# Whisper-6/DynamicTreeAttn

Measured on AMD Instinct MI355X. Metric: tree-attn fwd+bwd tokens/sec, Qwen3-0.6B tau2-16k tries, higher is better.
Workload: dtype bf16

## Files before the change

### dynamictreeattn_amd/_lib.py

```python
from __future__ import annotations

import ctypes as C
import os

from .build import LIB

_lib = None
_i32, _i64, _f32, _vp = C.c_int32, C.c_int64, C.c_float, C.c_void_p

_PROTOS = {
    "dta_version": ([], C.c_int),
    "dta_take_pending_error": ([C.c_char_p, _i32], C.c_int),
    "dta_lcp_adjacent": ([_vp, _vp, _vp, _i32, _vp, _vp, _vp], C.c_int),
    "dta_leafize": ([_vp, _vp, _i32, _vp, _vp, _vp, _vp, _vp], C.c_int),
    "dta_preorder_meta": ([_vp] * 8 + [_i32, _i32] + [_vp] * 4 + [_vp], C.c_int),
    "dta_tree_attn_fwd": ([_vp] * 8 + [_i32] * 6 + [_i64] * 3 + [_f32, _i32, _vp], C.c_int),
    "dta_tree_attn_bwd": ([_vp] * 14 + [_i32] * 6 + [_i64] * 5 + [_f32, _i32, _i32, _vp], C.c_int),
    "dta_tree_attn_fwd_ex": ([_vp] * 8 + [_i32] * 6 + [_i64] * 8 + [_f32, _i32, _vp], C.c_int),
    "dta_tree_attn_bwd_ex": ([_vp] * 14 + [_i32] * 6 + [_i64] * 12 + [_f32, _i32, _i32, _i32, _vp, _i32, _vp, _i32, _vp, _vp], C.c_int),
    "dta_tree_attn_fwd_win": ([_vp] * 8 + [_i32] * 6 + [_i64] * 8 + [_f32, _i32, _vp, _i32, _vp], C.c_int),
    "dta_tree_attn_bwd_win": ([_vp] * 14 + [_i32] * 6 + [_i64] * 12 + [_f32, _i32, _i32, _i32, _vp, _i32, _vp, _i32, _vp, _vp, _i32, _vp], C.c_int),
    "dta_window_lo": ([_vp] * 4 + [_i32, _i32, _i32, _vp, _vp], C.c_int),
    "dta_logprob_entropy_fwd": ([_vp] * 8 + [_i32, _i32, _i64, _f32, _i32, _vp], C.c_int),
    "dta_logprob_entropy_shard_stats": ([_vp] * 6 + [_i32, _i32, _i64, _f32, _i32, _vp], C.c_int),
    "dta_logprob_entropy_bwd": ([_vp] * 10 + [_i32, _i32, _i64, _i64, _f32, _i32, _vp], C.c_int),
    "dta_rmsnorm_fwd": ([_vp] * 6 + [_i32, _i32, _f32, _i32, _vp], C.c_int),
    "dta_rmsnorm_bwd_blocks": ([_i32], C.c_int),
    "dta_rmsnorm_bwd": ([_vp] * 7 + [_i32, _i32, _i32, _vp], C.c_int),
    "dta_qk_norm_rope_fwd": ([_vp] * 5 + [_i32, _i32, _i32, _i64, _f32, _i32, _vp], C.c_int),
    "dta_qk_norm_rope_bwd_blocks": ([_i64], C.c_int),
    "dta_qk_norm_rope_bwd": ([_vp] * 7 + [_i32, _i32, _i32, _i64, _i64, _i64, _i64, _i32, _vp], C.c_int),
    "dta_swiglu_fwd": ([_vp] * 3 + [_i64, _i32, _i64, _i32, _vp], C.c_int),
    "dta_swiglu_bwd": ([_vp] * 5 + [_i64, _i32, _i64, _i64, _i32, _vp], C.c_int),
    "dta_transpose": ([_vp, _vp, _i64, _i64, _i64, _i64, _i32, _vp], C.c_int),
    "dta_sum_slabs": ([_vp, _i64, _i64, _i64, _vp, _vp, _i32, _vp], C.c_int),
    "dta_moe_router_fwd": ([_vp] * 4 + [_i32] * 5 + [_vp], C.c_int),
    "dta_moe_router_bwd": ([_vp] * 5 + [_i32] * 5 + [_vp], C.c_int),
    "dta_moe_permute_workspace": ([_i32, _i32], C.c_int),
    "dta_moe_tile_bound": ([_i32, _i32], C.c_int),
    "dta_moe_permute": ([_vp, _i32, _i32, _i32] + [_vp] * 5 + [_vp], C.c_int),
    "dta_moe_grouped_gemm": ([_i32] + [_vp] * 7 + [_i32] * 5 + [_vp], C.c_int),
    "dta_moe_combine_fwd": ([_vp] * 4 + [_i32] * 4 + [_vp], C.c_int),
    "dta_moe_combine_bwd": ([_vp] * 6 + [_i32] * 4 + [_vp], C.c_int),
    "dta_lora_down": ([_vp, _i64, _vp, _i64, _vp, _i64, _vp, _i32, _i32, _i32, _i32, _vp], C.c_int),
    "dta_lora_wgrad_slabs": ([_i32, _i32], C.c_int),
    "dta_lora_wgrad": ([_vp, _i64, _vp, _i64, _vp, _vp, _i32, _i32, _i32, _i32, _vp], C.c_int),
}
EXPORTS = tuple(_PROTOS)
_ERR = {-1: "DTA_EINVAL", -2: "DTA_EUNSUPPORTED", -3: "DTA_EALIGN", -4: "DTA_ELAUNCH", -5: "DTA_EPRIOR"}


def _hip_runtimes_mapped():
    try:
        with open("/proc/self/maps") as f:
            return sorted({line.split()[-1] for line in f if "libamdhip64" in line})
    except OSError:
        return []


def lib():
    global _lib
    if _lib is None:
        if not os.path.exists(LIB):
            raise RuntimeError(f"{LIB} is missing: run `python -m dynamictreeattn_amd.build` (hipcc, gfx950). "
                               "There is no CPU fallback for the hot path.")
        import torch
        l = C.CDLL(LIB)
        rts = _hip_runtimes_mapped()
        if len(rts) > 1:
            raise RuntimeError("more than one libamdhip64 is mapped into this process: " + ", ".join(rts) +
                               " — libdta_mi355x.so must resolve to the HIP runtime torch ships")
        for name, (args, res) in _PROTOS.items():
            fn = getattr(l, name)
            fn.argtypes, fn.restype = args, res
        _lib = l
    return _lib


def check(status: int, what: str):
    if status == 0:
        return
    if status == -5:
        buf = C.create_string_buffer(256)
        code = lib().dta_take_pending_error(buf, 256)
        raise RuntimeError(f"{what}: not launched, a HIP error was already pending on this thread: {buf.value.decode() or code} "
                           f"(hipError {code}; now cleared — after an asynchronous kernel fault the GPU context stays unusable)")
    raise RuntimeError(f"{what} failed: {_ERR.get(status, status)}")


def ptr(t):
    return None if t is None else t.data_ptr()
```

### dynamictreeattn_amd/csrc/tree_attn.hip

```cpp
#include <hip/hip_runtime.h>
#include <stdint.h>
#include <type_traits>
#include "dta_common.h"

#if defined(DTA_STAMP) && DTA_STAMP
__device__ unsigned long long* dta_stamp_buf = nullptr;
extern "C" int dta_debug_set_stamp_buffer(void* p) { return hipMemcpyToSymbol(HIP_SYMBOL(dta_stamp_buf), &p, sizeof(p)) == hipSuccess ? 0 : -4; }
#define DTA_STAMP_DECL unsigned long long st_prev_, st_sum_[6] = {0, 0, 0, 0, 0, 0}; unsigned long long st_tiles_ = 0; \
  __builtin_amdgcn_sched_barrier(0); asm volatile("s_memtime %0\n\ts_waitcnt lgkmcnt(0)" : "=s"(st_prev_) :: "memory"); __builtin_amdgcn_sched_barrier(0);
#define DTA_STAMP_AT(K) { unsigned long long t_; __builtin_amdgcn_sched_barrier(0); asm volatile("s_memtime %0\n\ts_waitcnt lgkmcnt(0)" : "=s"(t_) :: "memory"); \
  __builtin_amdgcn_sched_barrier(0); st_sum_[K] += t_ - st_prev_; st_prev_ = t_; }
#define DTA_STAMP_TILE ++st_tiles_;
#define DTA_STAMP_STORE if (dta_stamp_buf && lane == 0) { unsigned long long* o_ = dta_stamp_buf + ((size_t)blockIdx.x * 8 + wave) * 8; \
  for (int k_ = 0; k_ < 6; ++k_) o_[k_] = st_sum_[k_]; o_[6] = st_tiles_; o_[7] = (unsigned long long)__builtin_amdgcn_s_getreg(0xF804) ; }
#else
#define DTA_STAMP_DECL
#define DTA_STAMP_AT(K)
#define DTA_STAMP_TILE
#define DTA_STAMP_STORE
#endif

namespace {

typedef __attribute__((ext_vector_type(16))) float f32x16;
typedef __attribute__((ext_vector_type(4))) short s16x4;
typedef __attribute__((ext_vector_type(8))) short s16x8;
typedef __attribute__((ext_vector_type(8))) __bf16 bf16x8;
typedef __attribute__((ext_vector_type(8))) _Float16 f16x8;
typedef __attribute__((ext_vector_type(4))) __bf16 bf16x4;
typedef __attribute__((ext_vector_type(4))) _Float16 f16x4;

template <int DT> struct Ty;
template <> struct Ty<DTA_BF16> {
  using e = __bf16; using v8 = bf16x8; using v4 = bf16x4;
  static __device__ __forceinline__ f32x16 mma(v8 a, v8 b, f32x16 c) { return __builtin_amdgcn_mfma_f32_32x32x16_bf16(a, b, c, 0, 0, 0); }
};
template <> struct Ty<DTA_F16> {
  using e = _Float16; using v8 = f16x8; using v4 = f16x4;
  static __device__ __forceinline__ f32x16 mma(v8 a, v8 b, f32x16 c) { return __builtin_amdgcn_mfma_f32_32x32x16_f16(a, b, c, 0, 0, 0); }
};

struct AttnParams {
  const void *q, *k, *v, *o, *dout;
  void *out, *dq, *dk, *dv;
  float *lse_w; const float* lse_r; float* delta;
  const int32_t *subtree_end, *run_ptr, *runs, *ktile_qend;
  const int32_t *dkv_units, *dkv_splits; float* dkv_ws;
  int32_t Tq, Tk, q_offset, Hq, Hkv, group;
  int32_t hgroups, head0;
  int64_t q_st, q_sh, kv_st, kv_sh, v_st, v_sh, o_st, o_sh, dq_st, dq_sh, dkv_st, dkv_sh;
  float scale; int32_t accumulate; int32_t ktile;
};
struct AttnParamsW : AttnParams { const int32_t* win_lo; int32_t window; };
template <bool WIN> using AttnP = typename std::conditional<WIN, AttnParamsW, AttnParams>::type;

constexpr float LOG2E = 1.4426950408889634f;

__device__ __forceinline__ int swz64(int row) { return ((row & 2) << 1) | ((row >> 2) & 3); }
template <int D> __device__ __forceinline__ int img_off_d(int row, int ch) {
  if constexpr (D == 128) return row * 256 + ((ch ^ (((row & 3) << 2) | ((row >> 2) & 3))) << 4);
  else { static_assert(D == 64, "head_dim 64 or 128"); return row * 128 + ((ch ^ swz64(row)) << 4); }
}
template <int D> constexpr int tile_bytes() { return 64 * 2 * D; }

template <class V8, int D> __device__ __forceinline__ V8 row_frag(const char* img, int row, int ch) {
  return *reinterpret_cast<const V8*>(img + img_off_d<D>(row, ch));
}

__device__ __forceinline__ s16x4 tr_read(const char* p) {
  return __builtin_amdgcn_ds_read_tr16_b64_v4i16((__attribute__((address_space(3))) s16x4*)(p));
}

template <class V8, int D> __device__ __forceinline__ V8 tr_frag(const char* img, int R0, int mb, int lane) {
  const int G = lane >> 4, hh = lane >> 5, i = lane & 15, qd = i >> 2, p = i & 3;
  const int ch = 4 * mb + 2 * (G & 1) + (p >> 1);
  const int ra = R0 + 4 * hh + qd;
  s16x4 lo = tr_read(img + img_off_d<D>(ra, ch) + 8 * (p & 1));
  s16x4 hi = tr_read(img + img_off_d<D>(ra + 8, ch) + 8 * (p & 1));
  s16x8 both = {lo[0], lo[1], lo[2], lo[3], hi[0], hi[1], hi[2], hi[3]};
  return __builtin_bit_cast(V8, both);
}

template <int DT> __device__ __forceinline__ typename Ty<DT>::v8 pack_half(const f32x16& x, int s2) {
  typename Ty<DT>::v8 r;
#pragma unroll
  for (int j = 0; j < 8; ++j) r[j] = (typename Ty<DT>::e)x[8 * s2 + j];
  return r;
}

__device__ __forceinline__ float fast_exp2(float x) { return __builtin_amdgcn_exp2f(x); }

struct TileIter {
  const int32_t* runs; int ri, re;
  int k0, kend, flag;
  int diag_first_q;
  __device__ __forceinline__ bool load_run() {
    while (ri < re) {
      k0 = __builtin_amdgcn_readfirstlane(runs[4 * ri]); kend = __builtin_amdgcn_readfirstlane(runs[4 * ri + 1]);
      flag = __builtin_amdgcn_readfirstlane(runs[4 * ri + 2]);
      if (k0 < kend) return true;
      ++ri;
    }
    return false;
  }
  __device__ __forceinline__ bool advance() {
    k0 += 64;
    if (k0 < kend) return true;
    if (runs == nullptr) return false;
    ++ri;
    return load_run();
  }
  __device__ __forceinline__ bool masked() const {
    if (runs == nullptr) return (k0 + 63 > diag_first_q) || (k0 + 64 > kend);
    return flag != 0 || (k0 + 64 > kend);
  }
};

#ifndef DTA_FWD_THR
#define DTA_FWD_THR 4.0f
#endif
constexpr float FWD_THR = DTA_FWD_THR;
constexpr int SE_BYTES = 256;

__device__ __forceinline__ float max3(float a, float b, float c) { return fmaxf(fmaxf(a, b), c); }
__device__ __forceinline__ float half_max(float x) {
  const unsigned u = __float_as_uint(x);
  const auto r = __builtin_amdgcn_permlane32_swap(u, u, false, false);
  return fmaxf(__uint_as_float(r[0]), __uint_as_float(r[1]));
}

template <int D> struct FragOffsT { int row[D / 16]; int tr[D / 16]; };
template <int D> __device__ __forceinline__ FragOffsT<D> frag_offsets(int lane) {
  FragOffsT<D> o;
  const int r = lane & 31, h = lane >> 5;
#pragma unroll
  for (int s = 0; s < D / 16; ++s) o.row[s] = img_off_d<D>(r, 2 * s + h);
  const int G = lane >> 4, i = lane & 15, qd = i >> 2, pp = i & 3;
#pragma unroll
  for (int mb = 0; mb < D / 32; ++mb) {
    const int ch = 4 * mb + 2 * (G & 1) + (pp >> 1);
    o.tr[mb] = img_off_d<D>(4 * h + qd, ch) + 8 * (pp & 1);
    o.tr[D / 32 + mb] = img_off_d<D>(4 * h + qd + 8, ch) + 8 * (pp & 1);
  }
  return o;
}
template <class V8> __device__ __forceinline__ V8 tr_pair(const char* lo_p, const char* hi_p) {
  s16x4 lo = tr_read(lo_p);
  s16x4 hi = tr_read(hi_p);
  s16x8 both = {lo[0], lo[1], lo[2], lo[3], hi[0], hi[1], hi[2], hi[3]};
  return __builtin_bit_cast(V8, both);
}
template <class V8, int D> __device__ __forceinline__ V8 tr_frag_o(const char* img_r0, const FragOffsT<D>& o, int mb) {
  s16x4 lo = tr_read(img_r0 + o.tr[mb]);
  s16x4 hi = tr_read(img_r0 + o.tr[D / 32 + mb]);
  s16x8 both = {lo[0], lo[1], lo[2], lo[3], hi[0], hi[1], hi[2], hi[3]};
  return __builtin_bit_cast(V8, both);
}

__device__ __forceinline__ uint32_t lds_addr(const void* p) {
  return (uint32_t)(uintptr_t)(__attribute__((address_space(3))) const char*)(p);
}
__device__ __forceinline__ void dma_pair2(uint32_t oa0, uint32_t oa1, const void* ba, uint32_t ob0, uint32_t ob1, const void* bb, uint32_t lds) {
  asm volatile(
      "s_nop 4\n\t"
      "s_mov_b32 m0, %6\n\t"
      "s_nop 0\n\t"
      "global_load_lds_dwordx4 %0, %4\n\t"
      "s_add_u32 m0, %6, 0x4000\n\t"
      "s_nop 0\n\t"
      "global_load_lds_dwordx4 %2, %5\n\t"
      "s_add_u32 m0, %6, 0x400\n\t"
      "s_nop 0\n\t"
      "global_load_lds_dwordx4 %1, %4\n\t"
      "s_add_u32 m0, %6, 0x4400\n\t"
      "s_nop 0\n\t"
      "global_load_lds_dwordx4 %3, %5"
      :: "v"(oa0), "v"(oa1), "v"(ob0), "v"(ob1), "s"(ba), "s"(bb), "s"(lds) : "memory", "scc");
}
__device__ __forceinline__ void dma_dword(uint32_t off, const void* base, uint32_t lds) {
  asm volatile("s_nop 4\n\ts_mov_b32 m0, %2\n\ts_nop 0\n\tglobal_load_lds_dword %0, %1" :: "v"(off), "s"(base), "s"(lds) : "memory");
}
#define DMA_WAIT() asm volatile("s_waitcnt vmcnt(0)" ::: "memory")

template <int D> __device__ __forceinline__ uint32_t dma_src_off_d(int row, int img_row, int lane, int64_t stride, int esz) {
  if constexpr (D == 128) return (uint32_t)((row * stride + ((lane & 15) ^ (((img_row & 3) << 2) | ((img_row >> 2) & 3))) * 8) * (int64_t)esz);
  else return (uint32_t)((row * stride + ((lane & 7) ^ swz64(img_row)) * 8) * (int64_t)esz);
}
template <int D> constexpr int dma_lane_row_shift() { return D == 128 ? 4 : 3; }
template <int TB> __device__ __forceinline__ void dma_one2(uint32_t oa, const void* ba, uint32_t ob, const void* bb, uint32_t lds) {
  asm volatile(
      "s_nop 4\n\t"
      "s_mov_b32 m0, %4\n\t"
      "s_nop 0\n\t"
      "global_load_lds_dwordx4 %0, %2\n\t"
      "s_add_u32 m0, %4, %5\n\t"
      "s_nop 0\n\t"
      "global_load_lds_dwordx4 %1, %3"
      :: "v"(oa), "v"(ob), "s"(ba), "s"(bb), "s"(lds), "n"(TB) : "memory", "scc");
}

#define DTA_KV_PPW(NW) (DH / 8 / (NW))
#define DTA_KV_ROW(NW, I) ((512 / DH) * (wave * DTA_KV_PPW(NW) + (I)) + (lane >> dma_lane_row_shift<DH>()))
#define DTA_KV_OFFSETS(NW)                                                                                 \
  uint32_t voff_k[DTA_KV_PPW(NW)], voff_v[DTA_KV_PPW(NW)];                                                 \
  _Pragma("unroll") for (int i_ = 0; i_ < DTA_KV_PPW(NW); ++i_) {                                          \
    const int row_ = DTA_KV_ROW(NW, i_);                                                                   \
    voff_k[i_] = dma_src_off_d<DH>(row_, row_, lane, p.kv_st, sizeof(e));                                  \
    voff_v[i_] = dma_src_off_d<DH>(row_, row_, lane, p.v_st, sizeof(e)); }
#define DTA_KV_DMA(BASE, K0, NW)                                                                           \
  { char* base_ = (BASE); const int k0_ = (K0);                                                            \
    if (wave == 0) {                                                                                       \
      if (p.subtree_end) { int ki_ = k0_ + lane; ki_ = ki_ < p.Tk ? ki_ : p.Tk - 1;                        \
        dma_dword((uint32_t)ki_ * 4u, p.subtree_end, lds_addr(base_ + 2 * tile_bytes<DH>())); }           \
      else reinterpret_cast<int*>(base_ + 2 * tile_bytes<DH>())[lane] = 0x7fffffff; }                     \
    const char* kb_ = reinterpret_cast<const char*>(kbase) + (int64_t)k0_ * p.kv_st * (int64_t)sizeof(e);  \
    const char* vb_ = reinterpret_cast<const char*>(vbase) + (int64_t)k0_ * p.v_st * (int64_t)sizeof(e);   \
    uint32_t ok_[DTA_KV_PPW(NW)], ov_[DTA_KV_PPW(NW)];                                                     \
    _Pragma("unroll") for (int i_ = 0; i_ < DTA_KV_PPW(NW); ++i_) { ok_[i_] = voff_k[i_]; ov_[i_] = voff_v[i_]; } \
    if (k0_ + 64 > p.Tk) {                          \
      _Pragma("unroll") for (int i_ = 0; i_ < DTA_KV_PPW(NW); ++i_) {                                      \
        const int row_ = DTA_KV_ROW(NW, i_);                                                               \
        const int rr_ = k0_ + row_ < p.Tk ? row_ : p.Tk - 1 - k0_;                                         \
        ok_[i_] = dma_src_off_d<DH>(rr_, row_, lane, p.kv_st, sizeof(e)); ov_[i_] = dma_src_off_d<DH>(rr_, row_, lane, p.v_st, sizeof(e)); } } \
    if constexpr (DH == 128) {                                                                             \
      _Pragma("unroll") for (int i_ = 0; i_ < DTA_KV_PPW(NW); i_ += 2)                                     \
        dma_pair2(ok_[i_], ok_[i_ + 1], kb_, ov_[i_], ov_[i_ + 1], vb_, lds_addr(base_ + (wave * DTA_KV_PPW(NW) + i_) * 1024)); \
    } else {                                                                                               \
      _Pragma("unroll") for (int i_ = 0; i_ < DTA_KV_PPW(NW); ++i_)                                        \
        dma_one2<tile_bytes<DH>()>(ok_[i_], kb_, ov_[i_], vb_, lds_addr(base_ + (wave * DTA_KV_PPW(NW) + i_) * 1024)); } }

#ifndef DTA_V_PRELOAD_N
#define DTA_V_PRELOAD_N 4
#endif
#if DTA_V_PRELOAD_N
#define DTA_V_PRELOAD v8 vpre_[DTA_V_PRELOAD_N]; _Pragma("unroll") for (int i_ = 0; i_ < DTA_V_PRELOAD_N; ++i_) { vpre_[i_] = tr_frag_o<v8>(Vs + 32 * DH * (i_ / (DH / 32)), offs, i_ % (DH / 32)); asm volatile("" : "+v"(vpre_[i_])); }
#define DTA_V_FRAG(S4, DB) (((DH / 32) * (S4) + (DB) < DTA_V_PRELOAD_N) ? vpre_[(DH / 32) * (S4) + (DB) < DTA_V_PRELOAD_N ? (DH / 32) * (S4) + (DB) : 0] : tr_frag_o<v8>(Vs + 32 * DH * (S4), offs, (DB)))
#else
#define DTA_V_PRELOAD
#define DTA_V_FRAG(S4, DB) tr_frag_o<v8>(Vs + 32 * DH * (S4), offs, (DB))
#endif

#ifndef DTA_SCORE_ORDER
#define DTA_SCORE_ORDER 1
#endif
#if DTA_SCORE_ORDER
#define DTA_SCORE_MFMAS                                                                                    \
    { v8 ka_ = *reinterpret_cast<const v8*>(Ks + offs.row[0]), kb2_ = *reinterpret_cast<const v8*>(Ks + 64 * DH + offs.row[0]); \
      _Pragma("unroll") for (int s = 0; s < DH / 16; ++s) {                                                \
        v8 na_ = ka_, nb_ = kb2_;                                                                          \
        if (s < DH / 16 - 1) { na_ = *reinterpret_cast<const v8*>(Ks + offs.row[s + 1]); nb_ = *reinterpret_cast<const v8*>(Ks + 64 * DH + offs.row[s + 1]); } \
        X[0] = T::mma(ka_, qf[s], X[0]); X[1] = T::mma(kb2_, qf[s], X[1]);                                 \
        ka_ = na_; kb2_ = nb_;                                                                             \
      } }
#else
#define DTA_SCORE_MFMAS                                                                                    \
    _Pragma("unroll") for (int kb = 0; kb < 2; ++kb)                                                       \
      _Pragma("unroll") for (int s = 0; s < DH / 16; ++s)                                                  \
        X[kb] = T::mma(*reinterpret_cast<const v8*>(Ks + 64 * DH * kb + offs.row[s]), qf[s], X[kb]);
#endif

template <int DT, int HPB, int DH, bool WIN>
__global__ __launch_bounds__(256 * HPB, 2) void tree_attn_fwd_kernel(AttnP<WIN> p) {
  using T = Ty<DT>; using e = typename T::e; using v8 = typename T::v8; using v4 = typename T::v4;
  constexpr int TB = tile_bytes<DH>(), NKS = DH / 16, NDB = DH / 32;
  constexpr int NW = 4 * HPB, BUF = 2 * TB + SE_BYTES;
  __shared__ __attribute__((aligned(16))) char smem[2 * BUF];

  const int tid = threadIdx.x, lane = tid & 63, r = lane & 31, h = lane >> 5;
  const int wave = __builtin_amdgcn_readfirstlane(tid >> 6);
  const int hb = wave >> 2, rw = wave & 3;
  const int bid = blockIdx.x;
  const int hgroups = p.hgroups;
  const int kvh = bid % p.Hkv; const int rest = bid / p.Hkv; const int hgb = rest % hgroups;
  const int nqt = (p.Tq + DTA_QTILE - 1) / DTA_QTILE;
  const int qt = nqt - 1 - rest / hgroups;
  const int hq = kvh * p.group + p.head0 + hgb * HPB + hb;
  const int q0 = qt * DTA_QTILE;
  const int qrow = q0 + rw * 32 + r;
  const int qrow_c = qrow < p.Tq ? qrow : p.Tq - 1;
  const int qidx = p.q_offset + qrow;
  int wlo = 0, wmax = 0;
  if constexpr (WIN) {
    wlo = p.win_lo ? p.win_lo[qrow_c] : (qidx - p.window + 1 > 0 ? qidx - p.window + 1 : 0);
    wmax = p.win_lo ? 0 : p.q_offset + (q0 + DTA_QTILE < p.Tq ? q0 + DTA_QTILE : p.Tq) - p.window;
  }

  TileIter it; it.runs = p.runs; it.diag_first_q = p.subtree_end ? -64 : p.q_offset + q0;
  if (p.runs) { it.ri = p.run_ptr[qt]; it.re = p.run_ptr[qt + 1]; if (!it.load_run()) return; }
  else { it.ri = 0; it.re = 1; it.k0 = 0; it.flag = 1; int last = p.q_offset + (q0 + DTA_QTILE < p.Tq ? q0 + DTA_QTILE : p.Tq); it.kend = last < p.Tk ? last : p.Tk; if (it.kend <= 0) return; }
  if constexpr (WIN) {
    const int lo0 = p.q_offset + q0 - p.window + 1;
    if (!p.runs && !p.win_lo && lo0 > 0) { it.k0 = lo0; if (it.k0 >= it.kend) return; }
  }

  const e* qp = reinterpret_cast<const e*>(p.q) + (int64_t)qrow_c * p.q_st + (int64_t)hq * p.q_sh;
  v8 qf[NKS];
#pragma unroll
  for (int s = 0; s < NKS; ++s) qf[s] = *reinterpret_cast<const v8*>(qp + 16 * s + 8 * h);

  const e* kbase = reinterpret_cast<const e*>(p.k) + (int64_t)kvh * p.kv_sh;
  const e* vbase = reinterpret_cast<const e*>(p.v) + (int64_t)kvh * p.v_sh;
  const FragOffsT<DH> offs = frag_offsets<DH>(lane);
  DTA_KV_OFFSETS(NW)

  f32x16 O[NDB];
#pragma unroll
  for (int db = 0; db < NDB; ++db)
#pragma unroll
    for (int g = 0; g < 16; ++g) O[db][g] = 0.f;
  float m = -1e30f, lsum = 0.f;
  const float c = p.scale * LOG2E;

  int ck0 = it.k0, ckend = it.kend; bool cmask = it.masked() || (WIN && it.k0 < wmax);
  DTA_KV_DMA(smem, it.k0, NW)
  bool has_next = it.advance();
#pragma unroll
  for (int s = 0; s < NKS; ++s) asm volatile("" : "+v"(qf[s]));
  DMA_WAIT(); __syncthreads();

#define FWD_TILE(BUFI)                                                                                     \
  {                                                                                                        \
    int nk0_ = 0, nkend_ = 0; bool nmask_ = false;                                                         \
    DTA_STAMP_AT(5) DTA_STAMP_TILE                                                                         \
    if (has_next) { nk0_ = it.k0; nkend_ = it.kend; nmask_ = it.masked() || (WIN && it.k0 < wmax); DTA_KV_DMA(smem + (1 - (BUFI)) * BUF, it.k0, NW) } \
    DTA_STAMP_AT(0)                                                                                        \
    const char* Ks = smem + (BUFI) * BUF; const char* Vs = Ks + TB;                                \
    const int* se_s = reinterpret_cast<const int*>(Ks + 2 * TB);                                   \
    f32x16 X[2];                                                                                           \
    _Pragma("unroll") for (int kb = 0; kb < 2; ++kb)                                                       \
      _Pragma("unroll") for (int g = 0; g < 16; ++g) X[kb][g] = 0.f;                                       \
    DTA_SCORE_MFMAS                                                                                        \
    DTA_STAMP_AT(1)                                                                                        \
    if (cmask) {                                                                                           \
      const int qlim = qidx < ckend ? qidx : ckend - 1;       \
      _Pragma("unroll") for (int kb = 0; kb < 2; ++kb)                                                     \
        _Pragma("unroll") for (int gq = 0; gq < 4; ++gq) {                                                 \
          const int kl = 32 * kb + 8 * gq + 4 * h;                                                         \
          const int4 se4 = *reinterpret_cast<const int4*>(se_s + kl);                                      \
          const int sev[4] = {se4.x, se4.y, se4.z, se4.w};                                                 \
          _Pragma("unroll") for (int j = 0; j < 4; ++j) {                                                  \
            const bool ok = (ck0 + kl + j <= qlim) && (qidx < sev[j]) && (!WIN || ck0 + kl + j >= wlo);    \
            X[kb][4 * gq + j] = ok ? X[kb][4 * gq + j] : -INFINITY;                                        \
          }                                                                                                \
        }                                                                                                  \
    }                                                                                                      \
    DTA_V_PRELOAD                                                                                          \
    float mx = max3(X[0][0], X[0][1], X[0][2]), mx1 = max3(X[1][0], X[1][1], X[1][2]);    \
    _Pragma("unroll") for (int g = 3; g < 15; g += 2) { mx = max3(mx, X[0][g], X[0][g + 1]); mx1 = max3(mx1, X[1][g], X[1][g + 1]); } \
    mx = max3(mx, X[0][15], mx1);                                                                          \
    mx = half_max(fmaxf(mx, X[1][15]));         \
    const float mc = mx * c;                                                                               \
    if (__any(mc > m + FWD_THR)) {              \
      const float mnew = fmaxf(m, mc);                                                                     \
      const float alpha = fast_exp2(m - mnew);                                                             \
      m = mnew; lsum *= alpha;                                                                             \
      _Pragma("unroll") for (int db = 0; db < NDB; ++db)                                                   \
        _Pragma("unroll") for (int g = 0; g < 16; ++g) O[db][g] *= alpha;                                  \
    }                                                                                                      \
    DTA_STAMP_AT(2)                                                                                        \
    _Pragma("unroll") for (int kb = 0; kb < 2; ++kb)                                                       \
      _Pragma("unroll") for (int g = 0; g < 16; ++g) { const float pv = fast_exp2(__builtin_fmaf(X[kb][g], c, -m)); lsum += pv; X[kb][g] = pv; } \
    _Pragma("unroll") for (int s4 = 0; s4 < 4; ++s4) {                                                     \
      const v8 pb = pack_half<DT>(X[s4 >> 1], s4 & 1);                                                     \
      _Pragma("unroll") for (int db = 0; db < NDB; ++db) O[db] = T::mma(DTA_V_FRAG(s4, db), pb, O[db]);      \
    }                                                                                                      \
    DTA_STAMP_AT(3)                                                                                        \
    DMA_WAIT(); __syncthreads();                         \
    DTA_STAMP_AT(4)                                                                                        \
    if (!has_next) break;                                                                                  \
    ck0 = nk0_; ckend = nkend_; cmask = nmask_;                                                            \
    has_next = it.advance();                                                                               \
  }
  DTA_STAMP_DECL
  while (true) {
    FWD_TILE(0)
    FWD_TILE(1)
  }
#undef FWD_TILE
  DTA_STAMP_STORE

  lsum += __shfl_xor(lsum, 32);
  const float inv = 1.f / lsum;
  if (qrow < p.Tq) {
    e* op = reinterpret_cast<e*>(p.out) + (int64_t)qrow * p.o_st + (int64_t)hq * p.o_sh;
#pragma unroll
    for (int db = 0; db < NDB; ++db)
#pragma unroll
      for (int gq = 0; gq < 4; ++gq) {
        v4 w;
#pragma unroll
        for (int j = 0; j < 4; ++j) w[j] = (e)(O[db][4 * gq + j] * inv);
        *reinterpret_cast<v4*>(op + 32 * db + 8 * gq + 4 * h) = w;
      }
    if (h == 0) p.lse_w[(int64_t)hq * p.Tq + qrow] = m + __builtin_amdgcn_logf(lsum);
  }
}

template <int DT, int HPB, int DH, bool WIN>
__global__ __launch_bounds__(256 * HPB, 2) void tree_attn_bwd_dq_kernel(AttnP<WIN> p) {
  using T = Ty<DT>; using e = typename T::e; using v8 = typename T::v8; using v4 = typename T::v4;
  constexpr int TB = tile_bytes<DH>(), NKS = DH / 16, NDB = DH / 32;
  __shared__ __attribute__((aligned(16))) char smem[2 * (2 * TB + SE_BYTES)];

  const int tid = threadIdx.x, lane = tid & 63, r = lane & 31, h = lane >> 5;
  const int wave = __builtin_amdgcn_readfirstlane(tid >> 6);
  const int hb = wave >> 2, rw = wave & 3;
  const int bid = blockIdx.x;
  const int hgroups = p.hgroups;
  const int kvh = bid % p.Hkv; const int rest = bid / p.Hkv; const int hgb = rest % hgroups;
  const int nqt = (p.Tq + DTA_QTILE - 1) / DTA_QTILE;
  const int qt = nqt - 1 - rest / hgroups;
  const int hq = kvh * p.group + p.head0 + hgb * HPB + hb;
  const int q0 = qt * DTA_QTILE;
  const int qrow = q0 + rw * 32 + r;
  const int qrow_c = qrow < p.Tq ? qrow : p.Tq - 1;
  const int qidx = p.q_offset + qrow;
  int wlo = 0, wmax = 0;
  if constexpr (WIN) {
    wlo = p.win_lo ? p.win_lo[qrow_c] : (qidx - p.window + 1 > 0 ? qidx - p.window + 1 : 0);
    wmax = p.win_lo ? 0 : p.q_offset + (q0 + DTA_QTILE < p.Tq ? q0 + DTA_QTILE : p.Tq) - p.window;
  }

  const e* qp = reinterpret_cast<const e*>(p.q) + (int64_t)qrow_c * p.q_st + (int64_t)hq * p.q_sh;
  const e* dop = reinterpret_cast<const e*>(p.dout) + (int64_t)qrow_c * p.o_st + (int64_t)hq * p.o_sh;
  const e* op = reinterpret_cast<const e*>(p.o) + (int64_t)qrow_c * p.o_st + (int64_t)hq * p.o_sh;
  v8 qf[NKS], dof[NKS];
  float dsum = 0.f;
#pragma unroll
  for (int s = 0; s < NKS; ++s) {
    qf[s] = *reinterpret_cast<const v8*>(qp + 16 * s + 8 * h);
    dof[s] = *reinterpret_cast<const v8*>(dop + 16 * s + 8 * h);
    const v8 of = *reinterpret_cast<const v8*>(op + 16 * s + 8 * h);
#pragma unroll
    for (int j = 0; j < 8; ++j) dsum += (float)dof[s][j] * (float)of[j];
  }
  dsum += __shfl_xor(dsum, 32);
  const float delta = dsum;
  const float lse2 = p.lse_r[(int64_t)hq * p.Tq + qrow_c];
  if (h == 0 && qrow < p.Tq) p.delta[(int64_t)hq * p.Tq + qrow] = -delta;

  TileIter it; it.runs = p.runs; it.diag_first_q = p.subtree_end ? -64 : p.q_offset + q0;
  bool any = true;
  if (p.runs) { it.ri = p.run_ptr[qt]; it.re = p.run_ptr[qt + 1]; any = it.load_run(); }
  else { it.ri = 0; it.re = 1; it.k0 = 0; it.flag = 1; int last = p.q_offset + (q0 + DTA_QTILE < p.Tq ? q0 + DTA_QTILE : p.Tq); it.kend = last < p.Tk ? last : p.Tk; any = it.kend > 0; }
  if constexpr (WIN) {
    const int lo0 = p.q_offset + q0 - p.window + 1;
    if (!p.runs && !p.win_lo && lo0 > 0) { it.k0 = lo0; any = any && it.k0 < it.kend; }
  }

  const e* kbase = reinterpret_cast<const e*>(p.k) + (int64_t)kvh * p.kv_sh;
  const e* vbase = reinterpret_cast<const e*>(p.v) + (int64_t)kvh * p.v_sh;
  constexpr int NW = 4 * HPB, BUF = 2 * TB + SE_BYTES;
  DTA_KV_OFFSETS(NW)

  f32x16 DQ[NDB];
#pragma unroll
  for (int db = 0; db < NDB; ++db)
#pragma unroll
    for (int g = 0; g < 16; ++g) DQ[db][g] = 0.f;
  const float c = p.scale * LOG2E;

  f32x16 DI;
#pragma unroll
  for (int g = 0; g < 16; ++g) DI[g] = -delta;
  if (any) {
    int ck0 = it.k0, ckend = it.kend; bool cmask = it.masked() || (WIN && it.k0 < wmax);
    DTA_KV_DMA(smem, it.k0, NW)
    bool has_next = it.advance();
    DMA_WAIT(); __syncthreads();
    int cur = 0;
    while (true) {
      int nk0 = 0, nkend = 0; bool nmask = false;
      if (has_next) { nk0 = it.k0; nkend = it.kend; nmask = it.masked() || (WIN && it.k0 < wmax); DTA_KV_DMA(smem + (cur ^ 1) * BUF, it.k0, NW) }
      const char* Ks = smem + cur * BUF; const char* Vs = Ks + TB;
      const int* se_s = reinterpret_cast<const int*>(Ks + 2 * TB);
#pragma unroll
      for (int kb = 0; kb < 2; ++kb) {
        f32x16 X, DP;
#pragma unroll
        for (int g = 0; g < 16; ++g) X[g] = 0.f;
        {
          v8 kf_ = row_frag<v8, DH>(Ks, 32 * kb + r, h), vf_ = row_frag<v8, DH>(Vs, 32 * kb + r, h);
#pragma unroll
          for (int s = 0; s < NKS; ++s) {
            v8 nk_ = kf_, nv_ = vf_;
            if (s < NKS - 1) { nk_ = row_frag<v8, DH>(Ks, 32 * kb + r, 2 * s + 2 + h); nv_ = row_frag<v8, DH>(Vs, 32 * kb + r, 2 * s + 2 + h); }
            X = T::mma(kf_, qf[s], X);
            DP = T::mma(vf_, dof[s], s == 0 ? DI : DP);
            kf_ = nk_; vf_ = nv_;
          }
          __builtin_amdgcn_sched_group_barrier(0x100, 4, 0);
#pragma unroll
          for (int i_ = 0; i_ < NKS - 2; ++i_) { __builtin_amdgcn_sched_group_barrier(0x008, 2, 0); __builtin_amdgcn_sched_group_barrier(0x100, 2, 0); }
          __builtin_amdgcn_sched_group_barrier(0x008, 4, 0);
        }
        if (cmask) {
          const int qlim = qidx < ckend ? qidx : ckend - 1;
#pragma unroll
          for (int gq = 0; gq < 4; ++gq) {
            const int kl = 32 * kb + 8 * gq + 4 * h;
            const int4 se4 = *reinterpret_cast<const int4*>(se_s + kl);
            const int sev[4] = {se4.x, se4.y, se4.z, se4.w};
#pragma unroll
            for (int j = 0; j < 4; ++j) {
              const int g = 4 * gq + j;
              const bool ok = (ck0 + kl + j <= qlim) && (qidx < sev[j]) && (!WIN || ck0 + kl + j >= wlo);
              const float pv = ok ? fast_exp2(__builtin_fmaf(X[g], c, -lse2)) : 0.f;
              X[g] = pv * DP[g];
            }
          }
        } else {
#pragma unroll
          for (int g = 0; g < 16; ++g) X[g] = fast_exp2(__builtin_fmaf(X[g], c, -lse2)) * DP[g];
        }
#pragma unroll
        for (int s2 = 0; s2 < 2; ++s2) {
          const v8 db_ = pack_half<DT>(X, s2);
#pragma unroll
          for (int db = 0; db < NDB; ++db) DQ[db] = T::mma(tr_frag<v8, DH>(Ks, 32 * kb + 16 * s2, db, lane), db_, DQ[db]);
        }
      }
      DMA_WAIT(); __syncthreads();
      if (!has_next) break;
      cur ^= 1; ck0 = nk0; ckend = nkend; cmask = nmask;
      has_next = it.advance();
    }
  }
  if (qrow < p.Tq) {
    e* dqp = reinterpret_cast<e*>(p.dq) + (int64_t)qrow * p.dq_st + (int64_t)hq * p.dq_sh;
#pragma unroll
    for (int db = 0; db < NDB; ++db)
#pragma unroll
      for (int gq = 0; gq < 4; ++gq) {
        v4 w;
#pragma unroll
        for (int j = 0; j < 4; ++j) w[j] = (e)(DQ[db][4 * gq + j] * p.scale);
        *reinterpret_cast<v4*>(dqp + 32 * db + 8 * gq + 4 * h) = w;
      }
  }
}

#ifndef DTA_KV2_PIN
#define DTA_KV2_PIN 2
#endif
#if DTA_KV2_PIN == 2
#define DTA_KV2_PIN_ORDER                                                                                  \
    __builtin_amdgcn_sched_group_barrier(0x100, 4, 0);                                                     \
    _Pragma("unroll") for (int i_ = 0; i_ < 2 * NKS; ++i_) { __builtin_amdgcn_sched_group_barrier(0x100, 2, 0); __builtin_amdgcn_sched_group_barrier(0x008, 1, 0); }
#elif DTA_KV2_PIN
#define DTA_KV2_PIN_ORDER                                                                                  \
    __builtin_amdgcn_sched_group_barrier(0x100, 12, 0);                                                    \
    _Pragma("unroll") for (int i_ = 0; i_ < NKS - 2; ++i_) { __builtin_amdgcn_sched_group_barrier(0x008, 2, 0); __builtin_amdgcn_sched_group_barrier(0x100, 4, 0); } \
    __builtin_amdgcn_sched_group_barrier(0x008, 4, 0);
#else
#define DTA_KV2_PIN_ORDER
#endif

template <int D> constexpr int kv2_slot() { return 2 * (D / 16) * 1024; }
template <int D> constexpr int kv2_frags() { return 4 * kv2_slot<D>(); }
template <int D, bool WIN> constexpr int kv2_buf() { return 2 * tile_bytes<D>() + (WIN ? 768 : 512); }
template <int D, bool WIN> constexpr int kv2_lds() { return kv2_frags<D>() + 2 * kv2_buf<D, WIN>() + 16; }

template <int DT, int DH, bool WIN>
__global__ __launch_bounds__(512, 2) void tree_attn_bwd_dkv2_kernel(AttnP<WIN> p) {
  using T = Ty<DT>; using e = typename T::e; using v8 = typename T::v8; using v4 = typename T::v4;
  constexpr int KT = 128;
  constexpr int TB = tile_bytes<DH>(), NKS = DH / 16, NDB = DH / 32, KV2_FRAGS = kv2_frags<DH>(), KV2_BUF = kv2_buf<DH, WIN>(), KSLOT = kv2_slot<DH>();
  __shared__ __attribute__((aligned(16))) char smem_all[kv2_lds<DH, WIN>()];
  const int tid8 = threadIdx.x, tid = tid8 & 255, lane = tid & 63, r = lane & 31, h = lane >> 5;
  const int wave8 = __builtin_amdgcn_readfirstlane(tid8 >> 6);
  const int grp = wave8 >> 2, wave = wave8 & 3;
  char* kvs = smem_all + wave * KSLOT;
  char* smem = smem_all + KV2_FRAGS;
  const int bid = blockIdx.x;
  const int kvh = bid % p.Hkv; const int unit = bid / p.Hkv;
  const int kt = p.dkv_units ? p.dkv_units[4 * unit] : unit;
  const int slab = p.dkv_units ? p.dkv_units[4 * unit + 3] : -1;
  const int k0 = kt * KT;
  const int q_hi = p.q_offset + p.Tq;
  const int kidx = k0 + wave * 32 + r;
  int se_l;
  { const int kc = kidx < p.Tk ? kidx : p.Tk - 1;
    int se = (kidx < p.Tk) ? (p.subtree_end ? p.subtree_end[kidx] : 0x7fffffff) : 0;
    se_l = se < q_hi ? se : q_hi;
    if (grp == 0) {
      const e* kp = reinterpret_cast<const e*>(p.k) + (int64_t)kc * p.kv_st + (int64_t)kvh * p.kv_sh;
      const e* vp = reinterpret_cast<const e*>(p.v) + (int64_t)kc * p.v_st + (int64_t)kvh * p.v_sh;
#pragma unroll
      for (int s = 0; s < NKS; ++s) {
        *reinterpret_cast<v8*>(kvs + s * 1024 + lane * 16) = *reinterpret_cast<const v8*>(kp + 16 * s + 8 * h);
        *reinterpret_cast<v8*>(kvs + KSLOT / 2 + s * 1024 + lane * 16) = *reinterpret_cast<const v8*>(vp + 16 * s + 8 * h);
      }
    } }
  int* se_min_s = reinterpret_cast<int*>(smem_all + KV2_FRAGS + 2 * KV2_BUF);
  { int mn = se_l;
#pragma unroll
    for (int o = 32; o > 0; o >>= 1) { const int t = __shfl_xor(mn, o); mn = t < mn ? t : mn; }
    if (lane == 0 && grp == 0) se_min_s[wave] = mn; }
  __syncthreads();
  const int se_min = __builtin_amdgcn_readfirstlane(min(min(se_min_s[0], se_min_s[1]), min(se_min_s[2], se_min_s[3])));

  const FragOffsT<DH> offs = frag_offsets<DH>(lane);
  f32x16 DK[NDB], DV[NDB];
#pragma unroll
  for (int db = 0; db < NDB; ++db)
#pragma unroll
    for (int g = 0; g < 16; ++g) { DK[db][g] = 0.f; DV[db][g] = 0.f; }

  int qbeg, qend;
  if (p.dkv_units) { qbeg = __builtin_amdgcn_readfirstlane(p.dkv_units[4 * unit + 1]); qend = __builtin_amdgcn_readfirstlane(p.dkv_units[4 * unit + 2]); }
  else {
    qbeg = k0 > p.q_offset ? k0 : p.q_offset;
    qend = p.ktile_qend ? p.ktile_qend[kt] : q_hi; qend = qend < q_hi ? qend : q_hi;
    if constexpr (WIN) if (!p.win_lo) {
      const int64_t wl = (int64_t)k0 + KT - 1 + p.window; qend = wl < qend ? (int)wl : qend;
    }
  }
  const int ntile = qend > qbeg ? (qend - qbeg + 63) / 64 : 0;
  const int total = ntile * p.group;
  const float c = p.scale * LOG2E;

  constexpr int NP = DH / 64;
  uint32_t voff_q[NP], voff_d[NP];
#pragma unroll
  for (int i = 0; i < NP; ++i) {
    const int row_ = 8 * wave8 + (512 / DH) * i + (lane >> dma_lane_row_shift<DH>());
    voff_q[i] = dma_src_off_d<DH>(row_, row_, lane, p.q_st, sizeof(e));
    voff_d[i] = dma_src_off_d<DH>(row_, row_, lane, p.o_st, sizeof(e));
  }
  const uint32_t lds_tiles = lds_addr(smem);
  const int64_t q_step = 64 * p.q_st * (int64_t)sizeof(e), d_step = 64 * p.o_st * (int64_t)sizeof(e);
  const int64_t q_wrap = p.q_sh * (int64_t)sizeof(e) - ntile * q_step, d_wrap = p.o_sh * (int64_t)sizeof(e) - ntile * d_step;
  int64_t q_cur = ((int64_t)(kvh * p.group) * p.q_sh + (int64_t)(qbeg - p.q_offset) * p.q_st) * (int64_t)sizeof(e);
  int64_t d_cur = ((int64_t)(kvh * p.group) * p.o_sh + (int64_t)(qbeg - p.q_offset) * p.o_st) * (int64_t)sizeof(e);
  int64_t c_cur = (int64_t)(kvh * p.group) * p.Tq;
  int row_n = qbeg - p.q_offset, ti_n = 0;
#define KV2_DMA(B)                                                                                         \
  { const uint32_t lb_ = lds_tiles + (uint32_t)(B) * KV2_BUF;                                              \
    if (wave8 < 2) { int qr_ = row_n + lane; qr_ = qr_ < p.Tq ? qr_ : p.Tq - 1;    \
      dma_dword((uint32_t)qr_ * 4u, (wave8 == 0 ? p.lse_r : p.delta) + c_cur, lb_ + 2 * TB + wave8 * 256); } \
    if constexpr (WIN) if (wave8 == 2 && p.win_lo) { int qr_ = row_n + lane; qr_ = qr_ < p.Tq ? qr_ : p.Tq - 1;    \
      dma_dword((uint32_t)qr_ * 4u, p.win_lo, lb_ + 2 * TB + 512); }                                       \
    uint32_t oq_[NP], od_[NP];                                                                             \
    _Pragma("unroll") for (int i_ = 0; i_ < NP; ++i_) { oq_[i_] = voff_q[i_]; od_[i_] = voff_d[i_]; }      \
    if (row_n + 64 > p.Tq) {                        \
      _Pragma("unroll") for (int i_ = 0; i_ < NP; ++i_) {                                                  \
        const int ra_ = 8 * wave8 + (512 / DH) * i_ + (lane >> dma_lane_row_shift<DH>());                  \
        const int ca_ = row_n + ra_ < p.Tq ? ra_ : p.Tq - 1 - row_n;                                       \
        oq_[i_] = dma_src_off_d<DH>(ca_, ra_, lane, p.q_st, sizeof(e)); od_[i_] = dma_src_off_d<DH>(ca_, ra_, lane, p.o_st, sizeof(e)); } } \
    if constexpr (NP == 2) dma_pair2(oq_[0], oq_[1], reinterpret_cast<const char*>(p.q) + q_cur, od_[0], od_[1], reinterpret_cast<const char*>(p.dout) + d_cur, lb_ + wave8 * 2048); \
    else dma_one2<TB>(oq_[0], reinterpret_cast<const char*>(p.q) + q_cur, od_[0], reinterpret_cast<const char*>(p.dout) + d_cur, lb_ + wave8 * 1024); \
    ++ti_n; row_n += 64; q_cur += q_step; d_cur += d_step;                                                 \
    if (ti_n >= ntile) { ti_n = 0; row_n = qbeg - p.q_offset; q_cur += q_wrap; d_cur += d_wrap; c_cur += p.Tq; } }

  int ar[NKS], at[NKS];
#pragma unroll
  for (int j = 0; j < NKS; ++j) { ar[j] = offs.row[j] + grp * (64 * DH); at[j] = offs.tr[j] + grp * (64 * DH); }
  const int rc_off = (32 * grp + 4 * h) * 4;

#define KV2_TILE(BUFI)                                                                                     \
  {                                                                                                        \
    const int ti = ti_c;                                                                                   \
    ti_c += 1;                                                                                             \
    if (ti_c >= ntile) ti_c = 0;                                                                           \
    if (idx + 1 < total) KV2_DMA(1 - (BUFI))       \
    const char* tb = smem + (BUFI) * KV2_BUF;                                                              \
    const char* rc = tb + 2 * TB + rc_off;                                                         \
    const int qi0 = qbeg + 64 * ti + 32 * grp;                        \
    bool full = (qbeg + 64 * ti >= k0 + KT - 1) && (qbeg + 64 * ti + 63 < se_min);    \
    if constexpr (WIN) full = full && !p.win_lo && qbeg + 64 * ti + 64 - p.window <= k0;    \
     \
    f32x16 S, DP;                                                                                          \
    _Pragma("unroll") for (int gq = 0; gq < 4; ++gq) {                                                     \
      const float4 d4 = *reinterpret_cast<const float4*>(rc + 256 + 32 * gq);                              \
      DP[4 * gq] = d4.x; DP[4 * gq + 1] = d4.y; DP[4 * gq + 2] = d4.z; DP[4 * gq + 3] = d4.w;              \
    }                                                                                                      \
    _Pragma("unroll") for (int g = 0; g < 16; ++g) S[g] = 0.f;                                             \
    _Pragma("unroll") for (int s = 0; s < NKS; ++s) {                                                      \
      const v8 aq = *reinterpret_cast<const v8*>(tb + ar[s]);                                              \
      const v8 ad = *reinterpret_cast<const v8*>(tb + ar[s] + TB);                                         \
      const v8 kfs = *reinterpret_cast<const v8*>(kvs + s * 1024 + lane * 16);                             \
      const v8 vfs = *reinterpret_cast<const v8*>(kvs + KSLOT / 2 + s * 1024 + lane * 16);                 \
      S = T::mma(aq, kfs, S); DP = T::mma(ad, vfs, DP);                                                    \
    }                                                                                                      \
    DTA_KV2_PIN_ORDER                                                                                      \
    float nl[16];                                                                                          \
    _Pragma("unroll") for (int gq = 0; gq < 4; ++gq) {                                                     \
      const float4 l4 = *reinterpret_cast<const float4*>(rc + 32 * gq);                                    \
      nl[4 * gq] = l4.x; nl[4 * gq + 1] = l4.y; nl[4 * gq + 2] = l4.z; nl[4 * gq + 3] = l4.w;              \
    }                                                                                                      \
    if (full) {                                                                                            \
      _Pragma("unroll") for (int g = 0; g < 16; ++g) {                                                     \
        const float pv = fast_exp2(__builtin_fmaf(S[g], c, -nl[g]));                                       \
        S[g] = pv;                                                                                         \
        DP[g] = pv * DP[g];                                                                                \
      }                                                                                                    \
    } else {                                                                                               \
      int wl[16];                                    \
      if constexpr (WIN) {                                                                                 \
        if (p.win_lo) {                                                                                    \
          _Pragma("unroll") for (int gq = 0; gq < 4; ++gq) {                                               \
            const int4 w4 = *reinterpret_cast<const int4*>(rc + 512 + 32 * gq);                            \
            wl[4 * gq] = w4.x; wl[4 * gq + 1] = w4.y; wl[4 * gq + 2] = w4.z; wl[4 * gq + 3] = w4.w; }      \
        } else {                                                                                           \
          _Pragma("unroll") for (int g = 0; g < 16; ++g) wl[g] = qi0 + 8 * (g >> 2) + 4 * h + (g & 3) - p.window + 1; } \
      }                                                                                                    \
      _Pragma("unroll") for (int g = 0; g < 16; ++g) {                                                     \
        const int qi = qi0 + 8 * (g >> 2) + 4 * h + (g & 3);                                               \
        const bool ok = (kidx <= qi) && (qi < se_l) && (!WIN || kidx >= wl[g]);                            \
        const float pv = ok ? fast_exp2(__builtin_fmaf(S[g], c, -nl[g])) : 0.f;                            \
        S[g] = pv;                                                                                         \
        DP[g] = pv * DP[g];                                                                                \
      }                                                                                                    \
    }                                                                                                      \
    _Pragma("unroll") for (int s2 = 0; s2 < 2; ++s2) {                                                     \
      const v8 pb = pack_half<DT>(S, s2), sbf = pack_half<DT>(DP, s2);                                     \
      _Pragma("unroll") for (int db = 0; db < NDB; ++db) {                                                 \
        const v8 adt = tr_pair<v8>(tb + at[db] + TB + 32 * DH * s2, tb + at[NDB + db] + TB + 32 * DH * s2); \
        const v8 aqt = tr_pair<v8>(tb + at[db] + 32 * DH * s2, tb + at[NDB + db] + 32 * DH * s2);          \
        DV[db] = T::mma(adt, pb, DV[db]); DK[db] = T::mma(aqt, sbf, DK[db]);                               \
      }                                                                                                    \
    }                                                                                                      \
    DMA_WAIT(); __syncthreads();                                                                           \
    ++idx;                                                                                                 \
  }

  {
    int ti_c = 0;
    if (total > 0) KV2_DMA(0)
    DMA_WAIT(); __syncthreads();
    int idx = 0;
    while (idx < total) {
      KV2_TILE(0)
      if (idx >= total) break;
      KV2_TILE(1)
    }
  }
#undef KV2_TILE
#undef KV2_DMA
  {
    float* red = reinterpret_cast<float*>(smem_all);
#pragma unroll
    for (int db = 0; db < NDB; ++db) {
      if (grp == 1) {
#pragma unroll
        for (int g = 0; g < 16; ++g) { red[g * 256 + tid] = DK[db][g]; red[(16 + g) * 256 + tid] = DV[db][g]; }
      }
      __syncthreads();
      if (grp == 0) {
#pragma unroll
        for (int g = 0; g < 16; ++g) { DK[db][g] += red[g * 256 + tid]; DV[db][g] += red[(16 + g) * 256 + tid]; }
      }
      __syncthreads();
    }
    if (grp == 1) return;
  }
#pragma unroll
  for (int db = 0; db < NDB; ++db)
#pragma unroll
    for (int g = 0; g < 16; ++g) DK[db][g] *= p.scale;
  const int kloc = wave * 32 + r;
  if (slab >= 0) {
    float* ws = p.dkv_ws + ((int64_t)slab * p.Hkv + kvh) * (2 * KT * DH) + (int64_t)kloc * DH;
#pragma unroll
    for (int db = 0; db < NDB; ++db)
#pragma unroll
      for (int gq = 0; gq < 4; ++gq) {
        const int d = 32 * db + 8 * gq + 4 * h;
        *reinterpret_cast<float4*>(ws + d) = make_float4(DK[db][4 * gq], DK[db][4 * gq + 1], DK[db][4 * gq + 2], DK[db][4 * gq + 3]);
        *reinterpret_cast<float4*>(ws + KT * DH + d) = make_float4(DV[db][4 * gq], DV[db][4 * gq + 1], DV[db][4 * gq + 2], DV[db][4 * gq + 3]);
      }
  } else if (kidx < p.Tk && p.accumulate == 2) {
    float* dkp = reinterpret_cast<float*>(p.dk) + (int64_t)kidx * p.dkv_st + (int64_t)kvh * p.dkv_sh;
    float* dvp = reinterpret_cast<float*>(p.dv) + (int64_t)kidx * p.dkv_st + (int64_t)kvh * p.dkv_sh;
#pragma unroll
    for (int db = 0; db < NDB; ++db)
#pragma unroll
      for (int gq = 0; gq < 4; ++gq) {
        const int d = 32 * db + 8 * gq + 4 * h;
        float4 a = *reinterpret_cast<const float4*>(dkp + d), b = *reinterpret_cast<const float4*>(dvp + d);
        a.x += DK[db][4 * gq]; a.y += DK[db][4 * gq + 1]; a.z += DK[db][4 * gq + 2]; a.w += DK[db][4 * gq + 3];
        b.x += DV[db][4 * gq]; b.y += DV[db][4 * gq + 1]; b.z += DV[db][4 * gq + 2]; b.w += DV[db][4 * gq + 3];
        *reinterpret_cast<float4*>(dkp + d) = a;
        *reinterpret_cast<float4*>(dvp + d) = b;
      }
  } else if (kidx < p.Tk) {
    e* dkp = reinterpret_cast<e*>(p.dk) + (int64_t)kidx * p.dkv_st + (int64_t)kvh * p.dkv_sh;
    e* dvp = reinterpret_cast<e*>(p.dv) + (int64_t)kidx * p.dkv_st + (int64_t)kvh * p.dkv_sh;
#pragma unroll
    for (int db = 0; db < NDB; ++db)
#pragma unroll
      for (int gq = 0; gq < 4; ++gq) {
        const int d = 32 * db + 8 * gq + 4 * h;
        v4 wk, wv;
        if (p.accumulate) {
          const v4 ok_ = *reinterpret_cast<const v4*>(dkp + d); const v4 ov_ = *reinterpret_cast<const v4*>(dvp + d);
#pragma unroll
          for (int j = 0; j < 4; ++j) { wk[j] = (e)(DK[db][4 * gq + j] + (float)ok_[j]); wv[j] = (e)(DV[db][4 * gq + j] + (float)ov_[j]); }
        } else {
#pragma unroll
          for (int j = 0; j < 4; ++j) { wk[j] = (e)DK[db][4 * gq + j]; wv[j] = (e)DV[db][4 * gq + j]; }
        }
        *reinterpret_cast<v4*>(dkp + d) = wk;
        *reinterpret_cast<v4*>(dvp + d) = wv;
      }
  }
}

constexpr int FIN_SPLIT = 8;
template <int DT, int DH>
__global__ __launch_bounds__(256) void tree_attn_bwd_dkv_finalize_kernel(AttnParams p) {
  using e = typename Ty<DT>::e; using v4 = typename Ty<DT>::v4;
  const int KT = p.ktile;
  const int kvh = blockIdx.x % p.Hkv, sp = blockIdx.x / p.Hkv;
  const int kt = p.dkv_splits[4 * sp], first = p.dkv_splits[4 * sp + 1], n = p.dkv_splits[4 * sp + 2];
  constexpr int Q4 = DH / 4, Q4_SHIFT = DH == 128 ? 5 : 4;
  const int per = 2 * KT * Q4 / FIN_SPLIT;
  const float* ws0 = p.dkv_ws + ((int64_t)first * p.Hkv + kvh) * (2 * KT * DH);
  const int64_t slab_st = (int64_t)p.Hkv * (2 * KT * DH);
  for (int i = blockIdx.y * per + threadIdx.x; i < (blockIdx.y + 1) * per; i += 256) {
    const int which = i / (KT * Q4), rem = i - which * KT * Q4;
    const int key = rem >> Q4_SHIFT, d = (rem & (Q4 - 1)) << 2;
    const int kidx = kt * KT + key;
    if (kidx >= p.Tk) continue;
    float4 acc = make_float4(0.f, 0.f, 0.f, 0.f);
    int j = 0;
    for (; j + 4 <= n; j += 4) {
      const float4 a0 = *reinterpret_cast<const float4*>(ws0 + (j + 0) * slab_st + (int64_t)i * 4);
      const float4 a1 = *reinterpret_cast<const float4*>(ws0 + (j + 1) * slab_st + (int64_t)i * 4);
      const float4 a2 = *reinterpret_cast<const float4*>(ws0 + (j + 2) * slab_st + (int64_t)i * 4);
      const float4 a3 = *reinterpret_cast<const float4*>(ws0 + (j + 3) * slab_st + (int64_t)i * 4);
      acc.x += a0.x; acc.y += a0.y; acc.z += a0.z; acc.w += a0.w;
      acc.x += a1.x; acc.y += a1.y; acc.z += a1.z; acc.w += a1.w;
      acc.x += a2.x; acc.y += a2.y; acc.z += a2.z; acc.w += a2.w;
      acc.x += a3.x; acc.y += a3.y; acc.z += a3.z; acc.w += a3.w;
    }
    for (; j < n; ++j) {
      const float4 v = *reinterpret_cast<const float4*>(ws0 + j * slab_st + (int64_t)i * 4);
      acc.x += v.x; acc.y += v.y; acc.z += v.z; acc.w += v.w;
    }
    if (p.accumulate == 2) {
      float* outf = reinterpret_cast<float*>(which ? p.dv : p.dk) + (int64_t)kidx * p.dkv_st + (int64_t)kvh * p.dkv_sh + d;
      float4 o = *reinterpret_cast<const float4*>(outf);
      o.x += acc.x; o.y += acc.y; o.z += acc.z; o.w += acc.w;
      *reinterpret_cast<float4*>(outf) = o;
      continue;
    }
    e* out = reinterpret_cast<e*>(which ? p.dv : p.dk) + (int64_t)kidx * p.dkv_st + (int64_t)kvh * p.dkv_sh + d;
    if (p.accumulate) { const v4 o = *reinterpret_cast<const v4*>(out); acc.x += (float)o[0]; acc.y += (float)o[1]; acc.z += (float)o[2]; acc.w += (float)o[3]; }
    v4 w; w[0] = (e)acc.x; w[1] = (e)acc.y; w[2] = (e)acc.z; w[3] = (e)acc.w;
    *reinterpret_cast<v4*>(out) = w;
  }
}

template <int DT, int DH, bool WIN>
void launch_bwd(const AttnP<WIN>& p, const AttnP<WIN>& pp, const AttnP<WIN>& ps, int npair, dim3 gqp, dim3 gqs, int ndkv, bool fin, int n_splits,
                int which, hipStream_t st) {
  if (which & 1) {
    if (npair > 0) hipLaunchKernelGGL((tree_attn_bwd_dq_kernel<DT, 2, DH, WIN>), gqp, dim3(512), 0, st, pp);
    if (p.group % 2) hipLaunchKernelGGL((tree_attn_bwd_dq_kernel<DT, 1, DH, WIN>), gqs, dim3(256), 0, st, ps);
  }
  if (which & 2) hipLaunchKernelGGL((tree_attn_bwd_dkv2_kernel<DT, DH, WIN>), dim3(ndkv * p.Hkv), dim3(512), 0, st, p);
  if (fin && p.dkv_units && n_splits > 0)
    hipLaunchKernelGGL((tree_attn_bwd_dkv_finalize_kernel<DT, DH>), dim3(n_splits * p.Hkv, FIN_SPLIT), dim3(256), 0, st, static_cast<const AttnParams&>(p));
}

inline bool aligned16(const void* p) { return (reinterpret_cast<uintptr_t>(p) & 15) == 0; }

}

template <bool WIN>
static int attn_fwd(const void* q, const void* k, const void* v, void* out, float* lse,
                                    const int32_t* subtree_end, const int32_t* run_ptr, const int32_t* runs,
                                    int32_t Tq, int32_t Tk, int32_t q_offset, int32_t Hq, int32_t Hkv, int32_t head_dim,
                                    int64_t q_st, int64_t q_sh, int64_t kv_st, int64_t kv_sh, int64_t v_st, int64_t v_sh, int64_t o_st, int64_t o_sh,
                                    float scale, int32_t dtype, const int32_t* win_lo, int32_t window, void* stream) {
  if (!q || !k || !v || !out || !lse || Tq <= 0 || Tk <= 0 || Hq <= 0 || Hkv <= 0 || q_offset < 0) return DTA_EINVAL;
  if ((runs == nullptr) != (run_ptr == nullptr)) return DTA_EINVAL;
  if ((head_dim != 128 && head_dim != 64) || Hq % Hkv != 0 || (dtype != DTA_BF16 && dtype != DTA_F16 && dtype != DTA_F32)) return DTA_EUNSUPPORTED;
  if (!aligned16(q) || !aligned16(k) || !aligned16(v) || !aligned16(out) || (q_st | q_sh | kv_st | kv_sh | v_st | v_sh | o_st | o_sh) % 8 != 0) return DTA_EALIGN;
  if (dtype == DTA_F32) {
    DTA_REFUSE_IF_PRIOR_ERROR();
    return dta_attn_fwd_f32(q, k, v, out, lse, subtree_end, run_ptr, runs, Tq, Tk, q_offset, Hq, Hkv, head_dim, q_st, q_sh, kv_st, kv_sh, v_st, v_sh, o_st, o_sh,
                            scale, win_lo, WIN ? window : 0, static_cast<hipStream_t>(stream));
  }
  if (kv_st < 0 || v_st < 0 || kv_st > (1 << 24) || v_st > (1 << 24)) return DTA_EUNSUPPORTED;
  AttnP<WIN> p{};
  if constexpr (WIN) { p.win_lo = win_lo; p.window = window; }
  p.q = q; p.k = k; p.v = v; p.out = out; p.lse_w = lse; p.subtree_end = subtree_end; p.run_ptr = run_ptr; p.runs = runs;
  p.Tq = Tq; p.Tk = Tk; p.q_offset = q_offset; p.Hq = Hq; p.Hkv = Hkv; p.group = Hq / Hkv;
  p.q_st = q_st; p.q_sh = q_sh; p.kv_st = kv_st; p.kv_sh = kv_sh; p.v_st = v_st; p.v_sh = v_sh; p.o_st = o_st; p.o_sh = o_sh; p.scale = scale;
  const int nqt = (Tq + DTA_QTILE - 1) / DTA_QTILE;
  hipStream_t st = static_cast<hipStream_t>(stream);
  DTA_REFUSE_IF_PRIOR_ERROR();
  const int npair = p.group / 2;
  if (npair > 0) {
    p.hgroups = npair; p.head0 = 0;
    dim3 grid(nqt * Hkv * npair), block(512);
    if (head_dim == 64) {
      if (dtype == DTA_BF16) hipLaunchKernelGGL((tree_attn_fwd_kernel<DTA_BF16, 2, 64, WIN>), grid, block, 0, st, p);
      else hipLaunchKernelGGL((tree_attn_fwd_kernel<DTA_F16, 2, 64, WIN>), grid, block, 0, st, p);
    } else {
      if (dtype == DTA_BF16) hipLaunchKernelGGL((tree_attn_fwd_kernel<DTA_BF16, 2, 128, WIN>), grid, block, 0, st, p);
      else hipLaunchKernelGGL((tree_attn_fwd_kernel<DTA_F16, 2, 128, WIN>), grid, block, 0, st, p);
    }
  }
  if (p.group % 2) {
    p.hgroups = 1; p.head0 = p.group - 1;
    dim3 grid(nqt * Hkv), block(256);
    if (head_dim == 64) {
      if (dtype == DTA_BF16) hipLaunchKernelGGL((tree_attn_fwd_kernel<DTA_BF16, 1, 64, WIN>), grid, block, 0, st, p);
      else hipLaunchKernelGGL((tree_attn_fwd_kernel<DTA_F16, 1, 64, WIN>), grid, block, 0, st, p);
    } else {
      if (dtype == DTA_BF16) hipLaunchKernelGGL((tree_attn_fwd_kernel<DTA_BF16, 1, 128, WIN>), grid, block, 0, st, p);
      else hipLaunchKernelGGL((tree_attn_fwd_kernel<DTA_F16, 1, 128, WIN>), grid, block, 0, st, p);
    }
  }
  return DTA_LAUNCH_STATUS();
}

template <bool WIN>
static int attn_bwd(const void* q, const void* k, const void* v, const void* out, const void* dout,
                                    const float* lse, float* delta, void* dq, void* dk, void* dv,
                                    const int32_t* subtree_end, const int32_t* run_ptr, const int32_t* runs,
                                    const int32_t* ktile_qend,
                                    int32_t Tq, int32_t Tk, int32_t q_offset, int32_t Hq, int32_t Hkv, int32_t head_dim,
                                    int64_t q_st, int64_t q_sh, int64_t kv_st, int64_t kv_sh, int64_t v_st, int64_t v_sh, int64_t o_st, int64_t o_sh,
                                    int64_t dq_st, int64_t dq_sh, int64_t dkv_st, int64_t dkv_sh,
                                    float scale, int32_t dtype, int32_t accumulate, int32_t which,
                                    const int32_t* dkv_units, int32_t n_units, const int32_t* dkv_splits, int32_t n_splits, float* dkv_ws,
                                    const int32_t* win_lo, int32_t window, void* stream) {
  if (!q || !k || !v || !out || !dout || !lse || !delta || !dq || !dk || !dv || Tq <= 0 || Tk <= 0 || Hq <= 0 || Hkv <= 0 || q_offset < 0) return DTA_EINVAL;
  if ((runs == nullptr) != (run_ptr == nullptr)) return DTA_EINVAL;
  if (dkv_units && (n_units <= 0 || n_splits < 0 || (n_splits > 0 && (!dkv_splits || !dkv_ws)))) return DTA_EINVAL;
  if ((head_dim != 128 && head_dim != 64) || Hq % Hkv != 0 || (dtype != DTA_BF16 && dtype != DTA_F16 && dtype != DTA_F32) || accumulate < 0 || accumulate > 2) return DTA_EUNSUPPORTED;
  if (!aligned16(q) || !aligned16(k) || !aligned16(v) || !aligned16(out) || !aligned16(dout) || !aligned16(dq) || !aligned16(dk) || !aligned16(dv) ||
      (q_st | q_sh | kv_st | kv_sh | v_st | v_sh | o_st | o_sh | dq_st | dq_sh | dkv_st | dkv_sh) % 8 != 0) return DTA_EALIGN;
  if (dtype == DTA_F32) {
    if ((which & 7) == 0) return DTA_EINVAL;
    DTA_REFUSE_IF_PRIOR_ERROR();
    return dta_attn_bwd_f32(q, k, v, out, dout, lse, delta, dq, dk, dv, subtree_end, run_ptr, runs, ktile_qend, Tq, Tk, q_offset, Hq, Hkv, head_dim,
                            q_st, q_sh, kv_st, kv_sh, v_st, v_sh, o_st, o_sh, dq_st, dq_sh, dkv_st, dkv_sh, scale, accumulate, which,
                            win_lo, WIN ? window : 0, static_cast<hipStream_t>(stream));
  }
  if (q_st < 0 || o_st < 0 || q_st > (1 << 24) || o_st > (1 << 24)) return DTA_EUNSUPPORTED;
  AttnP<WIN> p{};
  if constexpr (WIN) { p.win_lo = win_lo; p.window = window; }
  p.q = q; p.k = k; p.v = v; p.o = out; p.dout = dout; p.lse_r = lse; p.delta = delta; p.dq = dq; p.dk = dk; p.dv = dv;
  p.subtree_end = subtree_end; p.run_ptr = run_ptr; p.runs = runs; p.ktile_qend = ktile_qend;
  p.dkv_units = dkv_units; p.dkv_splits = dkv_splits; p.dkv_ws = dkv_ws;
  p.Tq = Tq; p.Tk = Tk; p.q_offset = q_offset; p.Hq = Hq; p.Hkv = Hkv; p.group = Hq / Hkv;
  p.q_st = q_st; p.q_sh = q_sh; p.kv_st = kv_st; p.kv_sh = kv_sh; p.v_st = v_st; p.v_sh = v_sh; p.o_st = o_st; p.o_sh = o_sh;
  p.dq_st = dq_st; p.dq_sh = dq_sh; p.dkv_st = dkv_st; p.dkv_sh = dkv_sh; p.scale = scale; p.accumulate = accumulate;
  const int nqt = (Tq + DTA_QTILE - 1) / DTA_QTILE;
  p.ktile = DTA_KTILE;
  const int nkt = (Tk + p.ktile - 1) / p.ktile;
  hipStream_t st = static_cast<hipStream_t>(stream);
  DTA_REFUSE_IF_PRIOR_ERROR();
  if ((which & 7) == 0) return DTA_EINVAL;
  const bool fin = ((which & 2) && !(which & 8)) || (which & 4);
  const int ndkv = dkv_units ? n_units : nkt;
  const int npair = p.group / 2;
  AttnP<WIN> pp = p, ps = p;
  pp.hgroups = npair; pp.head0 = 0; ps.hgroups = 1; ps.head0 = p.group - 1;
  const dim3 gqp(nqt * Hkv * (npair > 0 ? npair : 1)), gqs(nqt * Hkv);
  if (head_dim == 64) {
    if (dtype == DTA_BF16) launch_bwd<DTA_BF16, 64, WIN>(p, pp, ps, npair, gqp, gqs, ndkv, fin, n_splits, which, st);
    else launch_bwd<DTA_F16, 64, WIN>(p, pp, ps, npair, gqp, gqs, ndkv, fin, n_splits, which, st);
  } else {
    if (dtype == DTA_BF16) launch_bwd<DTA_BF16, 128, WIN>(p, pp, ps, npair, gqp, gqs, ndkv, fin, n_splits, which, st);
    else launch_bwd<DTA_F16, 128, WIN>(p, pp, ps, npair, gqp, gqs, ndkv, fin, n_splits, which, st);
  }
  return DTA_LAUNCH_STATUS();
}

extern "C" int dta_tree_attn_fwd_ex(const void* q, const void* k, const void* v, void* out, float* lse,
                                    const int32_t* subtree_end, const int32_t* run_ptr, const int32_t* runs,
                                    int32_t Tq, int32_t Tk, int32_t q_offset, int32_t Hq, int32_t Hkv, int32_t head_dim,
                                    int64_t q_st, int64_t q_sh, int64_t kv_st, int64_t kv_sh, int64_t v_st, int64_t v_sh, int64_t o_st, int64_t o_sh,
                                    float scale, int32_t dtype, void* stream) {
  return attn_fwd<false>(q, k, v, out, lse, subtree_end, run_ptr, runs, Tq, Tk, q_offset, Hq, Hkv, head_dim, q_st, q_sh, kv_st, kv_sh, v_st, v_sh,
                         o_st, o_sh, scale, dtype, nullptr, 0, stream);
}

extern "C" int dta_tree_attn_bwd_ex(const void* q, const void* k, const void* v, const void* out, const void* dout,
                                    const float* lse, float* delta, void* dq, void* dk, void* dv,
                                    const int32_t* subtree_end, const int32_t* run_ptr, const int32_t* runs,
                                    const int32_t* ktile_qend,
                                    int32_t Tq, int32_t Tk, int32_t q_offset, int32_t Hq, int32_t Hkv, int32_t head_dim,
                                    int64_t q_st, int64_t q_sh, int64_t kv_st, int64_t kv_sh, int64_t v_st, int64_t v_sh, int64_t o_st, int64_t o_sh,
                                    int64_t dq_st, int64_t dq_sh, int64_t dkv_st, int64_t dkv_sh,
                                    float scale, int32_t dtype, int32_t accumulate, int32_t which,
                                    const int32_t* dkv_units, int32_t n_units, const int32_t* dkv_splits, int32_t n_splits, float* dkv_ws,
                                    void* stream) {
  return attn_bwd<false>(q, k, v, out, dout, lse, delta, dq, dk, dv, subtree_end, run_ptr, runs, ktile_qend, Tq, Tk, q_offset, Hq, Hkv, head_dim,
                         q_st, q_sh, kv_st, kv_sh, v_st, v_sh, o_st, o_sh, dq_st, dq_sh, dkv_st, dkv_sh, scale, dtype, accumulate, which,
                         dkv_units, n_units, dkv_splits, n_splits, dkv_ws, nullptr, 0, stream);
}

static int window_args(const int32_t* subtree_end, const int32_t* win_lo, int32_t window) {
  if (window <= 0) return win_lo ? DTA_EINVAL : 0;
  if (subtree_end && !win_lo) return DTA_EINVAL;
  return 1;
}

extern "C" int dta_tree_attn_fwd_win(const void* q, const void* k, const void* v, void* out, float* lse,
                                    const int32_t* subtree_end, const int32_t* run_ptr, const int32_t* runs,
                                    int32_t Tq, int32_t Tk, int32_t q_offset, int32_t Hq, int32_t Hkv, int32_t head_dim,
                                    int64_t q_st, int64_t q_sh, int64_t kv_st, int64_t kv_sh, int64_t v_st, int64_t v_sh, int64_t o_st, int64_t o_sh,
                                    float scale, int32_t dtype, const int32_t* win_lo, int32_t window, void* stream) {
  const int w = window_args(subtree_end, win_lo, window);
  if (w < 0) return w;
  if (w == 0) return dta_tree_attn_fwd_ex(q, k, v, out, lse, subtree_end, run_ptr, runs, Tq, Tk, q_offset, Hq, Hkv, head_dim, q_st, q_sh, kv_st, kv_sh,
                                          v_st, v_sh, o_st, o_sh, scale, dtype, stream);
  return attn_fwd<true>(q, k, v, out, lse, subtree_end, run_ptr, runs, Tq, Tk, q_offset, Hq, Hkv, head_dim, q_st, q_sh, kv_st, kv_sh, v_st, v_sh,
                        o_st, o_sh, scale, dtype, win_lo, window, stream);
}

extern "C" int dta_tree_attn_bwd_win(const void* q, const void* k, const void* v, const void* out, const void* dout,
                                    const float* lse, float* delta, void* dq, void* dk, void* dv,
                                    const int32_t* subtree_end, const int32_t* run_ptr, const int32_t* runs,
                                    const int32_t* ktile_qend,
                                    int32_t Tq, int32_t Tk, int32_t q_offset, int32_t Hq, int32_t Hkv, int32_t head_dim,
                                    int64_t q_st, int64_t q_sh, int64_t kv_st, int64_t kv_sh, int64_t v_st, int64_t v_sh, int64_t o_st, int64_t o_sh,
                                    int64_t dq_st, int64_t dq_sh, int64_t dkv_st, int64_t dkv_sh,
                                    float scale, int32_t dtype, int32_t accumulate, int32_t which,
                                    const int32_t* dkv_units, int32_t n_units, const int32_t* dkv_splits, int32_t n_splits, float* dkv_ws,
                                    const int32_t* win_lo, int32_t window, void* stream) {
  const int w = window_args(subtree_end, win_lo, window);
  if (w < 0) return w;
  if (w == 0) return dta_tree_attn_bwd_ex(q, k, v, out, dout, lse, delta, dq, dk, dv, subtree_end, run_ptr, runs, ktile_qend, Tq, Tk, q_offset, Hq, Hkv,
                                          head_dim, q_st, q_sh, kv_st, kv_sh, v_st, v_sh, o_st, o_sh, dq_st, dq_sh, dkv_st, dkv_sh, scale, dtype,
                                          accumulate, which, dkv_units, n_units, dkv_splits, n_splits, dkv_ws, stream);
  return attn_bwd<true>(q, k, v, out, dout, lse, delta, dq, dk, dv, subtree_end, run_ptr, runs, ktile_qend, Tq, Tk, q_offset, Hq, Hkv, head_dim,
                        q_st, q_sh, kv_st, kv_sh, v_st, v_sh, o_st, o_sh, dq_st, dq_sh, dkv_st, dkv_sh, scale, dtype, accumulate, which,
                        dkv_units, n_units, dkv_splits, n_splits, dkv_ws, win_lo, window, stream);
}

extern "C" int dta_tree_attn_fwd(const void* q, const void* k, const void* v, void* out, float* lse,
                                 const int32_t* subtree_end, const int32_t* run_ptr, const int32_t* runs,
                                 int32_t Tq, int32_t Tk, int32_t q_offset, int32_t Hq, int32_t Hkv, int32_t head_dim,
                                 int64_t q_stride_t, int64_t kv_stride_t, int64_t o_stride_t,
                                 float scale, int32_t dtype, void* stream) {
  return dta_tree_attn_fwd_ex(q, k, v, out, lse, subtree_end, run_ptr, runs, Tq, Tk, q_offset, Hq, Hkv, head_dim == 128 ? 128 : 0,
                              q_stride_t, 128, kv_stride_t, 128, kv_stride_t, 128, o_stride_t, 128, scale, dtype, stream);
}

extern "C" int dta_tree_attn_bwd(const void* q, const void* k, const void* v, const void* out, const void* dout,
                                 const float* lse, float* delta, void* dq, void* dk, void* dv,
                                 const int32_t* subtree_end, const int32_t* run_ptr, const int32_t* runs,
                                 const int32_t* ktile_qend,
                                 int32_t Tq, int32_t Tk, int32_t q_offset, int32_t Hq, int32_t Hkv, int32_t head_dim,
                                 int64_t q_stride_t, int64_t kv_stride_t, int64_t o_stride_t,
                                 int64_t dq_stride_t, int64_t dkv_stride_t,
                                 float scale, int32_t dtype, int32_t accumulate, void* stream) {
  return dta_tree_attn_bwd_ex(q, k, v, out, dout, lse, delta, dq, dk, dv, subtree_end, run_ptr, runs, ktile_qend,
                              Tq, Tk, q_offset, Hq, Hkv, head_dim == 128 ? 128 : 0, q_stride_t, 128, kv_stride_t, 128, kv_stride_t, 128, o_stride_t, 128,
                              dq_stride_t, 128, dkv_stride_t, 128, scale, dtype, accumulate, 3, nullptr, 0, nullptr, 0, nullptr, stream);
}
```

### dynamictreeattn_amd/ops.py

```python
from __future__ import annotations

import math
from dataclasses import dataclass
from typing import Optional

import numpy as np
import torch
import torch.nn.functional as F

from . import packing
from ._lib import check, lib, ptr

_DT = {torch.bfloat16: 0, torch.float16: 1, torch.float32: 2}
_DT_LOGITS = _DT


class _on:
    __slots__ = ("dev", "_guard")

    def __init__(self, *ts):
        dev = None
        for t in ts:
            if t is None:
                continue
            if not t.is_cuda:
                raise RuntimeError("dynamictreeattn_amd ops run on the MI355X only (tensor is on %s); there is no CPU path" % t.device)
            if dev is None:
                dev = t.device
            elif t.device != dev:
                raise RuntimeError(f"operands of one dynamictreeattn_amd op live on different devices ({dev} and {t.device})")
        if dev is None:
            raise RuntimeError("dynamictreeattn_amd op called without a device tensor")
        self.dev, self._guard = dev, None

    def __enter__(self):
        if torch.cuda.current_device() != self.dev.index:
            self._guard = torch.cuda.device(self.dev)
            self._guard.__enter__()
        return torch.cuda.current_stream(self.dev).cuda_stream

    def __exit__(self, *exc):
        if self._guard is not None:
            self._guard.__exit__(*exc)
        return False


class KernelTimer:
    active: Optional["KernelTimer"] = None

    def __init__(self):
        from collections import defaultdict
        self.spans = defaultdict(list)
        for k in ("fwd", "bwd_dq", "bwd_dkv", "bwd_dkv_finalize"):
            self.spans[k]

    def span(self, name, nbytes: int = 0):
        a, b = torch.cuda.Event(enable_timing=True), torch.cuda.Event(enable_timing=True)
        self.spans[name].append((a, b, nbytes))
        return a, b

    def totals_ms(self):
        torch.cuda.synchronize()
        return {k: (sum(s[0].elapsed_time(s[1]) for s in v), len(v)) for k, v in self.spans.items()}

    def totals_bytes(self):
        return {k: sum(s[2] for s in v) for k, v in self.spans.items()}


def _require_cuda(*ts):
    _on(*ts)


def free_hbm(device) -> int:
    free, total = torch.cuda.mem_get_info(device)
    alloc, reserved = torch.cuda.memory_allocated(device), torch.cuda.memory_reserved(device)
    usable = free + reserved - alloc
    frac = torch.cuda.get_per_process_memory_fraction(device)
    if frac < 1.0:
        usable = min(usable, int(frac * total) - alloc)
    return max(int(usable), 0)


def _launch(name: str, tensors, *args, nbytes: int = 0, span: Optional[str] = None):
    tm = KernelTimer.active
    with _on(*tensors) as stream:
        if tm is not None:
            a, b = tm.span(span or name, nbytes); a.record()
        st = getattr(lib(), name)(*args, stream)
        if tm is not None:
            b.record()
    check(st, name)


@dataclass
class TreeAttnMeta:
    T: int
    subtree_end: Optional[torch.Tensor]
    run_ptr: Optional[torch.Tensor]
    runs: Optional[torch.Tensor]
    ktile_qend: Optional[torch.Tensor]
    q_offset: int = 0
    dkv_units: Optional[torch.Tensor] = None
    dkv_splits: Optional[torch.Tensor] = None
    n_slabs: int = 0
    win_lo: Optional[torch.Tensor] = None
    window: int = 0


def ktile_qend_from(subtree_end: torch.Tensor, tile: int = packing.KTILE) -> torch.Tensor:
    T = subtree_end.numel()
    nkt = (T + tile - 1) // tile
    pad = nkt * tile - T
    se = torch.nn.functional.pad(subtree_end, (0, pad), value=0) if pad else subtree_end
    return se.view(nkt, tile).amax(dim=1).to(torch.int32).contiguous()


def _strides(t):
    if t.stride(-1) != 1:
        raise ValueError("head_dim must be contiguous")
    return t.stride(0), t.stride(1)


def attn_fwd_raw(q, k, v, meta: TreeAttnMeta, scale: float):
    _require_cuda(q, k, v)
    Tq, Hq, D = q.shape
    Tk, Hkv, _ = k.shape
    out = torch.empty((Tq, Hq, D), dtype=q.dtype, device=q.device)
    lse = torch.empty((Hq, Tq), dtype=torch.float32, device=q.device)
    (qs, qh), (ks, kh), (vs, vh), (os_, oh) = _strides(q), _strides(k), _strides(v), _strides(out)
    tm = KernelTimer.active
    win = (ptr(meta.win_lo), int(meta.window)) if meta.window > 0 else ()
    with _on(q, k, v, meta.subtree_end, meta.runs) as stream:
        if tm is not None:
            ev = tm.span("fwd"); ev[0].record()
        st = getattr(lib(), "dta_tree_attn_fwd_win" if win else "dta_tree_attn_fwd_ex")(
            ptr(q), ptr(k), ptr(v), ptr(out), ptr(lse), ptr(meta.subtree_end), ptr(meta.run_ptr), ptr(meta.runs),
            Tq, Tk, meta.q_offset, Hq, Hkv, D, qs, qh, ks, kh, vs, vh, os_, oh, float(scale), _DT[q.dtype], *win, stream)
        if tm is not None:
            ev[1].record()
    check(st, "dta_tree_attn_fwd")
    return out, lse, k, v


def attn_bwd_raw(q, k, v, out, dout, lse, meta: TreeAttnMeta, scale: float, dk=None, dv=None, accumulate=False, dq=None):
    Tq, Hq, D = q.shape
    Tk, Hkv, _ = k.shape
    if dout.stride() != out.stride():
        dout = dout.contiguous(); out = out.contiguous()
    if dq is None:
        dq = torch.empty((Tq, Hq, D), dtype=q.dtype, device=q.device)
    if dk is None:
        dk = torch.empty((Tk, Hkv, D), dtype=q.dtype, device=q.device); dv = torch.empty_like(dk)
    delta = torch.empty((Hq, Tq), dtype=torch.float32, device=q.device)
    (qs, qh), (ks, kh), (vs, vh), (os_, oh), (dqs, dqh), (dks, dkh) = _strides(q), _strides(k), _strides(v), _strides(out), _strides(dq), _strides(dk)
    units, splits = meta.dkv_units, meta.dkv_splits
    n_units = units.shape[0] if units is not None else 0
    n_splits = splits.shape[0] if splits is not None else 0
    if q.dtype == torch.float32:
        units = splits = None; n_units = n_splits = 0
    ws = torch.empty((meta.n_slabs, Hkv, 2, packing.KTILE, D), dtype=torch.float32, device=q.device) if (units is not None and meta.n_slabs) else None

    win = (ptr(meta.win_lo), int(meta.window)) if meta.window > 0 else ()

    def launch(which, stream):
        return getattr(lib(), "dta_tree_attn_bwd_win" if win else "dta_tree_attn_bwd_ex")(
            ptr(q), ptr(k), ptr(v), ptr(out), ptr(dout), ptr(lse), ptr(delta), ptr(dq), ptr(dk), ptr(dv),
            ptr(meta.subtree_end), ptr(meta.run_ptr), ptr(meta.runs), ptr(meta.ktile_qend),
            Tq, Tk, meta.q_offset, Hq, Hkv, D, qs, qh, ks, kh, vs, vh, os_, oh, dqs, dqh, dks, dkh,
            float(scale), _DT[q.dtype], int(accumulate), which,
            ptr(units), n_units, ptr(splits) if n_splits else None, n_splits, ptr(ws), *win, stream)
    tm = KernelTimer.active
    with _on(q, k, v, out, dout, lse, dk, dv, meta.subtree_end, units, meta.win_lo) as stream:
        if tm is None:
            check(launch(3, stream), "dta_tree_attn_bwd")
        else:
            for which, name in ((1, "bwd_dq"), (2 | 8, "bwd_dkv"), (4, "bwd_dkv_finalize")):
                if which == 4 and not n_splits:
                    continue
                a, b = tm.span(name); a.record(); st = launch(which, stream); b.record()
                check(st, "dta_tree_attn_bwd")
    return dq, dk, dv


class AttentionTape:
    current = None

    def __init__(self, mode: str, items=None):
        assert mode in ("record", "replay")
        self.mode, self.items, self.pos = mode, ([] if items is None else items), 0

    def __enter__(self):
        self._prev, AttentionTape.current = AttentionTape.current, self
        return self

    def __exit__(self, *exc):
        AttentionTape.current = self._prev
        return False


class _TreeAttention(torch.autograd.Function):
    @staticmethod
    def forward(ctx, q, k, v, meta: TreeAttnMeta, scale: float):
        tape = AttentionTape.current
        if tape is not None and tape.mode == "replay" and tape.pos < len(tape.items):
            out, lse = tape.items[tape.pos]; tape.pos += 1
            if out.shape != q.shape:
                raise RuntimeError("attention replay: recorded output does not match the recomputed query")
        else:
            out, lse, k, v = attn_fwd_raw(q, k, v, meta, scale)
            if tape is not None and tape.mode == "record":
                tape.items.append((out, lse))
        ctx.save_for_backward(q, k, v, out, lse)
        ctx.meta, ctx.scale = meta, scale
        return out

    @staticmethod
    def backward(ctx, dout):
        q, k, v, out, lse = ctx.saved_tensors
        Hq, Hkv = q.shape[1], k.shape[1]
        if q.shape[0] == k.shape[0]:
            fused = torch.empty((q.shape[0], Hq + 2 * Hkv, q.shape[2]), dtype=q.dtype, device=q.device)
            dq, dk, dv = fused[:, :Hq], fused[:, Hq:Hq + Hkv], fused[:, Hq + Hkv:]
            attn_bwd_raw(q, k, v, out, dout, lse, ctx.meta, ctx.scale, dk=dk, dv=dv, dq=dq)
        else:
            dq, dk, dv = attn_bwd_raw(q, k, v, out, dout, lse, ctx.meta, ctx.scale)
        return dq, dk, dv, None, None


class _StackAttention(torch.autograd.Function):

    @staticmethod
    def forward(ctx, q, k_new, v_new, kst, vst, gk, gv, start, scale, window):
        B = q.shape[0]
        end = start + B
        kst[start:end].copy_(k_new); vst[start:end].copy_(v_new)
        meta = stack_meta(start, window)
        out, lse, _, _ = attn_fwd_raw(q, kst[:end], vst[:end], meta, scale)
        ctx.save_for_backward(q, out, lse)
        ctx.stacks, ctx.meta, ctx.scale, ctx.span = (kst, vst, gk, gv), meta, scale, (start, end)
        return out

    @staticmethod
    def backward(ctx, dout):
        q, out, lse = ctx.saved_tensors
        kst, vst, gk, gv = ctx.stacks
        start, end = ctx.span
        dq, _, _ = attn_bwd_raw(q, kst[:end], vst[:end], out, dout, lse, ctx.meta, ctx.scale, dk=gk[:end], dv=gv[:end], accumulate=2)
        return dq, gk[start:end].to(q.dtype), gv[start:end].to(q.dtype), None, None, None, None, None, None, None


def stack_attention(q, k_new, v_new, kst, vst, gk, gv, start: int, scale: Optional[float] = None, window: int = 0):
    if q.dtype not in _DT:
        raise TypeError("stack_attention supports bf16 / f16 / f32 (got %s)" % q.dtype)
    scale = q.shape[-1] ** -0.5 if scale is None else scale
    return _StackAttention.apply(q, k_new, v_new, kst, vst, gk, gv, start, scale, int(window))


def tree_attention(q: torch.Tensor, k: torch.Tensor, v: torch.Tensor, meta: TreeAttnMeta, scale: Optional[float] = None) -> torch.Tensor:
    if q.dtype not in _DT:
        raise TypeError("tree_attention supports bf16 / f16 / f32 (got %s)" % q.dtype)
    scale = q.shape[-1] ** -0.5 if scale is None else scale
    return _TreeAttention.apply(q, k, v, meta, scale)


def stack_meta(start: int, window: int = 0) -> TreeAttnMeta:
    return TreeAttnMeta(T=0, subtree_end=None, run_ptr=None, runs=None, ktile_qend=None, q_offset=start, window=max(int(window), 0))


def attach_dkv_units(meta: TreeAttnMeta, Hkv: int) -> TreeAttnMeta:
    kq = meta.ktile_qend.cpu().numpy()
    units, splits, n_slabs = packing.plan_dkv_units(kq, meta.T, meta.T, meta.q_offset, Hkv)
    dev = meta.ktile_qend.device
    meta.dkv_units = torch.from_numpy(units).to(dev).contiguous()
    meta.dkv_splits = torch.from_numpy(splits).to(dev).contiguous() if splits.shape[0] else None
    meta.n_slabs = n_slabs
    return meta


def meta_from_plan(plan: packing.SegmentPlan, subtree_end: torch.Tensor, device, Hkv: int = 8) -> TreeAttnMeta:
    rp, runs = packing.plan_qtile_runs(plan)
    meta = TreeAttnMeta(T=plan.T, subtree_end=subtree_end,
                        run_ptr=torch.from_numpy(rp).to(device), runs=torch.from_numpy(runs).to(device).contiguous(),
                        ktile_qend=ktile_qend_from(subtree_end))
    return attach_dkv_units(meta, Hkv)


def window_lo_device(depth: torch.Tensor, seg_off: torch.Tensor, seg_depth0: torch.Tensor, parent_of_seg: torch.Tensor,
                     window: int) -> torch.Tensor:
    T, M = depth.numel(), parent_of_seg.numel()
    out = torch.empty(T, dtype=torch.int32, device=depth.device)
    _launch("dta_window_lo", (depth,), ptr(depth), ptr(seg_off), ptr(seg_depth0), ptr(parent_of_seg), M, T, int(window), ptr(out))
    return out


def window_meta(meta: TreeAttnMeta, plan: packing.SegmentPlan, depth: torch.Tensor, window: int, Hkv: int = 8, seg_tables=None) -> TreeAttnMeta:
    if window <= 0 or window > packing.max_depth(plan):
        return meta
    dev = depth.device
    up = lambda a: torch.from_numpy(np.ascontiguousarray(a, np.int32)).to(dev)
    if seg_tables is None:
        seg_tables = (up(plan.seg_off), up(plan.seg_depth0), up(plan.parent_of_seg))
    win_lo = window_lo_device(depth, *seg_tables, window)
    wl_host = packing.window_lo_host(plan, window)
    rp, runs = packing.plan_qtile_runs_window(plan, wl_host)
    kq = packing.ktile_qend_window(packing.ktile_qend_host(plan), wl_host)
    units, splits, n_slabs = packing.plan_dkv_units(kq, plan.T, plan.T, 0, Hkv)
    return TreeAttnMeta(T=plan.T, subtree_end=meta.subtree_end, run_ptr=up(rp), runs=up(runs).view(-1, 4), ktile_qend=up(kq),
                        dkv_units=up(units).view(-1, 4), dkv_splits=up(splits).view(-1, 4) if splits.shape[0] else None, n_slabs=n_slabs,
                        win_lo=win_lo, window=int(window))


def logprob_entropy_fwd_raw(logits, labels, want_entropy=True, temperature=1.0, extra_ptr=None, extra_labels=None, extra_out=None):
    R, V = logits.shape
    lse = torch.empty(R, dtype=torch.float32, device=logits.device)
    ent = torch.empty_like(lse) if want_entropy else None
    lp = torch.empty_like(lse) if labels is not None else None
    _launch("dta_logprob_entropy_fwd", (logits, labels, extra_ptr, extra_labels, extra_out),
            ptr(logits), ptr(labels), ptr(extra_ptr), ptr(extra_labels), ptr(lse), ptr(ent), ptr(lp), ptr(extra_out),
            R, V, logits.stride(0), float(temperature), _DT_LOGITS[logits.dtype], nbytes=R * V * logits.element_size())
    return lse, ent, lp


def logprob_entropy_bwd_raw(logits, labels, lse, ent, g_lp, g_ent, temperature=1.0, extra_ptr=None, extra_labels=None, g_extra=None, out=None):
    R, V = logits.shape
    out = logits if out is None else out
    _launch("dta_logprob_entropy_bwd", (logits, out, labels, extra_ptr, extra_labels, lse, g_lp, g_extra, g_ent),
            ptr(logits), ptr(out), ptr(labels), ptr(extra_ptr), ptr(extra_labels), ptr(lse), ptr(ent), ptr(g_lp), ptr(g_extra), ptr(g_ent),
            R, V, logits.stride(0), out.stride(0), float(temperature), _DT_LOGITS[logits.dtype], nbytes=2 * R * V * logits.element_size())
    return out


def logprob_entropy_shard_stats_raw(logits, labels_local, temperature=1.0, extra_ptr=None, extra_labels=None, extra_out=None):
    R, V = logits.shape
    stats = torch.empty((R, 4), dtype=torch.float32, device=logits.device)
    _launch("dta_logprob_entropy_shard_stats", (logits, labels_local, extra_ptr, extra_labels, extra_out),
            ptr(logits), ptr(labels_local), ptr(extra_ptr), ptr(extra_labels), ptr(stats), ptr(extra_out),
            R, V, logits.stride(0), float(temperature), _DT_LOGITS[logits.dtype], nbytes=R * V * logits.element_size())
    return stats


_LN2 = 0.6931471805599453


def combine_shard_stats(stats, extra_sum, group):
    import torch.distributed as dist
    m = stats[:, 0].contiguous()
    M = m.clone()
    dist.all_reduce(M, op=dist.ReduceOp.MAX, group=group)
    f = torch.exp2(m - M)
    R = stats.shape[0]
    packed = torch.cat([stats[:, 1] * f, stats[:, 2] * f, stats[:, 3], extra_sum])
    dist.all_reduce(packed, op=dist.ReduceOp.SUM, group=group)
    S, Tt, picked, extra = packed[:R], packed[R:2 * R], packed[2 * R:3 * R], packed[3 * R:]
    lse = (M + torch.log2(S)) * _LN2
    ent = lse - (Tt / S) * _LN2
    return lse, ent, picked, extra


def local_labels(t, vocab_offset, V):
    return torch.where((t >= vocab_offset) & (t < vocab_offset + V), t - vocab_offset, torch.full_like(t, -1))


HEAD_WGRAD_FUSED_ACCUMULATE = False


class _HeadRows(torch.autograd.Function):

    @staticmethod
    def forward(ctx, h, W, next_tok, fork_ptr, fork_tok, fork_rows, fork_bounds, want_entropy, chunk, keep_bytes, tp_group, vocab_offset):
        T = h.shape[0]
        dev = h.device
        V = W.shape[0]
        F_ = fork_tok.numel()
        keep = T * V * h.element_size() <= keep_bytes
        step = T if keep else chunk
        lse = torch.empty(T, dtype=torch.float32, device=dev)
        ent = torch.empty(T, dtype=torch.float32, device=dev) if (want_entropy or tp_group is not None) else None
        lp_next = torch.empty(T, dtype=torch.float32, device=dev)
        lp_fork = torch.empty(F_, dtype=torch.float32, device=dev)
        if tp_group is not None:
            next_loc, fork_loc = local_labels(next_tok, vocab_offset, V), local_labels(fork_tok, vocab_offset, V)
        else:
            next_loc, fork_loc = next_tok, fork_tok
        xp = fork_ptr if F_ else None
        kept = None
        for ci, a in enumerate(range(0, T, step)):
            b = min(a + step, T)
            logits = torch.mm(h[a:b], W.t())
            if tp_group is None:
                l, e, p = logprob_entropy_fwd_raw(logits, next_loc[a:b], want_entropy, 1.0,
                                                  xp[a:b + 1] if F_ else None, fork_loc if F_ else None, lp_fork if F_ else None)
            else:
                f0, f1 = (0, F_) if keep else (fork_bounds[ci], fork_bounds[ci + 1])
                stats = logprob_entropy_shard_stats_raw(logits, next_loc[a:b], 1.0, xp[a:b + 1] if F_ else None, fork_loc if F_ else None,
                                                        lp_fork if F_ else None)
                l, e, picked, raw = combine_shard_stats(stats, lp_fork[f0:f1], tp_group)
                p = picked - l
                if f1 > f0:
                    lp_fork[f0:f1] = raw - l[fork_rows[f0:f1] - a]
            lse[a:b] = l; lp_next[a:b] = p
            if ent is not None:
                ent[a:b] = e
            if keep:
                kept = logits
        ctx.save_for_backward(h, W, next_loc, fork_loc, lse, ent if ent is not None else lse, xp if F_ else lse)
        ctx.kept, ctx.chunk, ctx.want_entropy, ctx.tp_group, ctx.has_forks = kept, chunk, want_entropy, tp_group, bool(F_)
        return lp_next, lp_fork, (ent if want_entropy else lse.new_zeros(0))

    @staticmethod
    def backward(ctx, g_next, g_fork, g_ent):
        h, W, next_loc, fork_loc, lse, ent, xp = ctx.saved_tensors
        T = h.shape[0]
        g_next = g_next.contiguous().float()
        g_ent = g_ent.contiguous().float() if ctx.want_entropy else None
        g_fork = g_fork.contiguous().float() if ctx.has_forks else None
        kept = ctx.kept
        step = T if kept is not None else ctx.chunk
        dh = torch.empty_like(h)
        need_w = ctx.needs_input_grad[1]
        dW = None if (kept is not None or not need_w) else torch.zeros(W.shape, dtype=torch.float32, device=W.device)
        pending = []
        for a in range(0, T, step):
            b = min(a + step, T)
            logits = kept if kept is not None else torch.mm(h[a:b], W.t())
            logprob_entropy_bwd_raw(logits, next_loc[a:b], lse[a:b], ent[a:b] if ctx.want_entropy else None, g_next[a:b],
                                    g_ent[a:b] if ctx.want_entropy else None, 1.0,
                                    xp[a:b + 1] if ctx.has_forks else None, fork_loc if ctx.has_forks else None, g_fork)
            if W.dtype in (torch.bfloat16, torch.float16) and (b - a) >= 4096 and W.shape[0] % 8 == 0 and W.shape[1] % 8 == 0:
                torch.mm(logits, _TransposedWeights.get(W).t(), out=dh[a:b])
            else:
                torch.mm(logits, W, out=dh[a:b])
            if ctx.tp_group is not None:
                import torch.distributed as dist
                pending.append(dist.all_reduce(dh[a:b], op=dist.ReduceOp.SUM, group=ctx.tp_group, async_op=True))
            if not need_w:
                pass
            elif kept is not None:
                dW = torch.mm(logits.t(), h)
            elif HEAD_WGRAD_FUSED_ACCUMULATE:
                dW = torch.addmm(dW, logits.t(), h[a:b], out_dtype=torch.float32)
            else:
                dW += torch.mm(logits.t(), h[a:b])
        ctx.kept = None
        for w in pending:
            w.wait()
        return dh, (dW.to(W.dtype) if need_w else None), None, None, None, None, None, None, None, None, None, None


def lm_head_rows(h, W, next_tok, fork_ptr, fork_tok, fork_rows, fork_bounds, want_entropy, chunk, keep_bytes=None, tp_group=None, vocab_offset=0):
    _require_cuda(h, W)
    if keep_bytes is None:
        keep_bytes = free_hbm(h.device) // 4
    if tp_group is not None:
        import torch.distributed as dist
        ok = torch.tensor([1 if h.shape[0] * W.shape[0] * h.element_size() <= keep_bytes else 0], device=h.device, dtype=torch.int32)
        dist.all_reduce(ok, op=dist.ReduceOp.MIN, group=tp_group)
        keep_bytes = (1 << 62) if int(ok.item()) else 0
    lp_next, lp_fork, ent = _HeadRows.apply(h, W, next_tok, fork_ptr, fork_tok, fork_rows, fork_bounds, want_entropy, chunk, keep_bytes,
                                            tp_group, vocab_offset)
    return lp_next, lp_fork, (ent if want_entropy else None)


class _LogProbEntropyHIP(torch.autograd.Function):

    @staticmethod
    def forward(ctx, logits, labels, temperature, want_entropy):
        lse, ent, lp = logprob_entropy_fwd_raw(logits, labels, want_entropy, temperature)
        ctx.save_for_backward(logits, labels, lse, ent if ent is not None else lse)
        ctx.temperature, ctx.want_entropy = temperature, want_entropy
        return lp, (ent if want_entropy else lse.new_zeros(0))

    @staticmethod
    def backward(ctx, g_lp, g_ent):
        logits, labels, lse, ent = ctx.saved_tensors
        out = torch.empty_strided(logits.shape, logits.stride(), dtype=logits.dtype, device=logits.device)
        logprob_entropy_bwd_raw(logits, labels, lse, ent if ctx.want_entropy else None, g_lp.contiguous().float(),
                                g_ent.contiguous().float() if ctx.want_entropy else None, ctx.temperature, out=out)
        return out, None, None, None


class _ShardedLogProbEntropyHIP(torch.autograd.Function):

    @staticmethod
    def forward(ctx, logits, labels_local, temperature, want_entropy, group):
        stats = logprob_entropy_shard_stats_raw(logits, labels_local, temperature)
        lse, ent, picked, _ = combine_shard_stats(stats, stats.new_zeros(0), group)
        ctx.save_for_backward(logits, labels_local, lse, ent)
        ctx.temperature, ctx.want_entropy = temperature, want_entropy
        return picked - lse, (ent if want_entropy else lse.new_zeros(0))

    @staticmethod
    def backward(ctx, g_lp, g_ent):
        logits, labels_local, lse, ent = ctx.saved_tensors
        out = torch.empty_strided(logits.shape, logits.stride(), dtype=logits.dtype, device=logits.device)
        logprob_entropy_bwd_raw(logits, labels_local, lse, ent if ctx.want_entropy else None, g_lp.contiguous().float(),
                                g_ent.contiguous().float() if ctx.want_entropy else None, ctx.temperature, out=out)
        return out, None, None, None, None


def _rows_for_kernel(logits2d):
    if logits2d.stride(-1) != 1:
        logits2d = logits2d.contiguous()
    if logits2d.stride(0) % 8 or logits2d.data_ptr() % 32:
        R, V = logits2d.shape
        buf = torch.empty((R, (V + 7) // 8 * 8), dtype=logits2d.dtype, device=logits2d.device)
        view = buf[:, :V]
        view.copy_(logits2d)
        return view
    return logits2d


def logprob_entropy(logits2d, labels1d, temperature=1.0, want_entropy=True, tp_group=None):
    if logits2d.dtype not in _DT_LOGITS:
        raise TypeError("logprob_entropy supports bf16 / f16 / f32 logits (got %s)" % logits2d.dtype)
    x = _rows_for_kernel(logits2d)
    if tp_group is None:
        lp, ent = _LogProbEntropyHIP.apply(x, labels1d, float(temperature), want_entropy)
    else:
        import torch.distributed as dist
        V = x.shape[1]
        lab = local_labels(labels1d, dist.get_rank(tp_group) * V, V)
        lp, ent = _ShardedLogProbEntropyHIP.apply(x, lab, float(temperature), want_entropy, tp_group)
    return lp, (ent if want_entropy else None)


class _RMSNorm(torch.autograd.Function):

    @staticmethod
    def forward(ctx, x, delta, w, eps):
        _require_cuda(x, w)
        x2 = x.contiguous().view(-1, x.shape[-1])
        R, H = x2.shape
        y = torch.empty_like(x2)
        rstd = torch.empty(R, dtype=torch.float32, device=x.device)
        if delta is not None:
            d2 = delta.contiguous().view(R, H)
            xo = torch.empty_like(x2)
        else:
            d2, xo = None, None
        _launch("dta_rmsnorm_fwd", (x2, d2, w), ptr(x2), ptr(d2), ptr(w), ptr(xo), ptr(y), ptr(rstd), R, H, float(eps), _DT[x.dtype],
                nbytes=R * H * x2.element_size() * (4 if delta is not None else 2))
        xin = xo if xo is not None else x2
        ctx.save_for_backward(xin, w, rstd)
        ctx.has_delta = delta is not None
        return xin.view(x.shape), y.view(x.shape)

    @staticmethod
    def backward(ctx, g_res, dy):
        x2, w, rstd = ctx.saved_tensors
        R, H = x2.shape
        dy2 = dy.contiguous().view(R, H)
        gr = g_res.contiguous().view(R, H) if g_res is not None else None
        dx = torch.empty_like(x2)
        need_w = ctx.needs_input_grad[2]
        part = torch.empty(lib().dta_rmsnorm_bwd_blocks(R), H, dtype=torch.float32, device=x2.device) if need_w else None
        _launch("dta_rmsnorm_bwd", (x2, w, dy2, gr), ptr(x2), ptr(w), ptr(dy2), ptr(gr), ptr(rstd), ptr(dx), ptr(part), R, H, _DT[x2.dtype],
                nbytes=R * H * x2.element_size() * (4 if gr is not None else 3))
        dx = dx.view(dy.shape)
        return dx, (dx if ctx.has_delta else None), (sum_slabs(part, w.dtype) if need_w else None), None


def rms_norm(x: torch.Tensor, w: torch.Tensor, eps: float) -> torch.Tensor:
    return _RMSNorm.apply(x, None, w, eps)[1]


def add_rms_norm(x: torch.Tensor, delta: Optional[torch.Tensor], w: torch.Tensor, eps: float):
    return _RMSNorm.apply(x, delta, w, eps)


class _QKNormRope(torch.autograd.Function):
    @staticmethod
    def forward(ctx, x, w, cos_sin, eps):
        _require_cuda(x, cos_sin)
        T, NH, D = x.shape
        if x.stride(2) != 1 or x.stride(1) != D:
            x = x.contiguous()
        y = torch.empty((T, NH, D), dtype=x.dtype, device=x.device)
        rstd = torch.empty(T * NH, dtype=torch.float32, device=x.device) if w is not None else None
        _launch("dta_qk_norm_rope_fwd", (x, w, cos_sin), ptr(x), ptr(w), ptr(cos_sin), ptr(y), ptr(rstd), T, NH, D, x.stride(0), float(eps),
                _DT[x.dtype], nbytes=2 * T * NH * D * x.element_size() + T * D * 4)
        ctx.save_for_backward(x, w if w is not None else cos_sin, cos_sin, rstd if rstd is not None else cos_sin)
        ctx.has_w = w is not None
        return y

    @staticmethod
    def backward(ctx, dy):
        x, w, cos_sin, rstd = ctx.saved_tensors
        T, NH, D = x.shape
        if dy.stride(2) != 1:
            dy = dy.contiguous()
        dx = torch.empty((T, NH, D), dtype=x.dtype, device=x.device)
        part = None
        if ctx.has_w and ctx.needs_input_grad[1]:
            part = torch.empty(lib().dta_qk_norm_rope_bwd_blocks(T * NH), D, dtype=torch.float32, device=x.device)
        _launch("dta_qk_norm_rope_bwd", (x, cos_sin, dy), ptr(x), ptr(w) if ctx.has_w else None, ptr(cos_sin), ptr(dy), ptr(rstd) if ctx.has_w else None,
                ptr(dx), ptr(part), T, NH, D, x.stride(0), dy.stride(0), dy.stride(1), dx.stride(0), _DT[x.dtype],
                nbytes=(3 if ctx.has_w else 2) * T * NH * D * x.element_size() + T * D * 4)
        return dx, (sum_slabs(part, w.dtype) if part is not None else None), None, None


class _QKVPrep(torch.autograd.Function):

    @staticmethod
    def forward(ctx, qkv, wq, wk, cos_sin, eps, Hq, Hkv):
        _require_cuda(qkv, cos_sin)
        T, H3, D = qkv.shape
        assert H3 == Hq + 2 * Hkv and qkv.is_contiguous()
        outs, rstds = [], []
        for x, w, NH in ((qkv[:, :Hq], wq, Hq), (qkv[:, Hq:Hq + Hkv], wk, Hkv)):
            y = torch.empty((T, NH, D), dtype=qkv.dtype, device=qkv.device)
            rstd = torch.empty(T * NH, dtype=torch.float32, device=qkv.device) if w is not None else None
            _launch("dta_qk_norm_rope_fwd", (qkv, w, cos_sin), ptr(x), ptr(w), ptr(cos_sin), ptr(y), ptr(rstd), T, NH, D, qkv.stride(0), float(eps),
                    _DT[qkv.dtype], nbytes=2 * T * NH * D * qkv.element_size() + T * D * 4)
            outs.append(y); rstds.append(rstd if rstd is not None else cos_sin)
        ctx.save_for_backward(qkv, wq if wq is not None else cos_sin, wk if wk is not None else cos_sin, cos_sin, rstds[0], rstds[1])
        ctx.has_w = (wq is not None, wk is not None)
        ctx.heads = (Hq, Hkv)
        return outs[0], outs[1], qkv[:, Hq + Hkv:]

    @staticmethod
    def backward(ctx, dq, dk, dv):
        qkv, wq, wk, cos_sin, rq, rk = ctx.saved_tensors
        Hq, Hkv = ctx.heads
        T, H3, D = qkv.shape
        base = dv._base
        in_place = (base is not None and dq._base is base and dk._base is base and base.shape == qkv.shape and base.is_contiguous()
                    and base.dtype == qkv.dtype and dq.shape == (T, Hq, D) and dk.shape == (T, Hkv, D) and dv.shape == (T, Hkv, D)
                    and dq.stride() == dk.stride() == dv.stride() == (H3 * D, D, 1)
                    and (dq.storage_offset(), dk.storage_offset(), dv.storage_offset()) == (0, Hq * D, (Hq + Hkv) * D))
        d = base if in_place else torch.empty_like(qkv)
        dws = []
        for lo, NH, w, rstd, has_w, need_w, dy in ((0, Hq, wq, rq, ctx.has_w[0], ctx.needs_input_grad[1], dq),
                                                   (Hq, Hkv, wk, rk, ctx.has_w[1], ctx.needs_input_grad[2], dk)):
            if dy.stride(2) != 1:
                dy = dy.contiguous()
            part = torch.empty(lib().dta_qk_norm_rope_bwd_blocks(T * NH), D, dtype=torch.float32, device=qkv.device) if has_w and need_w else None
            _launch("dta_qk_norm_rope_bwd", (qkv, cos_sin, dy), ptr(qkv[:, lo:lo + NH]), ptr(w) if has_w else None, ptr(cos_sin), ptr(dy),
                    ptr(rstd) if has_w else None, ptr(d[:, lo:lo + NH]), ptr(part), T, NH, D, qkv.stride(0), dy.stride(0), dy.stride(1), d.stride(0),
                    _DT[qkv.dtype], nbytes=(3 if has_w else 2) * T * NH * D * qkv.element_size() + T * D * 4)
            dws.append(sum_slabs(part, w.dtype) if part is not None else None)
        if not in_place:
            d[:, Hq + Hkv:].copy_(dv)
        return d, dws[0], dws[1], None, None, None, None


def qkv_prep(qkv: torch.Tensor, wq: Optional[torch.Tensor], wk: Optional[torch.Tensor], cos_sin: torch.Tensor, eps: float,
             Hq: int, Hkv: int):
    return _QKVPrep.apply(qkv, wq, wk, cos_sin, eps, Hq, Hkv)


def qk_norm_rope(x: torch.Tensor, w: Optional[torch.Tensor], cos_sin: torch.Tensor, eps: float) -> torch.Tensor:
    return _QKNormRope.apply(x, w, cos_sin, eps)


ROPE_TYPES = ("default", "linear", "llama3", "yarn")


def rope_inv_freq(D: int, rope_parameters: dict, max_position_embeddings: Optional[int] = None):
    rp = rope_parameters
    kind = rp.get("rope_type", rp.get("type")) or "default"
    if kind not in ROPE_TYPES:
        raise ValueError(f"rope_parameters: rope_type {kind!r} is not supported ({' / '.join(ROPE_TYPES)})")
    base = float(rp["rope_theta"])
    steps = torch.arange(0, D, 2, dtype=torch.int64).to(torch.float32)
    if kind == "default":
        return 1.0 / (base ** (steps / D)), 1.0
    if kind == "linear":
        inv = 1.0 / (base ** (steps / D))
        inv /= rp["factor"]
        return inv, 1.0
    orig = rp.get("original_max_position_embeddings") or max_position_embeddings
    if orig is None:
        raise ValueError(f"rope_parameters: rope_type {kind!r} needs original_max_position_embeddings (or max_position_embeddings)")
    if kind == "llama3":
        inv = 1.0 / (base ** (steps / D))
        factor, low_f, high_f = rp["factor"], rp["low_freq_factor"], rp["high_freq_factor"]
        low_wavelen, high_wavelen = orig / low_f, orig / high_f
        wavelen = 2 * math.pi / inv
        scaled = torch.where(wavelen > low_wavelen, inv / factor, inv)
        smooth = (orig / wavelen - low_f) / (high_f - low_f)
        smoothed = (1 - smooth) * scaled / factor + smooth * scaled
        medium = ~(wavelen < high_wavelen) * ~(wavelen > low_wavelen)
        return torch.where(medium, smoothed, scaled), 1.0
    factor = rp.get("factor")
    if factor is None:
        if max_position_embeddings is None:
            raise ValueError("rope_parameters: yarn needs factor (or max_position_embeddings)")
        factor = max_position_embeddings / orig
    mscale_of = lambda scale, m=1: 1.0 if scale <= 1 else 0.1 * m * math.log(scale) + 1.0
    att = rp.get("attention_factor")
    if att is None:
        ms, ms_all = rp.get("mscale"), rp.get("mscale_all_dim")
        att = float(mscale_of(factor, ms) / mscale_of(factor, ms_all)) if ms and ms_all else mscale_of(factor)
    beta_fast, beta_slow = rp.get("beta_fast") or 32, rp.get("beta_slow") or 1
    corr_dim = lambda rot: (D * math.log(orig / (rot * 2 * math.pi))) / (2 * math.log(base))
    low, high = corr_dim(beta_fast), corr_dim(beta_slow)
    if rp.get("truncate", True):
        low, high = math.floor(low), math.ceil(high)
    low, high = max(low, 0), min(high, D - 1)
    if low == high:
        high += 0.001
    pos_freqs = base ** (steps / D)
    extrapolation, interpolation = 1.0 / pos_freqs, 1.0 / (factor * pos_freqs)
    keep = 1 - torch.clamp((torch.arange(D // 2, dtype=torch.float32) - low) / (high - low), 0, 1)
    return interpolation * (1 - keep) + extrapolation * keep, att


_INV_FREQ: dict = {}


def rope_cos_sin(depth: torch.Tensor, D: int, rope) -> torch.Tensor:
    if isinstance(rope, (int, float)):
        key, host, factor = (D, float(rope), depth.device), None, 1.0
    else:
        host, factor = rope
        if host.shape != (D // 2,) or host.dtype != torch.float32 or host.device.type != "cpu":
            raise ValueError(f"rope_cos_sin: inv_freq must be a host fp32 [{D // 2}] tensor, got {host.dtype} {tuple(host.shape)} on {host.device}")
        key = (D, host.numpy().tobytes(), depth.device)
    inv = _INV_FREQ.get(key)
    if inv is None:
        if host is None:
            host = rope_inv_freq(D, {"rope_theta": float(rope)})[0]
        inv = host.to(depth.device)
        _INV_FREQ[key] = inv
    ang = depth.float()[:, None] * inv[None, :]
    table = torch.cat([ang.cos(), ang.sin()], dim=-1)
    if float(factor) != 1.0:
        table = table * float(factor)
    return table.contiguous()


class _SwiGLU(torch.autograd.Function):

    @staticmethod
    def forward(ctx, gu, g, u):
        if gu is not None:
            _require_cuda(gu)
            gu = gu if gu.stride(-1) == 1 and gu.dim() == 2 else gu.contiguous().view(-1, gu.shape[-1])
            C = gu.shape[1] // 2
            g, u, ld = gu[:, :C], gu[:, C:], gu.stride(0)
        else:
            _require_cuda(g, u)
            g = g.contiguous().view(-1, g.shape[-1]); u = u.contiguous().view(-1, u.shape[-1])
            C, ld = g.shape[1], g.shape[1]
        rows = g.shape[0]
        y = torch.empty((rows, C), dtype=g.dtype, device=g.device)
        _launch("dta_swiglu_fwd", (g, u), ptr(g), ptr(u), ptr(y), rows, C, ld, _DT[g.dtype], nbytes=3 * rows * C * g.element_size())
        ctx.save_for_backward(g, u)
        ctx.fused, ctx.ld = gu is not None, ld
        return y

    @staticmethod
    def backward(ctx, dy):
        g, u = ctx.saved_tensors
        rows, C = g.shape
        dy = dy.contiguous()
        if ctx.fused:
            dgu = torch.empty((rows, 2 * C), dtype=g.dtype, device=g.device)
            dg, du, ldg = dgu[:, :C], dgu[:, C:], 2 * C
        else:
            dg, du, ldg = torch.empty_like(g), torch.empty_like(u), C
        _launch("dta_swiglu_bwd", (g, u, dy), ptr(g), ptr(u), ptr(dy), ptr(dg), ptr(du), rows, C, ctx.ld, ldg, _DT[g.dtype],
                nbytes=5 * rows * C * g.element_size())
        return (dgu, None, None) if ctx.fused else (None, dg, du)


def swiglu(g: torch.Tensor, u: torch.Tensor) -> torch.Tensor:
    return _SwiGLU.apply(None, g, u)


def swiglu_fused(gu: torch.Tensor) -> torch.Tensor:
    return _SwiGLU.apply(gu, None, None)


class weight_cache:
    depth = 0

    def __enter__(self):
        weight_cache.depth += 1
        return self

    def __exit__(self, *exc):
        weight_cache.depth -= 1
        if weight_cache.depth == 0:
            clear_weight_caches()
        return False


class _StackRows(torch.autograd.Function):

    CACHE_BYTES = 8 << 30
    _cache: dict = {}
    _cached_bytes = 0

    @staticmethod
    def _fused(ws):
        rows = [w.shape[0] for w in ws]
        key = tuple((id(w), w.data_ptr(), w._version) for w in ws)
        if weight_cache.depth > 0:
            hit = _StackRows._cache.get(key)
            if hit is not None:
                return hit
        out = torch.empty((sum(rows),) + tuple(ws[0].shape[1:]), dtype=ws[0].dtype, device=ws[0].device)
        o = 0
        for w, r in zip(ws, rows):
            out[o:o + r].copy_(w); o += r
        nbytes = out.numel() * out.element_size()
        if weight_cache.depth > 0 and _StackRows._cached_bytes + nbytes <= _StackRows.CACHE_BYTES:
            _StackRows._cache[key] = out; _StackRows._cached_bytes += nbytes
        return out

    @staticmethod
    def forward(ctx, *ws):
        ctx.rows = [w.shape[0] for w in ws]
        return _StackRows._fused(ws).detach()

    @staticmethod
    def backward(ctx, g):
        outs, o = [], 0
        for r in ctx.rows:
            outs.append(g[o:o + r]); o += r
        return tuple(outs)


def stack_rows(*ws: torch.Tensor) -> torch.Tensor:
    return _StackRows.apply(*ws)


def clear_stack_rows_cache() -> None:
    _StackRows._cache.clear(); _StackRows._cached_bytes = 0


def sum_slabs(part: torch.Tensor, out_dtype: torch.dtype, extra: torch.Tensor = None) -> torch.Tensor:
    assert part.dtype == torch.float32 and part.is_contiguous() and (extra is None or (extra.dtype == torch.float32 and extra.is_contiguous()))
    S, n = part.shape[0], part[0].numel()
    assert extra is None or extra.numel() == n
    out = torch.empty(part.shape[1:], dtype=out_dtype, device=part.device)
    _launch("dta_sum_slabs", (part, extra, out), ptr(part), S, n, n, ptr(extra), ptr(out), _DT[out_dtype], nbytes=(S + (extra is not None)) * n * 4)
    return out


def transpose_2d(w: torch.Tensor) -> torch.Tensor:
    R, C = w.shape
    if w.stride(1) != 1:
        w = w.contiguous()
    out = torch.empty((C, R), dtype=w.dtype, device=w.device)
    _launch("dta_transpose", (w, out), ptr(w), ptr(out), R, C, w.stride(0), R, w.element_size(), nbytes=2 * R * C * w.element_size())
    return out


class _TransposedWeights:
    cache: dict = {}
    nbytes = 0

    @staticmethod
    def get(w: torch.Tensor) -> torch.Tensor:
        if weight_cache.depth == 0:
            return transpose_2d(w)
        key = (w.data_ptr(), tuple(w.shape), w.dtype, w._version)
        hit = _TransposedWeights.cache.get(key)
        if hit is not None:
            return hit
        wt = transpose_2d(w)
        n = wt.numel() * wt.element_size()
        if _TransposedWeights.nbytes + n <= _StackRows.CACHE_BYTES:
            _TransposedWeights.cache[key] = wt; _TransposedWeights.nbytes += n
        return wt


def clear_weight_caches() -> None:
    clear_stack_rows_cache()
    _TransposedWeights.cache.clear(); _TransposedWeights.nbytes = 0


def _dgrad(dy: torch.Tensor, w: torch.Tensor) -> torch.Tensor:
    if dy.is_cuda and w.dtype in (torch.bfloat16, torch.float16) and dy.shape[0] >= 4096 and w.shape[0] % 8 == 0 and w.shape[1] % 8 == 0:
        return dy @ _TransposedWeights.get(w).t()
    return dy @ w


WGRAD_SPLIT_K = 4


def _wgrad(x: torch.Tensor, dy: torch.Tensor, transposed: bool) -> torch.Tensor:
    T = x.shape[0]
    a, b = (x, dy) if transposed else (dy, x)
    S = WGRAD_SPLIT_K
    tiles = -(-a.shape[1] // 256) * -(-b.shape[1] // 256)
    per = (T // S) // 64 * 64
    if tiles > 64 or per < 2048 or not x.is_cuda or x.dtype == torch.float32:
        out = a.t() @ b
    else:
        body = per * S
        part = torch.bmm(a[:body].reshape(S, per, a.shape[1]).transpose(1, 2), b[:body].reshape(S, per, b.shape[1]), out_dtype=torch.float32)
        rest = torch.mm(a[body:].t(), b[body:], out_dtype=torch.float32) if body < T else None
        out = sum_slabs(part, x.dtype, rest)
    if not transposed:
        return out
    V = 16 // out.element_size()
    return transpose_2d(out) if out.is_cuda and out.shape[0] % V == 0 and out.shape[1] % V == 0 else out.t()


class _Linear(torch.autograd.Function):

    @staticmethod
    def forward(ctx, x, w, b):
        ctx.save_for_backward(x, w)
        ctx.has_bias = b is not None
        return F.linear(x, w, b)

    @staticmethod
    def backward(ctx, dy):
        x, w = ctx.saved_tensors
        dx = _dgrad(dy, w) if ctx.needs_input_grad[0] else None
        dw = None
        if ctx.needs_input_grad[1]:
            dw = _wgrad(x, dy, w.shape[1] >= 2 * w.shape[0])
        db = dy.sum(0) if ctx.has_bias and ctx.needs_input_grad[2] else None
        return dx, dw, db


def linear(x: torch.Tensor, w: torch.Tensor, b: Optional[torch.Tensor] = None) -> torch.Tensor:
    return _Linear.apply(x, w, b)


MOE_FWD, MOE_DGRAD, MOE_WGRAD = 0, 1, 2


@dataclass
class MoeRouting:
    T: int
    k: int
    E: int
    expert_offsets: torch.Tensor
    row_of_pair: torch.Tensor
    src_token: torch.Tensor
    tiles: torch.Tensor


def moe_router_fwd_raw(logits: torch.Tensor, k: int, norm: bool):
    T, E_ = logits.shape
    logits = logits.contiguous()
    ids = torch.empty((T, k), dtype=torch.int32, device=logits.device)
    w = torch.empty((T, k), dtype=logits.dtype, device=logits.device)
    lse = torch.empty(T, dtype=torch.float32, device=logits.device)
    _launch("dta_moe_router_fwd", (logits,), ptr(logits), ptr(ids), ptr(w), ptr(lse), T, E_, k, int(bool(norm)), _DT[logits.dtype],
            nbytes=T * E_ * logits.element_size())
    return ids, w, lse


def moe_router_bwd_raw(logits, lse, ids, dw, norm: bool):
    T, E_ = logits.shape
    dw = dw.contiguous().to(logits.dtype)
    dl = torch.empty_like(logits)
    _launch("dta_moe_router_bwd", (logits, dw), ptr(logits), ptr(lse), ptr(ids), ptr(dw), ptr(dl), T, E_, ids.shape[1], int(bool(norm)),
            _DT[logits.dtype], nbytes=2 * T * E_ * logits.element_size())
    return dl


def moe_permute(ids: torch.Tensor, E_: int) -> MoeRouting:
    T, k = ids.shape
    P = T * k
    L = lib()
    dev = ids.device
    ws = torch.empty(max(int(L.dta_moe_permute_workspace(P, E_)), 1), dtype=torch.int32, device=dev)
    bound = int(L.dta_moe_tile_bound(P, E_))
    offs = torch.empty(E_ + 1, dtype=torch.int32, device=dev)
    rop = torch.empty(max(P, 1), dtype=torch.int32, device=dev)
    src = torch.empty(max(P, 1), dtype=torch.int32, device=dev)
    tiles = torch.empty(2 * bound, dtype=torch.int32, device=dev)
    ids = ids.contiguous()
    _launch("dta_moe_permute", (ids,), ptr(ids), T, k, E_, ptr(ws), ptr(offs), ptr(rop), ptr(src), ptr(tiles), nbytes=12 * P)
    return MoeRouting(T, k, E_, offs, rop[:P], src[:P], tiles)


def moe_grouped_gemm(mode: int, route: MoeRouting, w_shape, out_dtype, x=None, w=None, dy=None, gather: bool = False) -> torch.Tensor:
    E_, N, K = w_shape
    R = route.T * route.k
    ref = x if x is not None else dy
    shape = (R, N) if mode == MOE_FWD else (R, K) if mode == MOE_DGRAD else (E_, N, K)
    out = torch.empty(shape, dtype=out_dtype, device=ref.device)
    if R == 0 and mode != MOE_WGRAD:
        return out
    x, w, dy = (None if t is None else t.contiguous() for t in (x, w, dy))
    esz = out.element_size()
    _launch("dta_moe_grouped_gemm", tuple(t for t in (x, w, dy) if t is not None), mode, ptr(x), ptr(w), ptr(dy), ptr(out),
            ptr(route.src_token) if gather else None, ptr(route.expert_offsets), ptr(route.tiles), R, E_, N, K, _DT[out_dtype],
            nbytes=esz * (R * N + R * K + E_ * N * K), span=f"moe_gemm_{('fwd', 'dgrad', 'wgrad')[mode]}_{N}x{K}")
    return out


def moe_combine_fwd_raw(y, w, route: MoeRouting):
    H = y.shape[1]
    out = torch.empty((route.T, H), dtype=y.dtype, device=y.device)
    _launch("dta_moe_combine_fwd", (y,), ptr(y), ptr(w), ptr(route.row_of_pair), ptr(out), route.T, route.k, H, _DT[y.dtype],
            nbytes=(route.k + 1) * route.T * H * y.element_size())
    return out


def moe_combine_bwd_raw(dout, y, w, route: MoeRouting):
    H = y.shape[1]
    dout = dout.contiguous()
    dy = torch.empty_like(y)
    dw = torch.empty_like(w)
    _launch("dta_moe_combine_bwd", (dout, y, w), ptr(dout), ptr(y), ptr(w), ptr(route.row_of_pair), ptr(dy), ptr(dw), route.T, route.k, H,
            _DT[y.dtype], nbytes=(3 * route.k + 1) * route.T * H * y.element_size())
    return dy, dw


class _MoeRouter(torch.autograd.Function):

    @staticmethod
    def forward(ctx, logits, k, norm):
        ids, w, lse = moe_router_fwd_raw(logits, k, norm)
        ctx.save_for_backward(logits, lse, ids)
        ctx.norm = norm
        ctx.mark_non_differentiable(ids)
        return w, ids

    @staticmethod
    def backward(ctx, dw, _dids):
        logits, lse, ids = ctx.saved_tensors
        return moe_router_bwd_raw(logits, lse, ids, dw, ctx.norm), None, None


class _MoeLinear(torch.autograd.Function):

    @staticmethod
    def forward(ctx, x, w, route, gather):
        ctx.save_for_backward(x, w)
        ctx.route, ctx.gather = route, gather
        return moe_grouped_gemm(MOE_FWD, route, w.shape, x.dtype, x=x, w=w, gather=gather)

    @staticmethod
    def backward(ctx, dy):
        x, w = ctx.saved_tensors
        route, gather = ctx.route, ctx.gather
        dy = dy.contiguous()
        dx = dw = None
        if ctx.needs_input_grad[0]:
            dxs = moe_grouped_gemm(MOE_DGRAD, route, w.shape, x.dtype, w=w, dy=dy)
            dx = moe_combine_fwd_raw(dxs, None, route) if gather else dxs
        if ctx.needs_input_grad[1]:
            dw = moe_grouped_gemm(MOE_WGRAD, route, w.shape, w.dtype, x=x, dy=dy, gather=gather)
        return dx, dw, None, None


class _MoeCombine(torch.autograd.Function):
    @staticmethod
    def forward(ctx, y, w, route):
        ctx.save_for_backward(y, w)
        ctx.route = route
        return moe_combine_fwd_raw(y, w, route)

    @staticmethod
    def backward(ctx, dout):
        y, w = ctx.saved_tensors
        dy, dw = moe_combine_bwd_raw(dout, y, w, ctx.route)
        return dy, dw, None


def moe_mlp(h: torch.Tensor, router_w: torch.Tensor, gate_up_w: torch.Tensor, down_w: torch.Tensor, top_k: int,
            norm_topk_prob: bool) -> torch.Tensor:
    if not h.is_cuda:
        raise RuntimeError("moe_mlp runs on the MI355X only; there is no CPU path")
    E_ = gate_up_w.shape[0]
    logits = linear(h, router_w)
    w, ids = _MoeRouter.apply(logits, int(top_k), bool(norm_topk_prob))
    route = moe_permute(ids, E_)
    gu = _MoeLinear.apply(h, gate_up_w, route, True)
    act = swiglu_fused(gu)
    y = _MoeLinear.apply(act, down_w, route, False)
    return _MoeCombine.apply(y, w, route)


def _host_f32(vals):
    return None if vals is None else np.ascontiguousarray(vals, np.float32)


def lora_down(x: torch.Tensor, m: torch.Tensor, rscale=None) -> torch.Tensor:
    T, K = x.shape
    R = m.shape[0]
    assert x.stride(1) == 1 and m.stride(1) == 1 and m.shape[1] == K and m.dtype == x.dtype
    out = torch.empty((T, R), dtype=x.dtype, device=x.device)
    rs = _host_f32(rscale)
    _launch("dta_lora_down", (x, m), ptr(x), x.stride(0), ptr(m), m.stride(0), ptr(out), R, None if rs is None else rs.ctypes.data,
            T, R, K, _DT[x.dtype], nbytes=(T * K + R * K + T * R) * x.element_size())
    return out


def lora_wgrad(l: torch.Tensor, x: torch.Tensor, out_dtype: torch.dtype, rscale=None) -> torch.Tensor:
    T, K = x.shape
    R = l.shape[1]
    assert l.shape[0] == T and l.stride(1) == 1 and x.stride(1) == 1 and l.dtype == x.dtype
    S = int(lib().dta_lora_wgrad_slabs(T, K))
    part = torch.empty((S, R, K), dtype=torch.float32, device=x.device)
    rs = _host_f32(rscale)
    _launch("dta_lora_wgrad", (l, x), ptr(l), l.stride(0), ptr(x), x.stride(0), ptr(part), None if rs is None else rs.ctypes.data,
            T, R, K, _DT[x.dtype], nbytes=(T * K + T * R) * x.element_size() + S * R * K * 4)
    return part[0] if (S == 1 and out_dtype == torch.float32) else sum_slabs(part, out_dtype)


WGRAD_KERNEL_MAX_K = 12288


def _down_by_kernel(K: int, R: int) -> bool:
    return K <= 1024 and R <= 32


def _wgrad_by_kernel(K: int) -> bool:
    return K <= WGRAD_KERNEL_MAX_K


def _lora_wgrad(l: torch.Tensor, x: torch.Tensor, out_dtype: torch.dtype, seg_scale=None) -> torch.Tensor:
    K = x.shape[1]
    if _wgrad_by_kernel(K):
        rs = None
        if seg_scale is not None:
            rs = np.ones(l.shape[1], np.float32)
            for r0, r, sc in seg_scale:
                rs[r0:r0 + r] = sc
        return lora_wgrad(l, x, out_dtype, rs)
    g = torch.mm(l.t(), x, out_dtype=torch.float32)
    for r0, r, sc in seg_scale or ():
        if sc != 1.0:
            g[r0:r0 + r] *= sc
    return g if out_dtype == torch.float32 else g.to(out_dtype)


class _LoraLinear(torch.autograd.Function):

    @staticmethod
    def forward(ctx, x, w, b, spec, *ab):
        dt = x.dtype
        As, Bs = ab[0::2], ab[1::2]
        y = F.linear(x, w, b)
        a_cat = torch.cat([a.to(dt) for a in As]) if len(As) > 1 else As[0].to(dt)
        if not a_cat.is_contiguous():
            a_cat = a_cat.contiguous()
        xa = lora_down(x, a_cat) if _down_by_kernel(x.shape[1], a_cat.shape[0]) else x @ a_cat.t()
        bs = [B_.to(dt) for B_ in Bs]
        r0 = 0
        for (n0, nlen, r, s), B_ in zip(spec, bs):
            y[:, n0:n0 + nlen].addmm_(xa[:, r0:r0 + r], B_.t(), alpha=s); r0 += r
        ctx.save_for_backward(x, w, xa, a_cat, *bs)
        ctx.spec, ctx.has_bias, ctx.ab_dtypes = spec, b is not None, [t.dtype for t in ab]
        return y

    @staticmethod
    def backward(ctx, dy):
        x, w, xa, a_cat = ctx.saved_tensors[:4]
        bs = ctx.saved_tensors[4:]
        spec, dt = ctx.spec, x.dtype
        dy = dy.contiguous()
        R, N = a_cat.shape[0], dy.shape[1]
        seg_scale, r0 = [], 0
        for n0, nlen, r, s in spec:
            seg_scale.append((r0, r, s)); r0 += r
        if _down_by_kernel(N, R):
            bd = torch.zeros((R, N), dtype=dt, device=x.device)
            rs = np.ones(R, np.float32)
            for (n0, nlen, r, s), (q0, _, _), B_ in zip(spec, seg_scale, bs):
                bd[q0:q0 + r, n0:n0 + nlen] = B_.t(); rs[q0:q0 + r] = s
            dxa = lora_down(dy, bd, rs)
        else:
            dxa = torch.empty((dy.shape[0], R), dtype=dt, device=x.device)
            for (n0, nlen, r, s), (q0, _, _), B_ in zip(spec, seg_scale, bs):
                torch.addmm(dxa[:, q0:q0 + r], dy[:, n0:n0 + nlen], B_, beta=0, alpha=s, out=dxa[:, q0:q0 + r])
        dx = None
        if ctx.needs_input_grad[0]:
            dx = _dgrad(dy, w)
            dx = dx.addmm_(dxa, a_cat) if dx.is_contiguous() else dx + dxa @ a_cat
        dw = _wgrad(x, dy, w.shape[1] >= 2 * w.shape[0]) if ctx.needs_input_grad[1] else None
        db = dy.sum(0) if ctx.has_bias and ctx.needs_input_grad[2] else None
        need = ctx.needs_input_grad[4:]
        g32 = lambda i: torch.float32 if ctx.ab_dtypes[i] == torch.float32 else dt
        dA = dB = None
        if any(need[0::2]):
            dA = _lora_wgrad(dxa, x, torch.float32 if any(ctx.ab_dtypes[i] == torch.float32 for i in range(0, len(need), 2)) else dt)
        if any(need[1::2]):
            dB = _lora_wgrad(xa, dy, torch.float32 if any(ctx.ab_dtypes[i] == torch.float32 for i in range(1, len(need), 2)) else dt, seg_scale)
        out, r0 = [], 0
        for i, (n0, nlen, r, _) in enumerate(spec):
            out.append(dA[r0:r0 + r].to(g32(2 * i)) if need[2 * i] else None)
            out.append(dB[r0:r0 + r, n0:n0 + nlen].t().to(g32(2 * i + 1)).contiguous() if need[2 * i + 1] else None)
            r0 += r
        return (dx, dw, db, None, *out)


def lora_linear(x: torch.Tensor, w: torch.Tensor, b: Optional[torch.Tensor], adapters) -> torch.Tensor:
    if not adapters:
        return linear(x, w, b)
    if x.is_cuda and x.dtype in (torch.bfloat16, torch.float16):
        spec = tuple((int(n0), int(nlen), int(A.shape[0]), float(s)) for n0, nlen, A, B_, s in adapters)
        ab = [t for _, _, A, B_, _ in adapters for t in (A, B_)]
        return _LoraLinear.apply(x, w, b, spec, *ab)
    y = linear(x, w, b)
    cols, o = [], 0
    for n0, nlen, A, B_, s in adapters:
        if n0 > o:
            cols.append(y[:, o:n0])
        cols.append(y[:, n0:n0 + nlen] + float(s) * ((x @ A.to(x.dtype).t()) @ B_.to(x.dtype).t()))
        o = n0 + nlen
    if o < y.shape[1]:
        cols.append(y[:, o:])
    return cols[0] if len(cols) == 1 else torch.cat(cols, dim=1)
```

### dynamictreeattn_amd/packing.py

```python
from __future__ import annotations

from dataclasses import dataclass
from typing import List, Sequence, Tuple

import numpy as np

QTILE = 128
KTILE = 128


@dataclass
class SegmentPlan:
    M: int
    T: int
    seg_off: np.ndarray
    seg_depth0: np.ndarray
    parent_of_seg: np.ndarray
    brk_ptr: np.ndarray
    brk_depth: np.ndarray
    brk_end: np.ndarray
    path_runs: List[List[Tuple[int, int]]]


def plan_segments(lens: Sequence[int], lcp_lens: Sequence[int]) -> SegmentPlan:
    M = len(lens)
    if len(lcp_lens) != M - 1:
        raise ValueError("lcp_lens must have len(lens)-1 entries")
    d0 = [0] + [int(c) for c in lcp_lens]
    seg_off = [0] * (M + 1)
    for i in range(M):
        if not (0 <= d0[i] <= lens[i]) or (i > 0 and d0[i] > lens[i - 1]):
            raise ValueError("lcp_lens inconsistent with lens")
        seg_off[i + 1] = seg_off[i] + (lens[i] - d0[i])
    T = seg_off[M]
    live: List[List[int]] = []
    brk: List[List[Tuple[int, int]]] = [[] for _ in range(M)]
    parent = [-1] * M
    path_runs: List[List[Tuple[int, int]]] = []
    for i in range(M):
        cut, here = d0[i], seg_off[i]
        while live and live[-1][1] >= cut:
            j, lo, _ = live.pop()
            brk[j].append((lo, here))
        if live and live[-1][2] > cut:
            live[-1][2] = cut
            brk[live[-1][0]].append((cut, here))
        runs = []
        for j, lo, hi in live:
            b, e = seg_off[j] + lo - d0[j], seg_off[j] + hi - d0[j]
            if runs and runs[-1][1] == b:
                runs[-1] = (runs[-1][0], e)
            else:
                runs.append((b, e))
        path_runs.append(runs)
        if cut > 0:
            j, lo, hi = live[-1]
            parent[i] = seg_off[j] + (cut - 1) - d0[j]
        if lens[i] > cut:
            live.append([i, cut, lens[i]])
    for j, lo, _ in live:
        brk[j].append((lo, T))
    ptr = [0]
    bd: List[int] = []
    be: List[int] = []
    for j in range(M):
        ent = brk[j][::-1]
        clean: List[Tuple[int, int]] = []
        for dep, end in ent:
            if clean and clean[-1][0] == dep:
                continue
            clean.append((dep, end))
        if not clean:
            clean = [(d0[j], seg_off[j])]
        bd += [c[0] for c in clean]; be += [c[1] for c in clean]
        ptr.append(len(bd))
    return SegmentPlan(M, T, np.asarray(seg_off, np.int32), np.asarray(d0, np.int32), np.asarray(parent, np.int32),
                       np.asarray(ptr, np.int32), np.asarray(bd, np.int32), np.asarray(be, np.int32), path_runs)


def pad_plan(plan: SegmentPlan, multiple: int = 256) -> SegmentPlan:
    pad = (-plan.T) % multiple
    if pad == 0:
        out = SegmentPlan(plan.M, plan.T, plan.seg_off, plan.seg_depth0, plan.parent_of_seg, plan.brk_ptr, plan.brk_depth,
                          plan.brk_end, plan.path_runs)
        out.n_real = plan.M
        return out
    T2 = plan.T + pad
    i32 = np.int32
    out = SegmentPlan(plan.M + 1, T2,
                      np.concatenate([plan.seg_off, np.asarray([T2], i32)]),
                      np.concatenate([plan.seg_depth0, np.asarray([0], i32)]),
                      np.concatenate([plan.parent_of_seg, np.asarray([-1], i32)]),
                      np.concatenate([plan.brk_ptr, np.asarray([plan.brk_ptr[-1] + 1], i32)]),
                      np.concatenate([plan.brk_depth, np.asarray([0], i32)]),
                      np.concatenate([plan.brk_end, np.asarray([T2], i32)]),
                      plan.path_runs + [[]])
    out.n_real = plan.M
    return out


def ktile_qend_host(plan: SegmentPlan, tile: int = KTILE) -> np.ndarray:
    T = plan.T
    nkt = (T + tile - 1) // tile
    out = np.zeros(nkt, np.int64)
    if T == 0:
        return out.astype(np.int32)
    seg = np.repeat(np.arange(plan.M, dtype=np.int64), np.diff(plan.brk_ptr))
    start = plan.seg_off[seg].astype(np.int64) + plan.brk_depth.astype(np.int64) - plan.seg_depth0[seg].astype(np.int64)
    nxt = np.empty_like(start)
    nxt[:-1] = start[1:]
    last_of_seg = plan.brk_ptr[1:].astype(np.int64) - 1
    nxt[last_of_seg] = plan.seg_off[1:].astype(np.int64)
    keep = nxt > start
    start, nxt, val = start[keep], nxt[keep], plan.brk_end.astype(np.int64)[keep]
    t0, t1 = start // tile, (nxt - 1) // tile
    np.maximum.at(out, t0, val)
    np.maximum.at(out, t1, val)
    inner = t1 - t0 - 1
    has = inner > 0
    if has.any():
        cnt = inner[has]
        first = (t0[has] + 1)
        idx = np.repeat(first - np.concatenate([[0], np.cumsum(cnt)[:-1]]), cnt) + np.arange(int(cnt.sum()))
        out[idx] = np.maximum(out[idx], np.repeat(val[has], cnt))
    return out.astype(np.int32)


def _merge(ivs):
    out = []
    for b, e in sorted(x for x in ivs if x[1] > x[0]):
        if out and b <= out[-1][1]:
            out[-1] = (out[-1][0], max(out[-1][1], e))
        else:
            out.append((b, e))
    return out


def _intersect(a, b):
    a, b = _merge(a), _merge(b)
    out, i, j = [], 0, 0
    while i < len(a) and j < len(b):
        lo, hi = max(a[i][0], b[j][0]), min(a[i][1], b[j][1])
        if hi > lo:
            out.append((lo, hi))
        if a[i][1] < b[j][1]:
            i += 1
        else:
            j += 1
    return out


def _subtract(a, b):
    out = []
    for lo, hi in a:
        cur = lo
        for b0, b1 in b:
            if b1 <= cur or b0 >= hi:
                continue
            if b0 > cur:
                out.append((cur, b0))
            cur = max(cur, b1)
        if cur < hi:
            out.append((cur, hi))
    return out


def plan_qtile_runs(plan: SegmentPlan, tile: int = QTILE):
    T = plan.T
    nqt = (T + tile - 1) // tile
    seg_off = plan.seg_off
    starts = np.arange(nqt, dtype=np.int64) * tile
    ends = np.minimum(starts + tile, T)
    first = np.searchsorted(seg_off, starts, side="right") - 1
    last = np.searchsorted(seg_off, ends - 1, side="right") - 1
    run_ptr = [0]
    out: List[Tuple[int, int, int, int]] = []
    for qt in range(nqt):
        q0, q1, i0, i1 = int(starts[qt]), int(ends[qt]), int(first[qt]), int(last[qt])
        if i0 == i1:
            for b, e in plan.path_runs[i0]:
                out.append((b, e, 0, 0))
            s = int(seg_off[i0])
            if s < q0:
                if out and len(out) > run_ptr[-1] and out[-1][1] == s and out[-1][2] == 0:
                    out[-1] = (out[-1][0], q0, 0, 0)
                else:
                    out.append((s, q0, 0, 0))
            out.append((q0, q1, 1, 0))
        else:
            common = None
            ivs = []
            for i in range(i0, i1 + 1):
                s, e = int(seg_off[i]), min(q1, int(seg_off[i + 1]))
                if e <= s:
                    continue
                anc = list(plan.path_runs[i])
                if s < q0:
                    anc.append((s, q0))
                common = anc if common is None else _intersect(common, anc)
                ivs.extend(plan.path_runs[i]); ivs.append((s, e))
            common = _merge([(b, min(e, q0)) for b, e in (common or []) if b < q0])
            for b, e in common:
                out.append((b, e, 0, 0))
            for b, e in _subtract(_merge(ivs), common):
                out.append((b, e, 1, 0))
        run_ptr.append(len(out))
    return np.asarray(run_ptr, np.int32), np.asarray(out, np.int32).reshape(-1, 4)


def plan_dkv_units(ktile_qend: np.ndarray, Tk: int, Tq: int, q_offset: int = 0, Hkv: int = 8, tile: int = KTILE,
                   waves_per_cu: int = 6, n_cu: int = 256, min_tiles: int = 8):
    nkt = ktile_qend.shape[0]
    k0 = np.arange(nkt, dtype=np.int64) * tile
    qbeg = np.maximum(k0, q_offset)
    qend = np.minimum(ktile_qend.astype(np.int64), q_offset + Tq)
    ntile = np.maximum(0, -(-(qend - qbeg) // 64))
    total = int(ntile.sum())
    target = max(1, (waves_per_cu * n_cu) // max(Hkv, 1))
    cap = max(min_tiles, -(-total // target))
    nsplit = np.maximum(1, -(-ntile // cap))
    per = -(-ntile // nsplit)
    kt_of = np.repeat(np.arange(nkt, dtype=np.int64), nsplit)
    first_unit = np.cumsum(nsplit) - nsplit
    j = np.arange(kt_of.shape[0], dtype=np.int64) - first_unit[kt_of]
    ub = qbeg[kt_of] + j * per[kt_of] * 64
    ue = np.minimum(qend[kt_of], ub + per[kt_of] * 64)
    is_split = nsplit[kt_of] > 1
    slab = np.where(is_split, np.cumsum(is_split) - 1, -1)
    units = np.stack([kt_of, ub, np.maximum(ue, ub), slab], axis=1)
    order = np.argsort(-(units[:, 2] - units[:, 1]), kind="stable")
    split_kt = np.flatnonzero(nsplit > 1)
    first_slab = (np.cumsum(np.where(nsplit > 1, nsplit, 0)) - np.where(nsplit > 1, nsplit, 0))[split_kt]
    splits = np.stack([split_kt, first_slab, nsplit[split_kt], np.zeros_like(split_kt)], axis=1) if split_kt.size else np.zeros((0, 4), np.int64)
    return units[order].astype(np.int32), splits.astype(np.int32), int(is_split.sum())



def window_lo_host(plan: SegmentPlan, window: int) -> np.ndarray:
    if window <= 0:
        raise ValueError("window must be > 0")
    T, M = plan.T, plan.M
    seg_off = plan.seg_off.astype(np.int64)
    d0 = plan.seg_depth0.astype(np.int64)
    seg = np.repeat(np.arange(M, dtype=np.int64), np.diff(seg_off))
    t = np.arange(T, dtype=np.int64)
    depth = d0[seg] + t - seg_off[seg]
    a = np.maximum(depth - window + 1, 0)
    i = seg.copy()
    need = np.flatnonzero(a < d0[i])
    par = plan.parent_of_seg.astype(np.int64)
    while need.size:
        i[need] = seg[par[i[need]]]
        need = need[a[need] < d0[i[need]]]
    return (seg_off[i] + a - d0[i]).astype(np.int32)


def max_depth(plan: SegmentPlan) -> int:
    n = np.diff(plan.seg_off.astype(np.int64))
    live = n > 0
    return int((plan.seg_depth0[live] + n[live] - 1).max()) if live.any() else -1


def _clip(ivs, lo):
    return [(max(b, lo), e) for b, e in ivs if e > max(b, lo)]


def plan_qtile_runs_window(plan: SegmentPlan, win_lo: np.ndarray, tile: int = QTILE):
    T = plan.T
    nqt = (T + tile - 1) // tile
    seg_off = plan.seg_off
    starts = np.arange(nqt, dtype=np.int64) * tile
    ends = np.minimum(starts + tile, T)
    first = np.searchsorted(seg_off, starts, side="right") - 1
    last = np.searchsorted(seg_off, ends - 1, side="right") - 1
    wl = np.asarray(win_lo, np.int64)
    run_ptr = [0]
    out: List[Tuple[int, int, int, int]] = []
    for qt in range(nqt):
        q0, q1, i0, i1 = int(starts[qt]), int(ends[qt]), int(first[qt]), int(last[qt])
        lo_min, lo_max = int(wl[q0:q1].min()), int(wl[q0:q1].max())
        if i0 == i1:
            full = []
            for b, e in plan.path_runs[i0]:
                full.append((b, e))
            s = int(seg_off[i0])
            if s < q0:
                if full and full[-1][1] == s:
                    full[-1] = (full[-1][0], q0)
                else:
                    full.append((s, q0))
            for b, e in full:
                b = max(b, lo_min)
                if b >= e:
                    continue
                if min(e, lo_max) > b:
                    out.append((b, min(e, lo_max), 1, 0))
                if e > max(b, lo_max):
                    out.append((max(b, lo_max), e, 0, 0))
            out.append((max(q0, lo_min), q1, 1, 0))
        else:
            common = None
            ivs = []
            for i in range(i0, i1 + 1):
                s, e = int(seg_off[i]), min(q1, int(seg_off[i + 1]))
                if e <= s:
                    continue
                lo_i = int(wl[max(s, q0):e].min())
                anc = list(plan.path_runs[i])
                if s < q0:
                    anc.append((s, q0))
                anc = _clip(anc, lo_i)
                common = anc if common is None else _intersect(common, anc)
                ivs.extend(_clip(list(plan.path_runs[i]) + [(s, e)], lo_i))
            common = _merge([(max(b, lo_max), min(e, q0)) for b, e in (common or []) if max(b, lo_max) < min(e, q0)])
            for b, e in common:
                out.append((b, e, 0, 0))
            for b, e in _subtract(_merge(ivs), common):
                out.append((b, e, 1, 0))
        run_ptr.append(len(out))
    return np.asarray(run_ptr, np.int32), np.asarray(out, np.int32).reshape(-1, 4)


def ktile_qend_window(ktile_qend: np.ndarray, win_lo: np.ndarray, tile: int = KTILE) -> np.ndarray:
    wl = np.asarray(win_lo, np.int64)
    T = wl.shape[0]
    nkt = ktile_qend.shape[0]
    if T == 0:
        return ktile_qend.astype(np.int32)
    sufmin = np.minimum.accumulate(wl[::-1])[::-1]
    kmax = np.minimum((np.arange(nkt, dtype=np.int64) + 1) * tile, T) - 1
    qe = np.searchsorted(sufmin, kmax, side="right")
    return np.minimum(ktile_qend.astype(np.int64), qe).astype(np.int32)
```

### dynamictreeattn_amd/tree_training_engine.py

```python
from __future__ import annotations

from typing import Callable, List, Optional

import numpy as np
import torch

from . import ops, packing
from .model import ensure_supported, head_weight, is_moe_layer, moe_geometry, packed_hidden_states
from .trie import pop_block_starts

__all__ = ["TreeTrainingEngine", "_get_forkpos", "packed_logprob_entropy"]


def _get_forkpos(lens, lcp_lens, block_size: Optional[int]) -> list:
    pos = {c - 1 for c in lcp_lens if c > 0}
    if block_size is not None:
        for i, end in enumerate(lens):
            start = lcp_lens[i] if i < len(lcp_lens) else 0
            pos.update(s - 1 for s in pop_block_starts(start, end, block_size) if s > 0)
    return sorted(pos)


def fork_tables_host(fork_child, fork_parent, T: int):
    fork_child, fork_parent = np.asarray(fork_child, np.int64), np.asarray(fork_parent, np.int64)
    order = np.argsort(fork_parent, kind="stable")
    fc, fp = fork_child[order], fork_parent[order]
    ptr = np.zeros(T + 1, np.int64)
    if fp.size:
        np.cumsum(np.bincount(fp, minlength=T), out=ptr[1:])
    return fc, fp, ptr


def packed_logprob_entropy(h: torch.Tensor, W: torch.Tensor, tokens: torch.Tensor, parent: torch.Tensor,
                           want_entropy: bool, chunk: int = 2048, fork_child: Optional[np.ndarray] = None,
                           fork_parent: Optional[np.ndarray] = None, tp_group=None, fork_dev=None):
    T = h.shape[0]
    dev = h.device
    if fork_child is None:
        fork_child = np.zeros(0, np.int64); fork_parent = np.zeros(0, np.int64)
    if fork_dev is None:
        fork_child, fork_parent, ptr = fork_tables_host(fork_child, fork_parent, T)
        fc_dev, fp_dev = torch.from_numpy(fork_child).to(dev), torch.from_numpy(fork_parent).to(dev)
        fork_ptr = torch.from_numpy(ptr.astype(np.int32)).to(dev) if fork_child.size else None
    else:
        fc_dev, fp_dev, fork_ptr = fork_dev
    nF = int(np.asarray(fork_child).size)
    ftok = tokens[fc_dev] if nF else tokens.new_zeros(0)
    if not nF:
        fork_ptr = None
    nxt = torch.cat([tokens[1:], tokens.new_zeros(1)])
    bounds = np.searchsorted(np.asarray(fork_parent), np.arange(0, T + chunk, chunk)).tolist()
    if tp_group is not None:
        import torch.distributed as dist
        tp, rk = dist.get_world_size(tp_group), dist.get_rank(tp_group)
        Vp = W.shape[0] // tp
        assert Vp * tp == W.shape[0], "vocabulary must divide by the tensor-parallel size"
        lp_next, lp_fork, ent = ops.lm_head_rows(h, W[rk * Vp:(rk + 1) * Vp], nxt, fork_ptr, ftok, fp_dev, bounds, want_entropy, chunk,
                                                 tp_group=tp_group, vocab_offset=rk * Vp)
    else:
        lp_next, lp_fork, ent = ops.lm_head_rows(h, W, nxt, fork_ptr, ftok, fp_dev, bounds, want_entropy, chunk)
    chain = torch.zeros(T, dtype=torch.bool, device=dev)
    chain[1:] = parent[1:] == torch.arange(0, T - 1, device=dev, dtype=parent.dtype)
    lp = torch.cat([lp_next.new_zeros(1), lp_next[:-1]]) * chain
    if nF:
        lp = lp.index_copy(0, fc_dev, lp_fork)
    return lp, ent


def sum_loss_terms(terms, device):
    if not terms:
        return None
    ts = [t if isinstance(t, torch.Tensor) else torch.as_tensor(float(t), dtype=torch.float32, device=device) for t in terms]
    return ts[0].reshape(()) if len(ts) == 1 else torch.stack([t.reshape(()).float() for t in ts]).sum()


class _PackedTrie:

    PAD_FROM = 2048
    PAD_TO = 256

    def __init__(self, trie, device, n_kv_heads: int = 8):
        device = torch.device(device)
        if device.type == "cuda" and device.index is None:
            device = torch.device("cuda", torch.cuda.current_device())
        if trie._dev.device != device:
            raise RuntimeError(f"TokenTrie holds its tokens on {trie._dev.device} but the engine runs on {device}: build it with "
                               f"TokenTrie(..., device={str(device)!r}) (or torch.cuda.set_device) so that one GPU owns the whole pass")
        plan = packing.plan_segments(trie.lens, trie.lcp_lens)
        self.n_real_tokens = plan.T
        M_real = plan.M
        leaf_off = [trie._dev.starts[s] for s in trie._leaf_src]
        if plan.T >= self.PAD_FROM and plan.T % self.PAD_TO:
            plan = packing.pad_plan(plan, self.PAD_TO)
            leaf_off = leaf_off + [0]
        self.plan = plan
        M, T = plan.M, plan.T
        run_ptr, runs = packing.plan_qtile_runs(plan)
        leaf_off = np.asarray(leaf_off, np.int64)
        kq = packing.ktile_qend_host(plan)
        units, splits, n_slabs = packing.plan_dkv_units(kq, T, T, 0, n_kv_heads)
        first = plan.seg_off[:-1].astype(np.int64)
        nonempty = np.diff(plan.seg_off) > 0
        par = plan.parent_of_seg.astype(np.int64)
        is_fork = nonempty & (par >= 0) & (par != first - 1)
        self.fork_child, self.fork_parent, fork_ptr = fork_tables_host(first[is_fork], par[is_fork], T)
        paths = []
        for i in range(M_real):
            pieces = [np.arange(b, e, dtype=np.int64) for b, e in plan.path_runs[i]]
            pieces.append(np.arange(plan.seg_off[i], plan.seg_off[i + 1], dtype=np.int64))
            paths.append(np.concatenate(pieces))
        self.path_sizes = [p.size for p in paths]
        self._paths_host = paths
        from ._staging import upload
        (seg_off, seg_d0, par_seg, brk_ptr, brk_depth, brk_end, run_ptr_d, runs_d, kq_d, units_d, splits_d, fptr_d) = upload(
            [plan.seg_off, plan.seg_depth0, plan.parent_of_seg, plan.brk_ptr, plan.brk_depth, plan.brk_end, run_ptr, runs.reshape(-1),
             kq, units.reshape(-1), splits.reshape(-1), fork_ptr], device, np.int32)
        leaf_off_d, self.path_cat, fc_d, fp_d = upload(
            [leaf_off, np.concatenate(paths) if paths else np.zeros(0, np.int64), self.fork_child, self.fork_parent], device, np.int64)
        self.fork_dev = (fc_d, fp_d, fptr_d)
        self.paths = list(torch.split(self.path_cat, self.path_sizes))
        self.tokens = torch.empty(T, dtype=torch.long, device=device)
        meta_i = torch.empty(3, T, dtype=torch.int32, device=device)
        self.depth, self.parent, self.subtree_end = meta_i[0], meta_i[1], meta_i[2]
        self._expand(trie._dev.tokens, leaf_off_d, seg_off, seg_d0, par_seg, brk_ptr, brk_depth, brk_end, M, T)
        self.meta = ops.TreeAttnMeta(T=T, subtree_end=self.subtree_end, run_ptr=run_ptr_d, runs=runs_d.view(-1, 4), ktile_qend=kq_d,
                                     dkv_units=units_d.view(-1, 4), dkv_splits=splits_d.view(-1, 4) if splits.shape[0] else None,
                                     n_slabs=n_slabs)
        self._seg_tables, self._n_kv_heads, self._win_metas = (seg_off, seg_d0, par_seg), n_kv_heads, {}

    def for_window(self, window: int):
        if window not in self._win_metas:
            self._win_metas[window] = ops.window_meta(self.meta, self.plan, self.depth, window, self._n_kv_heads, self._seg_tables)
        return self._win_metas[window]

    def sequence_rows(self, attach_lists):
        lp_rows, ent_rows = [], []
        for i, attach_list in enumerate(attach_lists):
            path = self._paths_host[i]
            for _, length in attach_list:
                lp_rows.append(path[1:length]); ent_rows.append(path[:length])
        from ._staging import upload
        empty = np.zeros(0, np.int64)
        return upload([np.concatenate(lp_rows) if lp_rows else empty, np.concatenate(ent_rows) if ent_rows else empty], self.tokens.device, np.int64)

    def _expand(self, tokens, leaf_off, seg_off, seg_d0, par_seg, brk_ptr, brk_depth, brk_end, M, T):
        from ._lib import check, lib, ptr
        with ops._on(tokens, leaf_off, seg_off, self.tokens) as stream:
            st = lib().dta_preorder_meta(ptr(tokens), ptr(leaf_off), ptr(seg_off), ptr(seg_d0), ptr(par_seg), ptr(brk_ptr), ptr(brk_depth),
                                         ptr(brk_end), M, T, ptr(self.tokens), ptr(self.depth), ptr(self.parent), ptr(self.subtree_end), stream)
        check(st, "dta_preorder_meta")


def _mlp_elems_per_token(c, l: int) -> float:
    if is_moe_layer(c, l):
        E, I, _ = moe_geometry(c)
        return c.num_experts_per_tok * (3 * I + c.hidden_size) + 2 * E
    return 4 * c.intermediate_size


def _has_moe(c) -> bool:
    return any(is_moe_layer(c, l) for l in range(c.num_hidden_layers))


def _stack_sink_fits(model, budget: int) -> bool:
    n = sum(p.numel() for p in model.parameters() if p.requires_grad)
    return n * 6 <= budget // 5


class TreeTrainingEngine:
    def __init__(self, model_config, device, dtype: torch.dtype, max_seq_len: int, forward_only: bool = False):
        if torch.device(device).type == "cuda" and dtype not in (torch.bfloat16, torch.float16, torch.float32):
            raise TypeError(f"TreeTrainingEngine supports dtype torch.bfloat16 / torch.float16 (MFMA kernels) and torch.float32 (the reference's "
                            f"--dtype fp32, run.py:122-132: plain-FMA attention kernels, a gradient-check path), got {dtype}")
        self.model = None
        self.device = torch.device(device)
        if self.device.type == "cuda" and self.device.index is None:
            self.device = torch.device("cuda", torch.cuda.current_device())
        self.dtype = dtype
        self.max_seq_len = max_seq_len
        self.forward_only = forward_only
        self.n_layers = model_config.num_hidden_layers
        self.n_kv_heads = getattr(model_config, "num_key_value_heads", 8)
        self.cur_len = 0
        self.forkpos_list: List[int] = []
        self._loss_host = None
        self.returns: List[Optional[torch.Tensor]] = []
        self.last_packed: Optional[_PackedTrie] = None
        self.head_chunk = 2048
        self.checkpoint_layers: Optional[bool] = None
        self.mode = "auto"
        self.memory_budget_bytes: Optional[int] = None
        self.last_mode: Optional[str] = None
        self.attn_keep_fraction = 0.25
        self.partial_recompute = True
        self.tp_group = None
        self._attn_keep_planned = 0
        self.stack_fp32_grads = True

    def _pack(self, token_trie) -> _PackedTrie:
        longest = max(token_trie.lens) if token_trie.lens else 0
        assert longest <= self.max_seq_len, (
            f"Exceeds max_seq_len: cur_len=0, new_tokens={longest}, max={self.max_seq_len}")
        p0 = next(iter(self.model.parameters()), None) if hasattr(self.model, "parameters") else None
        if p0 is not None and (p0.dtype != self.dtype or p0.device != self.device):
            raise RuntimeError(f"model parameters are {p0.dtype} on {p0.device}; this engine was built for {self.dtype} on {self.device}")
        packed = _PackedTrie(token_trie, self.device, self.n_kv_heads)
        self.last_packed = packed
        return packed

    def _should_checkpoint(self, model, T: int) -> bool:
        if self.checkpoint_layers is not None:
            return self.checkpoint_layers
        need = self._per_token_layer_bytes(model) * self.n_layers * T
        if self.device.type != "cuda":
            return False
        free = self._free_hbm()
        return need > 0.75 * free

    def _free_hbm(self) -> int:
        return ops.free_hbm(self.device)

    def _per_token_layer_bytes(self, model) -> int:
        c = model.config
        D = getattr(c, "head_dim", None) or c.hidden_size // c.num_attention_heads
        L = c.num_hidden_layers
        mlp = sum(_mlp_elems_per_token(c, l) for l in range(L)) / max(L, 1)
        from . import lora
        ranks = lora.rank_elems_per_token(model)
        return int(2 * (10 * c.hidden_size + mlp + ranks + 4 * (c.num_attention_heads + c.num_key_value_heads) * D))

    def _budget(self) -> Optional[int]:
        if self.memory_budget_bytes is not None:
            return int(self.memory_budget_bytes)
        if self.device.type != "cuda":
            return None
        free = self._free_hbm()
        return int(0.8 * free)

    def _stack_block_rows(self, model, T: int, block_size: Optional[int]) -> Optional[int]:
        if self.mode == "packed":
            return None
        budget = self._budget()
        per_layer = self._per_token_layer_bytes(model)
        c = model.config
        if self.mode != "stack":
            if budget is None:
                return None
            need = T * (2 * 2 * c.hidden_size * self.n_layers + 2 * per_layer)
            if need <= budget:
                return None
        if self.mode != "stack" and budget is not None and self.stack_fp32_grads and _has_moe(c) and not _stack_sink_fits(model, budget):
            return None
        bs = block_size or 2048
        if budget is None:
            return bs
        rows = int(0.5 * budget / max(per_layer * self.n_layers, 1)) // 256 * 256
        return int(max(bs, min(rows, 16384)))

    def _backward_stack(self, model, token_trie, loss_fn, block_rows: int) -> float:
        from . import dp
        from .stack_engine import StackWalk
        dp.defer_active_reducers()
        budget = self._budget()
        walk = StackWalk(model, token_trie, self.device, self.dtype, block_rows, self.head_chunk, self.tp_group,
                         grad_budget_bytes=0 if not self.stack_fp32_grads else (None if budget is None else budget // 5))
        total = walk.run(loss_fn)
        self.last_mode = f"stack[{block_rows}]x{walk.n_blocks}"
        self.cur_len = 0
        return float(total.item()) if total is not None else 0.0

    @staticmethod
    def packed_rows(n_tree_tokens: int) -> int:
        T = int(n_tree_tokens)
        if T >= _PackedTrie.PAD_FROM and T % _PackedTrie.PAD_TO:
            T += (-T) % _PackedTrie.PAD_TO
        return T

    def warm_gemm_shapes(self, model, row_counts) -> None:
        from types import SimpleNamespace
        body = model.model
        one = SimpleNamespace(config=model.config, model=SimpleNamespace(embed_tokens=body.embed_tokens, layers=[body.layers[0]], norm=body.norm))
        ident = lambda l: (lambda q, k, v: q)
        for T in sorted({int(t) for t in row_counts if t > 0}):
            tokens = torch.zeros(T, dtype=torch.long, device=self.device)
            depth = torch.arange(T, device=self.device, dtype=torch.int32) % 64
            parent = torch.arange(-1, T - 1, device=self.device, dtype=torch.int32)
            with torch.enable_grad():
                h = packed_hidden_states(one, tokens, depth, None, False, 0, ident)
                lp, ent = packed_logprob_entropy(h, head_weight(model), tokens, parent, True, self.head_chunk)
                (lp.sum() + ent.sum()).backward()
        for p in model.parameters():
            p.grad = None
        if self.device.type == "cuda":
            torch.cuda.synchronize(self.device)

    def _full_layers(self, model, T: int):
        if self.device.type != "cuda" or not self.partial_recompute or self.checkpoint_layers is not None:
            return 0
        c = model.config
        head = int(2.0 * T * c.vocab_size * 2 + 2 * 4 * c.vocab_size * c.hidden_size)
        esz = torch.empty(0, dtype=self.dtype).element_size()
        D = getattr(c, "head_dim", None) or c.hidden_size // c.num_attention_heads
        stash_l = 2 * T * c.hidden_size * esz
        attn_l = T * c.num_attention_heads * (D * esz + 4)
        attn_keep = self._attn_keep_planned
        L = self.n_layers

        def plan(layer0_bytes: int) -> int:
            d0 = max(int(layer0_bytes), 1)
            avail = int(0.7 * self._free_hbm()) - 2 * d0 - head
            for n in range(L, 1, -1):
                rec = L - n
                if (n - 1) * d0 + rec * stash_l + min(attn_keep, rec * attn_l) <= avail:
                    return n
            return 1
        return plan

    def _attn_keep_bytes(self) -> int:
        self._attn_keep_planned = 0
        if self.device.type != "cuda" or self.attn_keep_fraction <= 0:
            return 0
        free = self._free_hbm()
        self._attn_keep_planned = int(self.attn_keep_fraction * free)
        return self._attn_keep_planned

    def _path_losses(self, packed, token_trie, lp, ent, loss_fn):
        lp_all, ent_all = lp.detach()[packed.path_cat], ent.detach()[packed.path_cat]
        terms, leaves, o = [], [], 0
        want = torch.is_grad_enabled() and (lp.requires_grad or ent.requires_grad)
        for i, attach_list in enumerate(token_trie.attach_lists):
            for attachment, length in attach_list:
                a, e = lp_all[o + 1:o + length], ent_all[o:o + length]
                if want:
                    a.requires_grad_(lp.requires_grad); e.requires_grad_(ent.requires_grad)
                terms.append(loss_fn(a, e, attachment)); leaves += [a, e]
            o += packed.path_sizes[i]
        return sum_loss_terms(terms, lp.device), leaves

    @staticmethod
    def _backprop_paths(packed, token_trie, lp, ent, total, leaves):
        total.backward()
        rows = None
        roots, grads = [], []
        for k, src in ((0, lp), (1, ent)):
            gs = [t.grad for t in leaves[k::2]]
            if not src.requires_grad or all(g is None for g in gs):
                continue
            if rows is None:
                rows = packed.sequence_rows(token_trie.attach_lists)
            vals = torch.cat([g if g is not None else torch.zeros_like(t) for g, t in zip(gs, leaves[k::2])])
            acc = torch.zeros_like(src)
            acc.index_put_((rows[k],), vals.to(acc.dtype), accumulate=True)
            roots.append(src); grads.append(acc)
        if roots:
            torch.autograd.backward(roots, grads)

    @torch.no_grad()
    def forward(self, model, token_trie) -> List[torch.Tensor]:
        self.model = model
        ensure_supported(model)
        self.returns = [None] * token_trie.n_sequences
        self.forkpos_list = _get_forkpos(None, token_trie.lcp_lens, None)
        if token_trie.n_sequences == 0:
            return self.returns
        with ops.weight_cache():
            return self._forward(model, token_trie)

    def _forward(self, model, token_trie):
        packed = self._pack(token_trie)
        h = packed_hidden_states(model, packed.tokens, packed.depth, packed.meta, False, meta_for_window=packed.for_window)
        lp, _ = packed_logprob_entropy(h, head_weight(model), packed.tokens, packed.parent, False, self.head_chunk,
                                       packed.fork_child, packed.fork_parent, self.tp_group, packed.fork_dev)
        for i, attach_list in enumerate(token_trie.attach_lists):
            lp_path = lp[packed.paths[i][1:]]
            for attachment, length in attach_list:
                self.returns[attachment["_sequence_batch_id"]] = lp_path[:length - 1].clone()
        self.cur_len = 0
        return self.returns

    def backward(self, model, token_trie, loss_fn: Callable, block_size: int, cut_f1_tail: bool = True) -> float:
        self.model = model
        ensure_supported(model)
        lens = [int(ids.size(0)) for ids in token_trie.inputs]
        self.forkpos_list = _get_forkpos(lens, token_trie.lcp_lens, block_size)
        if token_trie.n_sequences == 0:
            return 0.0
        with ops.weight_cache():
            return self._backward(model, token_trie, loss_fn, block_size)

    def _backward(self, model, token_trie, loss_fn, block_size):
        n_tree = sum(token_trie.lens) - sum(token_trie.lcp_lens)
        rows = self._stack_block_rows(model, n_tree, block_size)
        if self.tp_group is not None:
            import torch.distributed as dist
            v = torch.tensor([rows if rows is not None else (1 << 30)], device=self.device, dtype=torch.int32)
            dist.all_reduce(v, op=dist.ReduceOp.MIN, group=self.tp_group)
            rows = None if int(v.item()) >= (1 << 30) else int(v.item())
        if rows is not None:
            longest = max(token_trie.lens)
            assert longest <= self.max_seq_len, f"Exceeds max_seq_len: cur_len=0, new_tokens={longest}, max={self.max_seq_len}"
            return self._backward_stack(model, token_trie, loss_fn, rows)
        packed = self._pack(token_trie)
        chunk = min(self.head_chunk, block_size) if block_size else self.head_chunk
        ckpt = self._should_checkpoint(model, packed.plan.T)
        self.last_mode = "packed+recompute" if ckpt else "packed"
        attn_keep = self._attn_keep_bytes() if ckpt else 0
        full = self._full_layers(model, packed.plan.T) if ckpt else 0
        kept = []
        h = packed_hidden_states(model, packed.tokens, packed.depth, packed.meta, ckpt, attn_keep, None, full, kept,
                                 meta_for_window=packed.for_window)
        if ckpt and kept:
            self.last_mode = "packed" if kept[0] >= self.n_layers else f"packed+recompute[{self.n_layers - kept[0]}/{self.n_layers}]"
        lp, ent = packed_logprob_entropy(h, head_weight(model), packed.tokens, packed.parent, True, max(chunk, 1),
                                         packed.fork_child, packed.fork_parent, self.tp_group, packed.fork_dev)
        total, leaves = self._path_losses(packed, token_trie, lp, ent, loss_fn)
        if total is None:
            return 0.0
        landed = None
        if total.is_cuda:
            if self._loss_host is None:
                self._loss_host = torch.empty(1, dtype=torch.float32).pin_memory()
            self._loss_host.copy_(total.detach().reshape(1).float(), non_blocking=True)
            landed = torch.cuda.Event(); landed.record()
        if total.requires_grad:
            self._backprop_paths(packed, token_trie, lp, ent, total, leaves)
        self.cur_len = 0
        if landed is None:
            return float(total.item())
        landed.synchronize()
        return float(self._loss_host.item())
```

### include/dta.h

```cpp
#ifndef DTA_H
#define DTA_H
#include <stdint.h>

#ifdef __cplusplus
extern "C" {
#endif

#define DTA_OK 0
#define DTA_EINVAL (-1)
#define DTA_EUNSUPPORTED (-2)
#define DTA_EALIGN (-3)
#define DTA_ELAUNCH (-4)
#define DTA_EPRIOR (-5)

#define DTA_BF16 0
#define DTA_F16 1
#define DTA_F32 2

#define DTA_QTILE 128
#define DTA_KTILE 128

int dta_version(void);

int dta_take_pending_error(char* msg, int32_t cap);


int dta_lcp_adjacent(const int64_t* tokens, const int64_t* starts, const int32_t* lens, int32_t S,
                     int32_t* out_lcp, int32_t* out_unsorted, void* stream);

int dta_leafize(const int32_t* lens, const int32_t* lcp, int32_t S,
                int32_t* out_leaf_pos, int32_t* out_leaf_lcp, int32_t* out_seq_leaf, int32_t* out_M,
                void* stream);

int dta_preorder_meta(const int64_t* tokens, const int64_t* leaf_tok_off,
                      const int32_t* seg_off, const int32_t* seg_depth0, const int32_t* parent_of_seg,
                      const int32_t* brk_ptr, const int32_t* brk_depth, const int32_t* brk_end,
                      int32_t M, int32_t T,
                      int64_t* out_token, int32_t* out_depth, int32_t* out_parent, int32_t* out_subtree_end,
                      void* stream);

int dta_tree_attn_fwd(const void* q, const void* k, const void* v, void* out, float* lse,
                      const int32_t* subtree_end, const int32_t* run_ptr, const int32_t* runs,
                      int32_t Tq, int32_t Tk, int32_t q_offset, int32_t Hq, int32_t Hkv, int32_t head_dim,
                      int64_t q_stride_t, int64_t kv_stride_t, int64_t o_stride_t,
                      float scale, int32_t dtype, void* stream);

int dta_tree_attn_fwd_ex(const void* q, const void* k, const void* v, void* out, float* lse,
                         const int32_t* subtree_end, const int32_t* run_ptr, const int32_t* runs,
                         int32_t Tq, int32_t Tk, int32_t q_offset, int32_t Hq, int32_t Hkv, int32_t head_dim,
                         int64_t q_stride_t, int64_t q_stride_h, int64_t k_stride_t, int64_t k_stride_h,
                         int64_t v_stride_t, int64_t v_stride_h,
                         int64_t o_stride_t, int64_t o_stride_h, float scale, int32_t dtype, void* stream);

int dta_tree_attn_bwd(const void* q, const void* k, const void* v, const void* out, const void* dout,
                      const float* lse, float* delta, void* dq, void* dk, void* dv,
                      const int32_t* subtree_end, const int32_t* run_ptr, const int32_t* runs,
                      const int32_t* ktile_qend,
                      int32_t Tq, int32_t Tk, int32_t q_offset, int32_t Hq, int32_t Hkv, int32_t head_dim,
                      int64_t q_stride_t, int64_t kv_stride_t, int64_t o_stride_t,
                      int64_t dq_stride_t, int64_t dkv_stride_t,
                      float scale, int32_t dtype, int32_t accumulate, void* stream);

int dta_tree_attn_bwd_ex(const void* q, const void* k, const void* v, const void* out, const void* dout,
                         const float* lse, float* delta, void* dq, void* dk, void* dv,
                         const int32_t* subtree_end, const int32_t* run_ptr, const int32_t* runs,
                         const int32_t* ktile_qend,
                         int32_t Tq, int32_t Tk, int32_t q_offset, int32_t Hq, int32_t Hkv, int32_t head_dim,
                         int64_t q_stride_t, int64_t q_stride_h, int64_t k_stride_t, int64_t k_stride_h,
                         int64_t v_stride_t, int64_t v_stride_h,
                         int64_t o_stride_t, int64_t o_stride_h, int64_t dq_stride_t, int64_t dq_stride_h,
                         int64_t dkv_stride_t, int64_t dkv_stride_h,
                         float scale, int32_t dtype, int32_t accumulate,
                         int32_t which ,
                         const int32_t* dkv_units, int32_t n_units, const int32_t* dkv_splits, int32_t n_splits, float* dkv_ws,
                         void* stream);

int dta_tree_attn_fwd_win(const void* q, const void* k, const void* v, void* out, float* lse,
                          const int32_t* subtree_end, const int32_t* run_ptr, const int32_t* runs,
                          int32_t Tq, int32_t Tk, int32_t q_offset, int32_t Hq, int32_t Hkv, int32_t head_dim,
                          int64_t q_stride_t, int64_t q_stride_h, int64_t k_stride_t, int64_t k_stride_h,
                          int64_t v_stride_t, int64_t v_stride_h,
                          int64_t o_stride_t, int64_t o_stride_h, float scale, int32_t dtype,
                          const int32_t* win_lo, int32_t window, void* stream);
int dta_tree_attn_bwd_win(const void* q, const void* k, const void* v, const void* out, const void* dout,
                          const float* lse, float* delta, void* dq, void* dk, void* dv,
                          const int32_t* subtree_end, const int32_t* run_ptr, const int32_t* runs,
                          const int32_t* ktile_qend,
                          int32_t Tq, int32_t Tk, int32_t q_offset, int32_t Hq, int32_t Hkv, int32_t head_dim,
                          int64_t q_stride_t, int64_t q_stride_h, int64_t k_stride_t, int64_t k_stride_h,
                          int64_t v_stride_t, int64_t v_stride_h,
                          int64_t o_stride_t, int64_t o_stride_h, int64_t dq_stride_t, int64_t dq_stride_h,
                          int64_t dkv_stride_t, int64_t dkv_stride_h,
                          float scale, int32_t dtype, int32_t accumulate, int32_t which,
                          const int32_t* dkv_units, int32_t n_units, const int32_t* dkv_splits, int32_t n_splits, float* dkv_ws,
                          const int32_t* win_lo, int32_t window, void* stream);
int dta_window_lo(const int32_t* depth, const int32_t* seg_off, const int32_t* seg_depth0, const int32_t* parent_of_seg,
                  int32_t M, int32_t T, int32_t window, int32_t* out_win_lo, void* stream);

int dta_logprob_entropy_fwd(const void* logits, const int64_t* labels, const int32_t* extra_ptr, const int64_t* extra_labels,
                            float* lse, float* entropy, float* logprob, float* extra_logprob,
                            int32_t R, int32_t V, int64_t row_stride, float temperature, int32_t dtype, void* stream);
int dta_logprob_entropy_shard_stats(const void* logits, const int64_t* labels, const int32_t* extra_ptr, const int64_t* extra_labels,
                                    float* stats, float* extra_picked,
                                    int32_t R, int32_t V, int64_t row_stride, float temperature, int32_t dtype, void* stream);
int dta_logprob_entropy_bwd(const void* logits, void* dlogits, const int64_t* labels, const int32_t* extra_ptr, const int64_t* extra_labels,
                            const float* lse, const float* entropy,
                            const float* g_logprob, const float* g_extra_logprob, const float* g_entropy,
                            int32_t R, int32_t V, int64_t row_stride, int64_t out_row_stride, float temperature, int32_t dtype, void* stream);

int dta_rmsnorm_fwd(const void* x, const void* delta, const void* w, void* x_out, void* y, float* rstd,
                    int32_t R, int32_t H, float eps, int32_t dtype, void* stream);
int dta_rmsnorm_bwd_blocks(int32_t R);
int dta_rmsnorm_bwd(const void* x, const void* w, const void* dy, const void* dres, const float* rstd, void* dx, float* dw_partial,
                    int32_t R, int32_t H, int32_t dtype, void* stream);
int dta_qk_norm_rope_fwd(const void* x, const void* w, const float* cos_sin, void* y, float* rstd,
                         int32_t T, int32_t NH, int32_t head_dim, int64_t x_stride_t, float eps, int32_t dtype, void* stream);
int dta_qk_norm_rope_bwd_blocks(int64_t n_heads_total);
int dta_qk_norm_rope_bwd(const void* x, const void* w, const float* cos_sin, const void* dy, const float* rstd,
                         void* dx, float* dw_partial, int32_t T, int32_t NH, int32_t head_dim,
                         int64_t x_stride_t, int64_t dy_stride_t, int64_t dy_stride_h, int64_t dx_stride_t,
                         int32_t dtype, void* stream);
int dta_swiglu_fwd(const void* gate, const void* up, void* y, int64_t rows, int32_t cols, int64_t ld, int32_t dtype, void* stream);
int dta_swiglu_bwd(const void* gate, const void* up, const void* dy, void* dgate, void* dup,
                   int64_t rows, int32_t cols, int64_t ld, int64_t ld_grad, int32_t dtype, void* stream);

int dta_transpose(const void* in, void* out, int64_t rows, int64_t cols, int64_t ld_in, int64_t ld_out, int32_t elem_size, void* stream);

int dta_sum_slabs(const float* part, int64_t slabs, int64_t n, int64_t slab_stride, const float* extra, void* out, int32_t out_dtype, void* stream);

#define DTA_MOE_BM 128
#define DTA_MOE_FWD 0
#define DTA_MOE_DGRAD 1
#define DTA_MOE_WGRAD 2

int dta_moe_router_fwd(const void* logits, int32_t* topk_ids, void* topk_w, float* lse, int32_t T, int32_t E, int32_t k, int32_t norm_topk,
                       int32_t dtype, void* stream);
int dta_moe_router_bwd(const void* logits, const float* lse, const int32_t* topk_ids, const void* dtopk_w, void* dlogits,
                       int32_t T, int32_t E, int32_t k, int32_t norm_topk, int32_t dtype, void* stream);

int dta_moe_permute_workspace(int32_t n_pairs, int32_t E);
int dta_moe_tile_bound(int32_t n_pairs, int32_t E);
int dta_moe_permute(const int32_t* topk_ids, int32_t T, int32_t k, int32_t E, int32_t* workspace,
                    int32_t* expert_offsets, int32_t* row_of_pair, int32_t* src_token, int32_t* tiles, void* stream);

int dta_moe_grouped_gemm(int32_t mode, const void* x, const void* w, const void* dy, void* out, const int32_t* gather,
                         const int32_t* expert_offsets, const int32_t* tiles, int32_t n_rows, int32_t E, int32_t N, int32_t K,
                         int32_t dtype, void* stream);

int dta_moe_combine_fwd(const void* y, const void* topk_w, const int32_t* row_of_pair, void* out, int32_t T, int32_t k, int32_t H,
                        int32_t dtype, void* stream);
int dta_moe_combine_bwd(const void* dout, const void* y, const void* topk_w, const int32_t* row_of_pair, void* dy, void* dtopk_w,
                        int32_t T, int32_t k, int32_t H, int32_t dtype, void* stream);

int dta_lora_down(const void* x, int64_t ldx, const void* m, int64_t ldm, void* out, int64_t ldo, const float* rscale_host,
                  int32_t T, int32_t R, int32_t K, int32_t dtype, void* stream);
int dta_lora_wgrad_slabs(int32_t T, int32_t K);
int dta_lora_wgrad(const void* l, int64_t ldl, const void* x, int64_t ldx, float* part, const float* rscale_host,
                   int32_t T, int32_t R, int32_t K, int32_t dtype, void* stream);

#ifdef __cplusplus
}
#endif
#endif
```

Before: 858,800.

## Hand off dS tiles from dKV kernel to a dedicated dQ kernel

Result: slower. 839,600 (-2.2%).

```diff
diff --git a/dynamictreeattn_amd/_lib.py b/dynamictreeattn_amd/_lib.py
--- a/dynamictreeattn_amd/_lib.py
+++ b/dynamictreeattn_amd/_lib.py
@@ -20,6 +20,8 @@
     "dta_tree_attn_bwd_ex": ([_vp] * 14 + [_i32] * 6 + [_i64] * 12 + [_f32, _i32, _i32, _i32, _vp, _i32, _vp, _i32, _vp, _vp], C.c_int),
     "dta_tree_attn_fwd_win": ([_vp] * 8 + [_i32] * 6 + [_i64] * 8 + [_f32, _i32, _vp, _i32, _vp], C.c_int),
     "dta_tree_attn_bwd_win": ([_vp] * 14 + [_i32] * 6 + [_i64] * 12 + [_f32, _i32, _i32, _i32, _vp, _i32, _vp, _i32, _vp, _vp, _i32, _vp], C.c_int),
+    "dta_tree_attn_bwd_ds": ([_vp] * 14 + [_i32] * 6 + [_i64] * 12 + [_f32, _i32, _i32, _i32, _vp, _i32, _vp, _i32, _vp, _vp, _i32] + [_vp] * 5 + [_vp],
+                             C.c_int),
     "dta_window_lo": ([_vp] * 4 + [_i32, _i32, _i32, _vp, _vp], C.c_int),
     "dta_logprob_entropy_fwd": ([_vp] * 8 + [_i32, _i32, _i64, _f32, _i32, _vp], C.c_int),
     "dta_logprob_entropy_shard_stats": ([_vp] * 6 + [_i32, _i32, _i64, _f32, _i32, _vp], C.c_int),
diff --git a/dynamictreeattn_amd/csrc/tree_attn.hip b/dynamictreeattn_amd/csrc/tree_attn.hip
--- a/dynamictreeattn_amd/csrc/tree_attn.hip
+++ b/dynamictreeattn_amd/csrc/tree_attn.hip
@@ -50,6 +50,7 @@
   int32_t hgroups, head0;
   int64_t q_st, q_sh, kv_st, kv_sh, v_st, v_sh, o_st, o_sh, dq_st, dq_sh, dkv_st, dkv_sh;
   float scale; int32_t accumulate; int32_t ktile;
+  void* ds_ws; const int32_t *ds_tile_ptr, *ds_qptr, *ds_qkt, *ds_order;
 };
 struct AttnParamsW : AttnParams { const int32_t* win_lo; int32_t window; };
 template <bool WIN> using AttnP = typename std::conditional<WIN, AttnParamsW, AttnParams>::type;
@@ -181,6 +182,11 @@
   asm volatile("s_nop 4\n\ts_mov_b32 m0, %2\n\ts_nop 0\n\tglobal_load_lds_dword %0, %1" :: "v"(off), "s"(base), "s"(lds) : "memory");
 }
 #define DMA_WAIT() asm volatile("s_waitcnt vmcnt(0)" ::: "memory")
+#define DMA_WAIT_BUT2() asm volatile("s_waitcnt vmcnt(2)" ::: "memory")
+typedef __attribute__((ext_vector_type(4))) int i32x4;
+__device__ __forceinline__ void ds_store(uint32_t off, i32x4 val, void* base) {
+  asm volatile("global_store_dwordx4 %0, %1, %2\n\ts_nop 0" :: "v"(off), "v"(val), "s"(base) : "memory");
+}
 
 template <int D> __device__ __forceinline__ uint32_t dma_src_off_d(int row, int img_row, int lane, int64_t stride, int esz) {
   if constexpr (D == 128) return (uint32_t)((row * stride + ((lane & 15) ^ (((img_row & 3) << 2) | ((img_row >> 2) & 3))) * 8) * (int64_t)esz);
@@ -620,6 +626,16 @@
   const int total = ntile * p.group;
   const float c = p.scale * LOG2E;
 
+  char* ds_cur = nullptr; int64_t ds_wrap = 0; int ds_left = 0;
+  const uint32_t lane16 = (uint32_t)lane * 16u;
+  if (p.ds_ws) {
+    const int ntile_f = __builtin_amdgcn_readfirstlane(p.ds_tile_ptr[kt + 1] - p.ds_tile_ptr[kt]);
+    const int ds_t0 = (qbeg - k0) >> 6;
+    ds_left = ntile_f - ds_t0;
+    ds_cur = reinterpret_cast<char*>(p.ds_ws) + (((int64_t)p.ds_tile_ptr[kt] * p.Hq + (int64_t)(kvh * p.group) * ntile_f + ds_t0) << 14) + wave8 * 2048;
+    ds_wrap = (int64_t)(ntile_f - ntile) << 14;
+  }
+
   constexpr int NP = DH / 64;
   uint32_t voff_q[NP], voff_d[NP];
 #pragma unroll
@@ -661,6 +677,7 @@
 #define KV2_TILE(BUFI)                                                                                     \
   {                                                                                                        \
     const int ti = ti_c;                                                                                   \
+    const bool ds_st = ds_cur && ti < ds_left;                                                             \
     ti_c += 1;                                                                                             \
     if (ti_c >= ntile) ti_c = 0;                                                                           \
     if (idx + 1 < total) KV2_DMA(1 - (BUFI))       \
@@ -715,13 +732,16 @@
     }                                                                                                      \
     _Pragma("unroll") for (int s2 = 0; s2 < 2; ++s2) {                                                     \
       const v8 pb = pack_half<DT>(S, s2), sbf = pack_half<DT>(DP, s2);                                     \
-      _Pragma("unroll") for (int db = 0; db < NDB; ++db) {                                                 \
+      if (ds_st) ds_store(lane16, __builtin_bit_cast(i32x4, sbf), ds_cur + s2 * 1024);                     \
+      _Pragma("unroll") for (int db = 0; db < NDB; ++db) {                                               \
         const v8 adt = tr_pair<v8>(tb + at[db] + TB + 32 * DH * s2, tb + at[NDB + db] + TB + 32 * DH * s2); \
         const v8 aqt = tr_pair<v8>(tb + at[db] + 32 * DH * s2, tb + at[NDB + db] + 32 * DH * s2);          \
         DV[db] = T::mma(adt, pb, DV[db]); DK[db] = T::mma(aqt, sbf, DK[db]);                               \
       }                                                                                                    \
     }                                                                                                      \
-    DMA_WAIT(); __syncthreads();                                                                           \
+    if (ds_cur) { ds_cur += 16384; if (ti_c == 0) ds_cur += ds_wrap; }                                     \
+    if (ds_st) DMA_WAIT_BUT2(); else DMA_WAIT();          \
+    __syncthreads();                                                                                       \
     ++idx;                                                                                                 \
   }
 
@@ -853,17 +873,158 @@
   }
 }
 
+template <int DT, int DH>
+__global__ __launch_bounds__(256) void tree_attn_bwd_delta_kernel(AttnParams p) {
+  using v8 = typename Ty<DT>::v8; using e = typename Ty<DT>::e;
+  constexpr int LPR = DH / 8;
+  const int64_t idx = (int64_t)blockIdx.x * (256 / LPR) + threadIdx.x / LPR;
+  const int ch = threadIdx.x % LPR;
+  const bool live = idx < (int64_t)p.Tq * p.Hq;
+  const int row = live ? (int)(idx / p.Hq) : 0, hq = live ? (int)(idx % p.Hq) : 0;
+  const int64_t off = (int64_t)row * p.o_st + (int64_t)hq * p.o_sh + 8 * ch;
+  const v8 df = *reinterpret_cast<const v8*>(reinterpret_cast<const e*>(p.dout) + off);
+  const v8 of = *reinterpret_cast<const v8*>(reinterpret_cast<const e*>(p.o) + off);
+  float s = 0.f;
+#pragma unroll
+  for (int j = 0; j < 8; ++j) s += (float)df[j] * (float)of[j];
+#pragma unroll
+  for (int o = LPR / 2; o > 0; o >>= 1) s += __shfl_xor(s, o);
+  if (live && ch == 0) p.delta[(int64_t)hq * p.Tq + row] = -s;
+}
+
+__device__ __forceinline__ void dma_one(uint32_t off, const void* base, uint32_t lds) {
+  asm volatile("s_nop 4\n\ts_mov_b32 m0, %2\n\ts_nop 0\n\tglobal_load_lds_dwordx4 %0, %1" :: "v"(off), "s"(base), "s"(lds) : "memory");
+}
+
+template <int DT, int HPB, int DH>
+__global__ __launch_bounds__(256 * HPB, 2) void tree_attn_bwd_dq_ds_kernel(AttnParams p) {
+  using T = Ty<DT>; using e = typename T::e; using v8 = typename T::v8; using v4 = typename T::v4;
+  constexpr int TBK = tile_bytes<DH>(), NDB = DH / 32, NW = 4 * HPB, KPW = DH / 8 / NW;
+  constexpr int DSI = 64 * 256;
+  constexpr int BUF = HPB * DSI + TBK;
+  __shared__ __attribute__((aligned(16))) char smem[2 * BUF];
+
+  const int tid = threadIdx.x, lane = tid & 63, n = lane & 31, h = lane >> 5;
+  const int wave = __builtin_amdgcn_readfirstlane(tid >> 6);
+  const int hb = wave >> 2, rw = wave & 3;
+  const int bid = blockIdx.x;
+  const int kvh = bid % p.Hkv; const int rest = bid / p.Hkv; const int hgb = rest % p.hgroups;
+  const int qt = __builtin_amdgcn_readfirstlane(p.ds_order[rest / p.hgroups]);
+  const int hq = kvh * p.group + p.head0 + hgb * HPB + hb;
+  const int q0 = qt * DTA_QTILE;
+  const int li = __builtin_amdgcn_readfirstlane(p.ds_qptr[qt]), le = __builtin_amdgcn_readfirstlane(p.ds_qptr[qt + 1]);
+
+  uint32_t voff_s[4]; uint32_t hoff = 0;
+#pragma unroll
+  for (int i = 0; i < 4; ++i) {
+    const int R = 4 * (4 * rw + i) + (lane >> 4);
+    const int cc = (lane & 15) ^ (((R & 3) << 2) | ((R >> 2) & 3));
+    voff_s[i] = (uint32_t)((((((cc >> 2) & 1) * 4 + (R >> 5)) * 2 + ((cc >> 1) & 1)) * 1024) + ((cc & 1) * 32 + (R & 31)) * 16);
+    hoff = (cc >> 3) ? 16384u : 0u;
+  }
+  uint32_t voff_k[KPW];
+#pragma unroll
+  for (int i = 0; i < KPW; ++i) {
+    const int row_ = (512 / DH) * (wave * KPW + i) + (lane >> dma_lane_row_shift<DH>());
+    voff_k[i] = dma_src_off_d<DH>(row_, row_, lane, p.kv_st, sizeof(e));
+  }
+  int bo_lo, bo_hi;
+  { const int i = lane & 15, ch = 4 * rw + 2 * ((lane >> 4) & 1) + ((i & 3) >> 1);
+    bo_lo = img_off_d<128>(4 * h + (i >> 2), ch) + 8 * (i & 1); bo_hi = img_off_d<128>(4 * h + (i >> 2) + 8, ch) + 8 * (i & 1); }
+  const FragOffsT<DH> offk = frag_offsets<DH>(lane);
+  const char* kbase = reinterpret_cast<const char*>(p.k) + (int64_t)kvh * p.kv_sh * (int64_t)sizeof(e);
+  const uint32_t lds0 = lds_addr(smem);
+
+  f32x16 DQ[NDB];
+#pragma unroll
+  for (int db = 0; db < NDB; ++db)
+#pragma unroll
+    for (int g = 0; g < 16; ++g) DQ[db][g] = 0.f;
+
+  const int ntl = le - li;
+#define DQS_DMA(EN, SUB, B)                                                                                \
+  { const int j_ = __builtin_amdgcn_readfirstlane((EN).x), nt_ = __builtin_amdgcn_readfirstlane((EN).y);    \
+    const int tp_ = __builtin_amdgcn_readfirstlane((EN).z), v1_ = __builtin_amdgcn_readfirstlane((EN).w);   \
+    const int k0_ = j_ * DTA_KTILE + 64 * (SUB);                                                            \
+    const char* sb_ = reinterpret_cast<const char*>(p.ds_ws) + (((int64_t)tp_ * p.Hq + (int64_t)hq * nt_ + 2 * (qt - j_)) << 14) + (SUB) * 4096; \
+    const uint32_t ho_ = v1_ ? hoff : 0u;                                                                  \
+    const uint32_t lb_ = lds0 + (uint32_t)(B) * BUF;                                                       \
+    _Pragma("unroll") for (int i_ = 0; i_ < 4; ++i_) dma_one(voff_s[i_] + ho_, sb_, lb_ + hb * DSI + (4 * rw + i_) * 1024); \
+    const char* kb_ = kbase + (int64_t)k0_ * p.kv_st * (int64_t)sizeof(e);                                 \
+    _Pragma("unroll") for (int i_ = 0; i_ < KPW; ++i_) {                                                   \
+      uint32_t ok_ = voff_k[i_];                                                                           \
+      if (k0_ + 64 > p.Tk) {                        \
+        const int row_ = (512 / DH) * (wave * KPW + i_) + (lane >> dma_lane_row_shift<DH>());              \
+        const int rr_ = k0_ + row_ < p.Tk ? row_ : p.Tk - 1 - k0_;                                         \
+        ok_ = dma_src_off_d<DH>(rr_, row_, lane, p.kv_st, sizeof(e)); }                                    \
+      dma_one(ok_, kb_, lb_ + HPB * DSI + (wave * KPW + i_) * 1024); } }
+#define DQS_STAGE(B)                                                                                       \
+  { const char* Ss = smem + (B) * BUF + hb * DSI; const char* Ks = smem + (B) * BUF + HPB * DSI;           \
+    _Pragma("unroll") for (int ks = 0; ks < 4; ++ks) {                                                     \
+      const v8 bf = tr_pair<v8>(Ss + ks * 16 * 256 + bo_lo, Ss + ks * 16 * 256 + bo_hi);                   \
+      _Pragma("unroll") for (int db = 0; db < NDB; ++db) DQ[db] = T::mma(tr_frag_o<v8, DH>(Ks + ks * 16 * (2 * DH), offk, db), bf, DQ[db]); } }
+
+  if (ntl > 0) {
+    int4 en = *reinterpret_cast<const int4*>(p.ds_qkt + 4 * li), en_n = en;
+    DQS_DMA(en, 0, 0)
+    DMA_WAIT(); __syncthreads();
+    for (int m = 0; m < ntl; ++m) {
+      const bool more = m + 1 < ntl;
+      if (more) en_n = *reinterpret_cast<const int4*>(p.ds_qkt + 4 * (li + m + 1));
+      const int cj = __builtin_amdgcn_readfirstlane(en.x), cv1 = __builtin_amdgcn_readfirstlane(en.w);
+      const bool two = cj * DTA_KTILE + 64 < p.Tk;
+      const bool use = rw < 2 || cv1 != 0;
+      if (two) DQS_DMA(en, 1, 1)
+      if (use) DQS_STAGE(0)
+      DMA_WAIT(); __syncthreads();
+      if (!two) break;
+      if (more) DQS_DMA(en_n, 0, 0)
+      if (use && !(rw < 2 && cj == qt)) DQS_STAGE(1)
+      DMA_WAIT(); __syncthreads();
+      en = en_n;
+    }
+  }
+#undef DQS_STAGE
+#undef DQS_DMA
+  const int x = 32 * rw + n, y = x & 15;
+  const int qrow = q0 + (x & ~15) + 8 * ((y >> 2) & 1) + 4 * (y >> 3) + (y & 3);
+  if (qrow < p.Tq) {
+    e* dqp = reinterpret_cast<e*>(p.dq) + (int64_t)qrow * p.dq_st + (int64_t)hq * p.dq_sh;
+#pragma unroll
+    for (int db = 0; db < NDB; ++db)
+#pragma unroll
+      for (int gq = 0; gq < 4; ++gq) {
+        v4 w;
+#pragma unroll
+        for (int j = 0; j < 4; ++j) w[j] = (e)(DQ[db][4 * gq + j] * p.scale);
+        *reinterpret_cast<v4*>(dqp + 32 * db + 8 * gq + 4 * h) = w;
+      }
+  }
+}
+
 template <int DT, int DH, bool WIN>
 void launch_bwd(const AttnP<WIN>& p, const AttnP<WIN>& pp, const AttnP<WIN>& ps, int npair, dim3 gqp, dim3 gqs, int ndkv, bool fin, int n_splits,
                 int which, hipStream_t st) {
-  if (which & 1) {
+  const bool ds = p.ds_tile_ptr != nullptr;
+  if ((which & 1) && !ds) {
     if (npair > 0) hipLaunchKernelGGL((tree_attn_bwd_dq_kernel<DT, 2, DH, WIN>), gqp, dim3(512), 0, st, pp);
     if (p.group % 2) hipLaunchKernelGGL((tree_attn_bwd_dq_kernel<DT, 1, DH, WIN>), gqs, dim3(256), 0, st, ps);
+  }
+  if ((which & 2) && ds) {
+    constexpr int RPB = 256 / (DH / 8);
+    const int64_t rows = (int64_t)p.Tq * p.Hq;
+    hipLaunchKernelGGL((tree_attn_bwd_delta_kernel<DT, DH>), dim3((unsigned)((rows + RPB - 1) / RPB)), dim3(256), 0, st, static_cast<const AttnParams&>(p));
   }
   if (which & 2) hipLaunchKernelGGL((tree_attn_bwd_dkv2_kernel<DT, DH, WIN>), dim3(ndkv * p.Hkv), dim3(512), 0, st, p);
   if (fin && p.dkv_units && n_splits > 0)
     hipLaunchKernelGGL((tree_attn_bwd_dkv_finalize_kernel<DT, DH>), dim3(n_splits * p.Hkv, FIN_SPLIT), dim3(256), 0, st, static_cast<const AttnParams&>(p));
-}
+  if ((which & 1) && ds) {
+    if (npair > 0) hipLaunchKernelGGL((tree_attn_bwd_dq_ds_kernel<DT, 2, DH>), gqp, dim3(512), 0, st, static_cast<const AttnParams&>(pp));
+    if (p.group % 2) hipLaunchKernelGGL((tree_attn_bwd_dq_ds_kernel<DT, 1, DH>), gqs, dim3(256), 0, st, static_cast<const AttnParams&>(ps));
+  }
+}
+
+struct DsArgs { void* ws; const int32_t *tile_ptr, *qptr, *qkt, *order; };
 
 inline bool aligned16(const void* p) { return (reinterpret_cast<uintptr_t>(p) & 15) == 0; }
 
@@ -929,7 +1090,7 @@
                                     int64_t dq_st, int64_t dq_sh, int64_t dkv_st, int64_t dkv_sh,
                                     float scale, int32_t dtype, int32_t accumulate, int32_t which,
                                     const int32_t* dkv_units, int32_t n_units, const int32_t* dkv_splits, int32_t n_splits, float* dkv_ws,
-                                    const int32_t* win_lo, int32_t window, void* stream) {
+                                    const int32_t* win_lo, int32_t window, void* stream, const DsArgs* ds = nullptr) {
   if (!q || !k || !v || !out || !dout || !lse || !delta || !dq || !dk || !dv || Tq <= 0 || Tk <= 0 || Hq <= 0 || Hkv <= 0 || q_offset < 0) return DTA_EINVAL;
   if ((runs == nullptr) != (run_ptr == nullptr)) return DTA_EINVAL;
   if (dkv_units && (n_units <= 0 || n_splits < 0 || (n_splits > 0 && (!dkv_splits || !dkv_ws)))) return DTA_EINVAL;
@@ -949,6 +1110,7 @@
   p.q = q; p.k = k; p.v = v; p.o = out; p.dout = dout; p.lse_r = lse; p.delta = delta; p.dq = dq; p.dk = dk; p.dv = dv;
   p.subtree_end = subtree_end; p.run_ptr = run_ptr; p.runs = runs; p.ktile_qend = ktile_qend;
   p.dkv_units = dkv_units; p.dkv_splits = dkv_splits; p.dkv_ws = dkv_ws;
+  if (ds) { p.ds_ws = ds->ws; p.ds_tile_ptr = ds->tile_ptr; p.ds_qptr = ds->qptr; p.ds_qkt = ds->qkt; p.ds_order = ds->order; }
   p.Tq = Tq; p.Tk = Tk; p.q_offset = q_offset; p.Hq = Hq; p.Hkv = Hkv; p.group = Hq / Hkv;
   p.q_st = q_st; p.q_sh = q_sh; p.kv_st = kv_st; p.kv_sh = kv_sh; p.v_st = v_st; p.v_sh = v_sh; p.o_st = o_st; p.o_sh = o_sh;
   p.dq_st = dq_st; p.dq_sh = dq_sh; p.dkv_st = dkv_st; p.dkv_sh = dkv_sh; p.scale = scale; p.accumulate = accumulate;
@@ -1037,6 +1199,33 @@
                         dkv_units, n_units, dkv_splits, n_splits, dkv_ws, win_lo, window, stream);
 }
 
+extern "C" int dta_tree_attn_bwd_ds(const void* q, const void* k, const void* v, const void* out, const void* dout,
+                                    const float* lse, float* delta, void* dq, void* dk, void* dv,
+                                    const int32_t* subtree_end, const int32_t* run_ptr, const int32_t* runs,
+                                    const int32_t* ktile_qend,
+                                    int32_t Tq, int32_t Tk, int32_t q_offset, int32_t Hq, int32_t Hkv, int32_t head_dim,
+                                    int64_t q_st, int64_t q_sh, int64_t kv_st, int64_t kv_sh, int64_t v_st, int64_t v_sh, int64_t o_st, int64_t o_sh,
+                                    int64_t dq_st, int64_t dq_sh, int64_t dkv_st, int64_t dkv_sh,
+                                    float scale, int32_t dtype, int32_t accumulate, int32_t which,
+                                    const int32_t* dkv_units, int32_t n_units, const int32_t* dkv_splits, int32_t n_splits, float* dkv_ws,
+                                    const int32_t* win_lo, int32_t window,
+                                    void* ds_ws, const int32_t* ds_tile_ptr, const int32_t* ds_qptr, const int32_t* ds_qkt, const int32_t* ds_order,
+                                    void* stream) {
+  if (!ds_tile_ptr || !ds_qptr || !ds_qkt || !ds_order || ((which & 1) && !ds_ws)) return DTA_EINVAL;
+  if (!subtree_end || !runs || !ktile_qend || q_offset != 0 || Tq != Tk) return DTA_EUNSUPPORTED;
+  if (dtype != DTA_BF16 && dtype != DTA_F16) return DTA_EUNSUPPORTED;
+  if (kv_st < 0 || kv_st > (1 << 24)) return DTA_EUNSUPPORTED;
+  const DsArgs ds{ds_ws, ds_tile_ptr, ds_qptr, ds_qkt, ds_order};
+  const int w = window_args(subtree_end, win_lo, window);
+  if (w < 0) return w;
+  if (w == 0) return attn_bwd<false>(q, k, v, out, dout, lse, delta, dq, dk, dv, subtree_end, run_ptr, runs, ktile_qend, Tq, Tk, q_offset, Hq, Hkv, head_dim,
+                                     q_st, q_sh, kv_st, kv_sh, v_st, v_sh, o_st, o_sh, dq_st, dq_sh, dkv_st, dkv_sh, scale, dtype, accumulate, which,
+                                     dkv_units, n_units, dkv_splits, n_splits, dkv_ws, nullptr, 0, stream, &ds);
+  return attn_bwd<true>(q, k, v, out, dout, lse, delta, dq, dk, dv, subtree_end, run_ptr, runs, ktile_qend, Tq, Tk, q_offset, Hq, Hkv, head_dim,
+                        q_st, q_sh, kv_st, kv_sh, v_st, v_sh, o_st, o_sh, dq_st, dq_sh, dkv_st, dkv_sh, scale, dtype, accumulate, which,
+                        dkv_units, n_units, dkv_splits, n_splits, dkv_ws, win_lo, window, stream, &ds);
+}
+
 extern "C" int dta_tree_attn_fwd(const void* q, const void* k, const void* v, void* out, float* lse,
                                  const int32_t* subtree_end, const int32_t* run_ptr, const int32_t* runs,
                                  int32_t Tq, int32_t Tk, int32_t q_offset, int32_t Hq, int32_t Hkv, int32_t head_dim,
diff --git a/dynamictreeattn_amd/ops.py b/dynamictreeattn_amd/ops.py
--- a/dynamictreeattn_amd/ops.py
+++ b/dynamictreeattn_amd/ops.py
@@ -142,6 +142,31 @@
     return out, lse, k, v
 
 
+DS_HBM_SHARE = 0.5
+
+
+def _ds_alloc(nbytes: int, device) -> torch.Tensor:
+    return torch.empty(nbytes, dtype=torch.uint8, device=device)
+
+
+def ds_handoff_tables(meta: TreeAttnMeta, kq_host=None):
+    if meta.subtree_end is None or meta.runs is None or meta.ktile_qend is None or meta.q_offset != 0 or (meta.window > 0 and meta.win_lo is None):
+        return None
+    t = getattr(meta, "_ds_tables", None)
+    if t is None:
+        dev = meta.ktile_qend.device
+        T = int(meta.subtree_end.numel())
+        tp, qptr, qkt, order = packing.plan_ds_handoff(meta.ktile_qend.cpu().numpy() if kq_host is None else kq_host, T)
+        t = (int(tp[-1]),) + tuple(torch.from_numpy(np.ascontiguousarray(a)).to(dev) for a in (tp, qptr, qkt, order))
+        meta._ds_tables = t
+    return t
+
+
+def ds_handoff_bytes(meta: TreeAttnMeta, Hq: int) -> int:
+    t = ds_handoff_tables(meta)
+    return 0 if t is None else t[0] * Hq * packing.DS_TILE_BYTES
+
+
 def attn_bwd_raw(q, k, v, out, dout, lse, meta: TreeAttnMeta, scale: float, dk=None, dv=None, accumulate=False, dq=None):
     Tq, Hq, D = q.shape
     Tk, Hkv, _ = k.shape
@@ -161,8 +186,28 @@
     ws = torch.empty((meta.n_slabs, Hkv, 2, packing.KTILE, D), dtype=torch.float32, device=q.device) if (units is not None and meta.n_slabs) else None
 
     win = (ptr(meta.win_lo), int(meta.window)) if meta.window > 0 else ()
+    packed16 = q.dtype != torch.float32 and meta.subtree_end is not None and Tq == Tk == meta.subtree_end.numel()
+    ds = ds_handoff_tables(meta) if packed16 else None
+    ds_ws = None
+    if ds is not None:
+        nbytes = ds[0] * Hq * packing.DS_TILE_BYTES
+        fits = getattr(meta, "_ds_fits", None)
+        if fits is None or fits[0] != nbytes:
+            fits = meta._ds_fits = (nbytes, nbytes <= DS_HBM_SHARE * free_hbm(q.device))
+        if fits[1]:
+            ds_ws = _ds_alloc(max(nbytes, 16), q.device)
+        else:
+            ds = None
 
     def launch(which, stream):
+        if ds is not None:
+            return lib().dta_tree_attn_bwd_ds(
+                ptr(q), ptr(k), ptr(v), ptr(out), ptr(dout), ptr(lse), ptr(delta), ptr(dq), ptr(dk), ptr(dv),
+                ptr(meta.subtree_end), ptr(meta.run_ptr), ptr(meta.runs), ptr(meta.ktile_qend),
+                Tq, Tk, meta.q_offset, Hq, Hkv, D, qs, qh, ks, kh, vs, vh, os_, oh, dqs, dqh, dks, dkh,
+                float(scale), _DT[q.dtype], int(accumulate), which,
+                ptr(units), n_units, ptr(splits) if n_splits else None, n_splits, ptr(ws),
+                *(win or (None, 0)), ptr(ds_ws), ptr(ds[1]), ptr(ds[2]), ptr(ds[3]), ptr(ds[4]), stream)
         return getattr(lib(), "dta_tree_attn_bwd_win" if win else "dta_tree_attn_bwd_ex")(
             ptr(q), ptr(k), ptr(v), ptr(out), ptr(dout), ptr(lse), ptr(delta), ptr(dq), ptr(dk), ptr(dv),
             ptr(meta.subtree_end), ptr(meta.run_ptr), ptr(meta.runs), ptr(meta.ktile_qend),
@@ -170,11 +215,14 @@
             float(scale), _DT[q.dtype], int(accumulate), which,
             ptr(units), n_units, ptr(splits) if n_splits else None, n_splits, ptr(ws), *win, stream)
     tm = KernelTimer.active
+    order = ((1, "bwd_dq"), (2 | 8, "bwd_dkv"), (4, "bwd_dkv_finalize"))
+    if ds is not None:
+        order = order[1:] + order[:1]
     with _on(q, k, v, out, dout, lse, dk, dv, meta.subtree_end, units, meta.win_lo) as stream:
         if tm is None:
             check(launch(3, stream), "dta_tree_attn_bwd")
         else:
-            for which, name in ((1, "bwd_dq"), (2 | 8, "bwd_dkv"), (4, "bwd_dkv_finalize")):
+            for which, name in order:
                 if which == 4 and not n_splits:
                     continue
                 a, b = tm.span(name); a.record(); st = launch(which, stream); b.record()
@@ -305,9 +353,11 @@
     rp, runs = packing.plan_qtile_runs_window(plan, wl_host)
     kq = packing.ktile_qend_window(packing.ktile_qend_host(plan), wl_host)
     units, splits, n_slabs = packing.plan_dkv_units(kq, plan.T, plan.T, 0, Hkv)
-    return TreeAttnMeta(T=plan.T, subtree_end=meta.subtree_end, run_ptr=up(rp), runs=up(runs).view(-1, 4), ktile_qend=up(kq),
-                        dkv_units=up(units).view(-1, 4), dkv_splits=up(splits).view(-1, 4) if splits.shape[0] else None, n_slabs=n_slabs,
-                        win_lo=win_lo, window=int(window))
+    wm = TreeAttnMeta(T=plan.T, subtree_end=meta.subtree_end, run_ptr=up(rp), runs=up(runs).view(-1, 4), ktile_qend=up(kq),
+                      dkv_units=up(units).view(-1, 4), dkv_splits=up(splits).view(-1, 4) if splits.shape[0] else None, n_slabs=n_slabs,
+                      win_lo=win_lo, window=int(window))
+    ds_handoff_tables(wm, kq)
+    return wm
 
 
 def logprob_entropy_fwd_raw(logits, labels, want_entropy=True, temperature=1.0, extra_ptr=None, extra_labels=None, extra_out=None):
diff --git a/dynamictreeattn_amd/packing.py b/dynamictreeattn_amd/packing.py
--- a/dynamictreeattn_amd/packing.py
+++ b/dynamictreeattn_amd/packing.py
@@ -331,3 +331,30 @@
     kmax = np.minimum((np.arange(nkt, dtype=np.int64) + 1) * tile, T) - 1
     qe = np.searchsorted(sufmin, kmax, side="right")
     return np.minimum(ktile_qend.astype(np.int64), qe).astype(np.int32)
+
+
+
+DS_TILE_BYTES = 64 * KTILE * 2
+
+
+def plan_ds_handoff(ktile_qend: np.ndarray, T: int, tile: int = KTILE, qtile: int = QTILE):
+    assert tile == 128 and qtile == 128
+    kq = np.asarray(ktile_qend, np.int64)
+    nkt = kq.shape[0]
+    nqt = (T + qtile - 1) // qtile
+    k0 = np.arange(nkt, dtype=np.int64) * tile
+    qe = np.minimum(kq, T)
+    ntile = np.maximum(0, -(-(qe - k0) // 64))
+    tile_ptr = np.concatenate([[0], np.cumsum(ntile)])
+    if int(tile_ptr[-1]) >= 2 ** 31:
+        raise ValueError("dS hand-off: tile count does not fit int32")
+    cnt = np.maximum(0, -(-qe // qtile) - np.arange(nkt, dtype=np.int64))
+    jj = np.repeat(np.arange(nkt, dtype=np.int64), cnt)
+    qq = jj + np.arange(jj.shape[0], dtype=np.int64) - np.repeat(np.cumsum(cnt) - cnt, cnt)
+    o = np.lexsort((jj, qq))
+    jj, qq = jj[o], qq[o]
+    per_q = np.bincount(qq, minlength=nqt)[:nqt] if qq.size else np.zeros(nqt, np.int64)
+    qptr = np.concatenate([[0], np.cumsum(per_q)])
+    qkt = np.stack([jj, ntile[jj], tile_ptr[jj], (qe[jj] > qq * qtile + 64).astype(np.int64)], axis=1) if jj.size else np.zeros((0, 4), np.int64)
+    order = np.argsort(-per_q, kind="stable")
+    return tile_ptr.astype(np.int32), qptr.astype(np.int32), qkt.astype(np.int32), order.astype(np.int32)
diff --git a/dynamictreeattn_amd/tree_training_engine.py b/dynamictreeattn_amd/tree_training_engine.py
--- a/dynamictreeattn_amd/tree_training_engine.py
+++ b/dynamictreeattn_amd/tree_training_engine.py
@@ -126,6 +126,7 @@
         self.meta = ops.TreeAttnMeta(T=T, subtree_end=self.subtree_end, run_ptr=run_ptr_d, runs=runs_d.view(-1, 4), ktile_qend=kq_d,
                                      dkv_units=units_d.view(-1, 4), dkv_splits=splits_d.view(-1, 4) if splits.shape[0] else None,
                                      n_slabs=n_slabs)
+        ops.ds_handoff_tables(self.meta, kq)
         self._seg_tables, self._n_kv_heads, self._win_metas = (seg_off, seg_d0, par_seg), n_kv_heads, {}
 
     def for_window(self, window: int):
@@ -211,11 +212,16 @@
     def _should_checkpoint(self, model, T: int) -> bool:
         if self.checkpoint_layers is not None:
             return self.checkpoint_layers
-        need = self._per_token_layer_bytes(model) * self.n_layers * T
+        need = self._per_token_layer_bytes(model) * self.n_layers * T + self._ds_workspace_bytes(model)
         if self.device.type != "cuda":
             return False
         free = self._free_hbm()
         return need > 0.75 * free
+
+    def _ds_workspace_bytes(self, model) -> int:
+        if self.last_packed is None or self.dtype == torch.float32:
+            return 0
+        return ops.ds_handoff_bytes(self.last_packed.meta, model.config.num_attention_heads)
 
     def _free_hbm(self) -> int:
         return ops.free_hbm(self.device)
@@ -305,10 +311,11 @@
         attn_l = T * c.num_attention_heads * (D * esz + 4)
         attn_keep = self._attn_keep_planned
         L = self.n_layers
+        ds_ws = self._ds_workspace_bytes(model)
 
         def plan(layer0_bytes: int) -> int:
             d0 = max(int(layer0_bytes), 1)
-            avail = int(0.7 * self._free_hbm()) - 2 * d0 - head
+            avail = int(0.7 * self._free_hbm()) - 2 * d0 - head - ds_ws
             for n in range(L, 1, -1):
                 rec = L - n
                 if (n - 1) * d0 + rec * stash_l + min(attn_keep, rec * attn_l) <= avail:
diff --git a/include/dta.h b/include/dta.h
--- a/include/dta.h
+++ b/include/dta.h
@@ -94,6 +94,20 @@
                           float scale, int32_t dtype, int32_t accumulate, int32_t which,
                           const int32_t* dkv_units, int32_t n_units, const int32_t* dkv_splits, int32_t n_splits, float* dkv_ws,
                           const int32_t* win_lo, int32_t window, void* stream);
+int dta_tree_attn_bwd_ds(const void* q, const void* k, const void* v, const void* out, const void* dout,
+                         const float* lse, float* delta, void* dq, void* dk, void* dv,
+                         const int32_t* subtree_end, const int32_t* run_ptr, const int32_t* runs,
+                         const int32_t* ktile_qend,
+                         int32_t Tq, int32_t Tk, int32_t q_offset, int32_t Hq, int32_t Hkv, int32_t head_dim,
+                         int64_t q_stride_t, int64_t q_stride_h, int64_t k_stride_t, int64_t k_stride_h,
+                         int64_t v_stride_t, int64_t v_stride_h,
+                         int64_t o_stride_t, int64_t o_stride_h, int64_t dq_stride_t, int64_t dq_stride_h,
+                         int64_t dkv_stride_t, int64_t dkv_stride_h,
+                         float scale, int32_t dtype, int32_t accumulate, int32_t which,
+                         const int32_t* dkv_units, int32_t n_units, const int32_t* dkv_splits, int32_t n_splits, float* dkv_ws,
+                         const int32_t* win_lo, int32_t window,
+                         void* ds_ws, const int32_t* ds_tile_ptr, const int32_t* ds_qptr, const int32_t* ds_qkt, const int32_t* ds_order,
+                         void* stream);
 int dta_window_lo(const int32_t* depth, const int32_t* seg_off, const int32_t* seg_depth0, const int32_t* parent_of_seg,
                   int32_t M, int32_t T, int32_t window, int32_t* out_win_lo, void* stream);
 
```
